# AsherJingkongChen/vlm-bridge-for-image-captioning

Hardware: NVIDIA B200
Metric: bridge fwd+bwd samples/sec (higher is better)
Workload: dtype bf16

## Files before the change

### include/b200_bridge.h

```cpp
#ifndef B200_BRIDGE_H_
#define B200_BRIDGE_H_

#include <stddef.h>
#include <stdint.h>

#ifdef __cplusplus
extern "C" {
#endif

#define B200B_ABI_VERSION 3

#define B200B_OK 0
#define B200B_ERR_SHAPE (-1)
#define B200B_ERR_ALIGN (-2)
#define B200B_ERR_ARG (-3)
#define B200B_ERR_DRIVER (-4)
#define B200B_ERR_TENSORMAP (-5)
#define B200B_ERR_WORKSPACE (-6)
#define B200B_ERR_DEVICE (-7)

int b200b_abi_version(void);
const char* b200b_last_error(void);
uint64_t b200b_launch_count(void);

int b200b_profile_begin(void* stream);
int b200b_profile_end(void);
const char* b200b_profile_entry(int index, float* ms);


enum b200b_epilogue {
  B200B_EPI_BF16_BIAS = 0,
  B200B_EPI_BF16_BIAS_GELU = 1,
  B200B_EPI_F32_BIAS_RESID = 2,
  B200B_EPI_BF16_DGELU = 3,
  B200B_EPI_F32 = 4
};

typedef struct b200b_gemm_args {
  const void* a;
  const void* b;
  int32_t a_major, b_major;
  int32_t m, n, k;
  int64_t lda, ldb;
  int32_t epilogue;
  int32_t block_n;
  void* out;
  int64_t ldo;
  void* aux;
  int64_t ldaux;
  const float* bias;
  const float* resid;
  int64_t ldr;
  float beta;
  float dropout_p;
  uint64_t seed;
  uint32_t dropout_stream;
  uint32_t cta_group;
} b200b_gemm_args;

int b200b_gemm(const b200b_gemm_args* args, void* stream);

int b200b_gemm_dual(const b200b_gemm_args* dgrad, const b200b_gemm_args* wgrad, void* stream);
int b200b_gemm_set_dual(int on);


int b200b_layernorm_fwd(const float* x, const float* gamma, const float* beta, void* y_bf16,
                        float* mean, float* rstd, int rows, int dim, float eps, void* stream);

int b200b_layernorm_bwd(const void* dy_bf16, const float* x, const float* mean, const float* rstd,
                        const float* gamma, const float* dres, float* dx, int rows, int dim,
                        void* stream);

size_t b200b_colsum_workspace_bytes(int rows, int cols);
int b200b_colsum(const void* dy_bf16, int64_t ld, const float* x, const float* mean,
                 const float* rstd, float* out_sum, float* out_gsum, int rows, int cols,
                 void* workspace, size_t workspace_bytes, void* stream);

int b200b_cast_bf16(const float* in, void* out_bf16, int64_t n, float dropout_p, uint64_t seed,
                    uint32_t dropout_stream, void* stream);

#define B200B_MAX_COLSUM_TASKS 16
typedef struct b200b_colsum_task {
  const float* partials;
  float* out;
  int32_t cols, chunks;
  int64_t chunk_stride;
} b200b_colsum_task;

int b200b_row_chunks(int rows);
int b200b_layernorm_fwd_rows(const float* x, const float* gamma, const float* beta, void* y_bf16,
                             float* mean, float* rstd, int rows, int dim, float eps, void* stream);
int b200b_layernorm_bwd_fused(const void* dy_bf16, const float* x, const float* mean, const float* rstd,
                              const float* gamma, const float* dres, float* dx, void* dy_next_bf16,
                              float* partials, int rows, int dim, void* stream);
int b200b_cast_bf16_colsum(const float* in, void* out_bf16, float* partials, int rows, int dim,
                           float dropout_p, uint64_t seed, uint32_t dropout_stream, void* stream);
int b200b_colsum_partials(const void* dy_bf16, int64_t ld, int rows, int cols, float* partials,
                          int* chunks_out, void* stream);
int b200b_colsum_finalize(const b200b_colsum_task* tasks, int ntasks, void* stream);

typedef struct b200b_attn_args {
  const void* q; int64_t ldq;
  const void* k; int64_t ldk;
  const void* v; int64_t ldv;
  void* o; int64_t ldo;
  float* lse;
  const void* d_o; int64_t lddo;
  void* dq; int64_t lddq;
  void* dk; int64_t lddk;
  void* dv; int64_t lddv;
  void* workspace; uint64_t workspace_bytes;
  int32_t batch, heads, len_q, len_k, head_dim;
  float dropout_p;
  uint64_t seed;
  uint32_t dropout_stream;
  uint32_t reserved;
} b200b_attn_args;

int b200b_attention_fwd(const b200b_attn_args* args, void* stream);
int b200b_attention_set_tc(int mask);
size_t b200b_attention_bwd_workspace_bytes(int batch, int heads, int len_q, int len_k);
int b200b_attention_bwd(const b200b_attn_args* args, void* stream);

size_t b200b_kv_cache_packed_bytes(int batch, int len_k, int heads, int head_dim, int num_blocks);
int b200b_kv_cache_pack(const void* kv, int64_t ldkv, void* packed, int batch, int len_k, int heads,
                        int head_dim, int num_blocks, void* stream);
int b200b_attention_decode_packed(const void* q, int64_t ldq, const void* kv_packed, int block_index,
                                  int num_blocks, void* o, int64_t ldo, float* lse, int batch, int heads,
                                  int len_q, int len_k, int head_dim, void* stream);

size_t b200b_kv_cache_tc_bytes(int batch, int len_k, int heads, int head_dim, int num_blocks);
int b200b_kv_cache_pack_tc(const void* kv, int64_t ldkv, void* packed, int batch, int len_k, int heads,
                           int head_dim, int num_blocks, void* stream);
int b200b_attention_decode_tc(const void* q, int64_t ldq, const void* kv_tc, int block_index, int num_blocks,
                              void* o, int64_t ldo, float* lse, int batch, int heads, int len_q, int len_k,
                              int head_dim, void* stream);

typedef struct b200b_bridge_dims {
  int32_t batch, len_text, len_vision;
  int32_t dim, dim_vision, dim_ffn;
  int32_t heads_cross, heads_self;
  int32_t num_blocks;
  int32_t flags;
} b200b_bridge_dims;

#define B200B_BRIDGE_WGRAD_BF16 1
#define B200B_BRIDGE_SEED_INDIRECT 2
#define B200B_BRIDGE_KV_PACKED 4
#define B200B_BRIDGE_KV_TC 8
#define B200B_BRIDGE_PART_CROSS 16
#define B200B_BRIDGE_PART_REST 32
#define B200B_SEED_INDIRECT 0x80000000u

typedef struct b200b_block_weights {
  const void* wq_c;
  const void* wo_c;
  const void* wqkv_s;
  const void* wo_s;
  const void* w1;
  const void* w2;
  const float* bq_c;
  const float* bo_c;
  const float* bqkv_s;
  const float* bo_s;
  const float* b1;
  const float* b2;
  const float* ln_c_g; const float* ln_c_b;
  const float* ln_s_g; const float* ln_s_b;
  const float* ln_f_g; const float* ln_f_b;
} b200b_block_weights;

typedef struct b200b_block_grads {
  void* wq_c; void* wo_c; void* wqkv_s; void* wo_s; void* w1; void* w2;
  float* bq_c; float* bo_c; float* bqkv_s; float* bo_s; float* b1; float* b2;
  float* ln_c_g; float* ln_c_b; float* ln_s_g; float* ln_s_b; float* ln_f_g; float* ln_f_b;
} b200b_block_grads;

size_t b200b_bridge_block_saved_bytes(const b200b_bridge_dims* dims);
size_t b200b_bridge_backward_workspace_bytes(const b200b_bridge_dims* dims);

int b200b_bridge_kv_project(const b200b_bridge_dims* dims, const float* vision_f32,
                            const void* wkv_all, const float* bkv_all, void* vision_bf16,
                            void* kv, void* stream);

int b200b_bridge_block_forward(const b200b_bridge_dims* dims, int block_index,
                               const b200b_block_weights* w, const float* x_in, const void* kv,
                               float* x_out, void* saved, size_t saved_bytes, float dropout_p,
                               uint64_t seed, void* stream);

typedef void (*b200b_grad_ready_fn)(void* user, const void* grad, int64_t elems);
typedef struct b200b_grad_notify {
  b200b_grad_ready_fn fn;
  void* user;
} b200b_grad_notify;

int b200b_bridge_block_backward(const b200b_bridge_dims* dims, int block_index,
                                const b200b_block_weights* w, const float* x_in, const void* kv,
                                const void* saved, const float* d_out, float* d_in, void* dkv,
                                const b200b_block_grads* g, void* workspace, size_t workspace_bytes,
                                float dropout_p, uint64_t seed, const b200b_grad_notify* notify,
                                void* stream);

int b200b_bridge_kv_backward(const b200b_bridge_dims* dims, const void* vision_bf16,
                             const void* dkv, void* dwkv_all, float* dbkv_all, void* workspace,
                             size_t workspace_bytes, void* stream);

size_t b200b_bridge_f32_workspace_bytes(const b200b_bridge_dims* dims);
int b200b_bridge_kv_project_f32(const b200b_bridge_dims* dims, const float* vision, const float* wkv_all,
                                const float* bkv_all, float* kv, void* stream);
int b200b_bridge_block_forward_f32(const b200b_bridge_dims* dims, int block_index, const b200b_block_weights* w,
                                   const float* x_in, const float* kv, float* x_out, void* workspace,
                                   size_t workspace_bytes, void* stream);

size_t b200b_grad_sqnorm_workspace_bytes(void);
int b200b_grad_sqnorm(const float* grad, int64_t n, const void* grad_bf16, int64_t n_bf16, void* workspace,
                      size_t workspace_bytes, float* out2, void* stream);
int b200b_adamw_fused(float* param, const float* grad, const void* grad_bf16, float* exp_avg, float* exp_avg_sq,
                      void* weights_bf16,
                      int64_t n, int64_t n_bf16, const float* sqnorm2, float max_grad_norm,
                      const float* grad_scale, const float* found_inf, float lr, float beta1, float beta2,
                      float eps, float weight_decay, int64_t step, float* step_dev, void* stream);

int b200b_cross_entropy_fwd(const void* logits, int dtype, int64_t ld, const int64_t* labels, int64_t rows,
                            int64_t vocab, int64_t ignore_index, int64_t shift_len, float* lse,
                            float* loss_rows, float* out2, void* stream);
int b200b_cross_entropy_bwd(const void* logits, int dtype, int64_t ld, const int64_t* labels, int64_t rows,
                            int64_t vocab, int64_t ignore_index, int64_t shift_len, const float* lse,
                            const float* out2, const float* grad_loss, void* dlogits, int64_t ldd,
                            void* stream);

int b200b_bf16_to_f32(const void* in_bf16, float* out, int64_t n, float scale, void* stream);

#define B200B_NVLS_MAX_RANKS 8
#define B200B_NVLS_MAX_BLOCKS 160
#define B200B_DTYPE_BF16 0
#define B200B_DTYPE_F32 1
typedef struct b200b_nvls_comm {
  void* multicast_base;
  void* local_base;
  void* flags[B200B_NVLS_MAX_RANKS];
  int32_t rank, world;
  int32_t timeout_s;
  int32_t reserved;
  void* error_word;
} b200b_nvls_comm;
#define B200B_NVLS_OUT_MULTICAST 1u
#define B200B_NVLS_EXCLUSIVE_SMS 2u
#define B200B_NVLS_UNROLL(n) (((uint32_t)(n) & 0xffu) << 8)
size_t b200b_allreduce_nvls_flag_bytes(void);
int b200b_allreduce_nvls(const b200b_nvls_comm* comm, int dtype, int64_t byte_offset, int64_t bytes,
                         float scale, float* out_f32, uint32_t epoch, const uint32_t* epoch_base,
                         int blocks, int threads, uint32_t flags, void* stream);

void b200b_set_sm_limit(int sms);
int b200b_get_sm_limit(void);

#ifdef __cplusplus
}
#endif
#endif
```

### vlm-bridge-for-image-captioning_b200/_lib.py

```python
from __future__ import annotations

import ctypes as C
import os
import threading

_PKG_DIR = os.path.dirname(os.path.abspath(__file__))
LIB_PATH = os.path.join(_PKG_DIR, "csrc", "libb200_bridge.so")

EPI_BF16_BIAS = 0
EPI_BF16_BIAS_GELU = 1
EPI_F32_BIAS_RESID = 2
EPI_BF16_DGELU = 3
EPI_F32 = 4
NVLS_OUT_MULTICAST = 1
NVLS_EXCLUSIVE_SMS = 2


class GemmArgs(C.Structure):
    _fields_ = [
        ("a", C.c_void_p),
        ("b", C.c_void_p),
        ("a_major", C.c_int32),
        ("b_major", C.c_int32),
        ("m", C.c_int32),
        ("n", C.c_int32),
        ("k", C.c_int32),
        ("lda", C.c_int64),
        ("ldb", C.c_int64),
        ("epilogue", C.c_int32),
        ("block_n", C.c_int32),
        ("out", C.c_void_p),
        ("ldo", C.c_int64),
        ("aux", C.c_void_p),
        ("ldaux", C.c_int64),
        ("bias", C.c_void_p),
        ("resid", C.c_void_p),
        ("ldr", C.c_int64),
        ("beta", C.c_float),
        ("dropout_p", C.c_float),
        ("seed", C.c_uint64),
        ("dropout_stream", C.c_uint32),
        ("cta_group", C.c_uint32),
    ]


class ColsumTask(C.Structure):
    _fields_ = [("partials", C.c_void_p), ("out", C.c_void_p), ("cols", C.c_int32), ("chunks", C.c_int32),
                ("chunk_stride", C.c_int64)]


class NvlsComm(C.Structure):
    _fields_ = [("multicast_base", C.c_void_p), ("local_base", C.c_void_p), ("flags", C.c_void_p * 8),
                ("rank", C.c_int32), ("world", C.c_int32), ("timeout_s", C.c_int32), ("reserved", C.c_int32),
                ("error_word", C.c_void_p)]


class AttnArgs(C.Structure):
    _fields_ = [
        ("q", C.c_void_p), ("ldq", C.c_int64),
        ("k", C.c_void_p), ("ldk", C.c_int64),
        ("v", C.c_void_p), ("ldv", C.c_int64),
        ("o", C.c_void_p), ("ldo", C.c_int64),
        ("lse", C.c_void_p),
        ("d_o", C.c_void_p), ("lddo", C.c_int64),
        ("dq", C.c_void_p), ("lddq", C.c_int64),
        ("dk", C.c_void_p), ("lddk", C.c_int64),
        ("dv", C.c_void_p), ("lddv", C.c_int64),
        ("workspace", C.c_void_p), ("workspace_bytes", C.c_uint64),
        ("batch", C.c_int32), ("heads", C.c_int32), ("len_q", C.c_int32), ("len_k", C.c_int32),
        ("head_dim", C.c_int32),
        ("dropout_p", C.c_float),
        ("seed", C.c_uint64),
        ("dropout_stream", C.c_uint32),
        ("reserved", C.c_uint32),
    ]


_lock = threading.Lock()
_lib = None


def _declare(lib) -> None:
    lib.b200b_abi_version.restype = C.c_int
    lib.b200b_abi_version.argtypes = []
    lib.b200b_last_error.restype = C.c_char_p
    lib.b200b_last_error.argtypes = []
    lib.b200b_launch_count.restype = C.c_uint64
    lib.b200b_launch_count.argtypes = []
    lib.b200b_profile_begin.restype = C.c_int
    lib.b200b_profile_begin.argtypes = [C.c_void_p]
    lib.b200b_profile_end.restype = C.c_int
    lib.b200b_profile_end.argtypes = []
    lib.b200b_profile_entry.restype = C.c_char_p
    lib.b200b_profile_entry.argtypes = [C.c_int, C.POINTER(C.c_float)]
    lib.b200b_gemm.restype = C.c_int
    lib.b200b_gemm.argtypes = [C.POINTER(GemmArgs), C.c_void_p]
    lib.b200b_layernorm_fwd.restype = C.c_int
    lib.b200b_layernorm_fwd.argtypes = [C.c_void_p] * 6 + [C.c_int, C.c_int, C.c_float, C.c_void_p]
    lib.b200b_layernorm_bwd.restype = C.c_int
    lib.b200b_layernorm_bwd.argtypes = [C.c_void_p] * 7 + [C.c_int, C.c_int, C.c_void_p]
    lib.b200b_colsum_workspace_bytes.restype = C.c_size_t
    lib.b200b_colsum_workspace_bytes.argtypes = [C.c_int, C.c_int]
    lib.b200b_colsum.restype = C.c_int
    lib.b200b_colsum.argtypes = [C.c_void_p, C.c_int64] + [C.c_void_p] * 5 + [C.c_int, C.c_int, C.c_void_p,
                                                                               C.c_size_t, C.c_void_p]
    lib.b200b_cast_bf16.restype = C.c_int
    lib.b200b_cast_bf16.argtypes = [C.c_void_p, C.c_void_p, C.c_int64, C.c_float, C.c_uint64, C.c_uint32,
                                    C.c_void_p]
    lib.b200b_row_chunks.restype = C.c_int
    lib.b200b_row_chunks.argtypes = [C.c_int]
    lib.b200b_layernorm_fwd_rows.restype = C.c_int
    lib.b200b_layernorm_fwd_rows.argtypes = [C.c_void_p] * 6 + [C.c_int, C.c_int, C.c_float, C.c_void_p]
    lib.b200b_layernorm_bwd_fused.restype = C.c_int
    lib.b200b_layernorm_bwd_fused.argtypes = [C.c_void_p] * 9 + [C.c_int, C.c_int, C.c_void_p]
    lib.b200b_cast_bf16_colsum.restype = C.c_int
    lib.b200b_cast_bf16_colsum.argtypes = [C.c_void_p] * 3 + [C.c_int, C.c_int, C.c_float, C.c_uint64, C.c_uint32,
                                           C.c_void_p]
    lib.b200b_colsum_partials.restype = C.c_int
    lib.b200b_colsum_partials.argtypes = [C.c_void_p, C.c_int64, C.c_int, C.c_int, C.c_void_p, C.POINTER(C.c_int),
                                          C.c_void_p]
    lib.b200b_bf16_to_f32.restype = C.c_int
    lib.b200b_bf16_to_f32.argtypes = [C.c_void_p, C.c_void_p, C.c_int64, C.c_float, C.c_void_p]
    lib.b200b_allreduce_nvls_flag_bytes.restype = C.c_size_t
    lib.b200b_allreduce_nvls_flag_bytes.argtypes = []
    lib.b200b_allreduce_nvls.restype = C.c_int
    lib.b200b_allreduce_nvls.argtypes = [C.POINTER(NvlsComm), C.c_int, C.c_int64, C.c_int64, C.c_float, C.c_void_p,
                                         C.c_uint32, C.c_void_p, C.c_int, C.c_int, C.c_uint32, C.c_void_p]
    lib.b200b_grad_sqnorm_workspace_bytes.restype = C.c_size_t
    lib.b200b_grad_sqnorm_workspace_bytes.argtypes = []
    lib.b200b_grad_sqnorm.restype = C.c_int
    lib.b200b_grad_sqnorm.argtypes = [C.c_void_p, C.c_int64, C.c_void_p, C.c_int64, C.c_void_p, C.c_size_t, C.c_void_p, C.c_void_p]
    lib.b200b_adamw_fused.restype = C.c_int
    lib.b200b_adamw_fused.argtypes = [C.c_void_p] * 6 + [C.c_int64, C.c_int64, C.c_void_p, C.c_float, C.c_void_p,
                                                          C.c_void_p] + [C.c_float] * 5 + [C.c_int64, C.c_void_p, C.c_void_p]
    lib.b200b_cross_entropy_fwd.restype = C.c_int
    lib.b200b_cross_entropy_fwd.argtypes = [C.c_void_p, C.c_int, C.c_int64, C.c_void_p] + [C.c_int64] * 4 + [C.c_void_p] * 4
    lib.b200b_cross_entropy_bwd.restype = C.c_int
    lib.b200b_cross_entropy_bwd.argtypes = ([C.c_void_p, C.c_int, C.c_int64, C.c_void_p] + [C.c_int64] * 4 +
                                            [C.c_void_p] * 4 + [C.c_int64, C.c_void_p])
    lib.b200b_gemm_dual.restype = C.c_int
    lib.b200b_gemm_dual.argtypes = [C.POINTER(GemmArgs), C.POINTER(GemmArgs), C.c_void_p]
    lib.b200b_gemm_set_dual.restype = C.c_int
    lib.b200b_gemm_set_dual.argtypes = [C.c_int]
    lib.b200b_attention_set_tc.restype = C.c_int
    lib.b200b_attention_set_tc.argtypes = [C.c_int]
    lib.b200b_set_sm_limit.restype = None
    lib.b200b_set_sm_limit.argtypes = [C.c_int]
    lib.b200b_get_sm_limit.restype = C.c_int
    lib.b200b_get_sm_limit.argtypes = []
    lib.b200b_colsum_finalize.restype = C.c_int
    lib.b200b_colsum_finalize.argtypes = [C.POINTER(ColsumTask), C.c_int, C.c_void_p]
    lib.b200b_attention_fwd.restype = C.c_int
    lib.b200b_attention_fwd.argtypes = [C.POINTER(AttnArgs), C.c_void_p]
    lib.b200b_kv_cache_packed_bytes.restype = C.c_size_t
    lib.b200b_kv_cache_packed_bytes.argtypes = [C.c_int] * 5
    lib.b200b_kv_cache_pack.restype = C.c_int
    lib.b200b_kv_cache_pack.argtypes = [C.c_void_p, C.c_int64, C.c_void_p] + [C.c_int] * 5 + [C.c_void_p]
    lib.b200b_attention_decode_packed.restype = C.c_int
    lib.b200b_attention_decode_packed.argtypes = [C.c_void_p, C.c_int64, C.c_void_p, C.c_int, C.c_int, C.c_void_p,
                                                  C.c_int64, C.c_void_p] + [C.c_int] * 5 + [C.c_void_p]
    lib.b200b_kv_cache_tc_bytes.restype = C.c_size_t
    lib.b200b_kv_cache_tc_bytes.argtypes = [C.c_int] * 5
    lib.b200b_kv_cache_pack_tc.restype = C.c_int
    lib.b200b_kv_cache_pack_tc.argtypes = [C.c_void_p, C.c_int64, C.c_void_p] + [C.c_int] * 5 + [C.c_void_p]
    lib.b200b_attention_decode_tc.restype = C.c_int
    lib.b200b_attention_decode_tc.argtypes = [C.c_void_p, C.c_int64, C.c_void_p, C.c_int, C.c_int, C.c_void_p,
                                              C.c_int64, C.c_void_p] + [C.c_int] * 5 + [C.c_void_p]
    lib.b200b_attention_bwd_workspace_bytes.restype = C.c_size_t
    lib.b200b_attention_bwd_workspace_bytes.argtypes = [C.c_int] * 4
    lib.b200b_attention_bwd.restype = C.c_int
    lib.b200b_attention_bwd.argtypes = [C.POINTER(AttnArgs), C.c_void_p]


def lib():
    global _lib
    if _lib is None:
        with _lock:
            if _lib is None:
                if not os.path.exists(LIB_PATH):
                    raise RuntimeError(
                        f"{LIB_PATH} is missing: build it with `python -m vlm_bridge_b200.build` "
                        "(there is no CPU or PyTorch fallback for the bridge kernels)"
                    )
                handle = C.CDLL(LIB_PATH)
                _declare(handle)
                _lib = handle
    return _lib


def check(rc: int, what: str) -> None:
    if rc != 0:
        msg = lib().b200b_last_error().decode("utf-8", "replace")
        raise RuntimeError(f"b200b {what} failed (rc={rc}): {msg}")


def launch_count() -> int:
    return int(lib().b200b_launch_count())


def profile_begin(stream_ptr: int) -> None:
    check(lib().b200b_profile_begin(C.c_void_p(stream_ptr)), "profile_begin")


def profile_end() -> list[tuple[str, float]]:
    n = lib().b200b_profile_end()
    out = []
    ms = C.c_float()
    for i in range(n):
        name = lib().b200b_profile_entry(i, C.byref(ms))
        if name is None:
            break
        out.append((name.decode(), float(ms.value)))
    return out
```

### vlm-bridge-for-image-captioning_b200/csrc/bridge.cu

```cuda
#include <string.h>

#include "common.cuh"
#include "launch.h"

namespace b200b {

static inline size_t al256(size_t x) { return (x + 255) & ~(size_t)255; }

struct Carver {
  uint8_t* base;
  size_t off = 0;
  explicit Carver(void* b) : base(reinterpret_cast<uint8_t*>(b)) {}
  template <typename T>
  T* take(size_t count) {
    T* p = reinterpret_cast<T*>(base + off);
    off += al256(count * sizeof(T));
    return p;
  }
};

struct Dims {
  int B, L, Nv, D, Dv, F, Hc, Hs, nb, flags;
  size_t T, Tv;
  int dc, ds;
};

static int read_dims(const b200b_bridge_dims* d, Dims* o, const char* what) {
  if (d == nullptr) {
    set_last_error("%s: null dims", what);
    return B200B_ERR_ARG;
  }
  o->B = d->batch; o->L = d->len_text; o->Nv = d->len_vision;
  o->D = d->dim; o->Dv = d->dim_vision; o->F = d->dim_ffn;
  o->Hc = d->heads_cross; o->Hs = d->heads_self; o->nb = d->num_blocks; o->flags = d->flags;
  if (o->B <= 0 || o->L <= 0 || o->Nv <= 0 || o->D <= 0 || o->Dv <= 0 || o->F <= 0 || o->Hc <= 0 || o->Hs <= 0 ||
      o->nb <= 0) {
    set_last_error("%s: all dims must be positive", what);
    return B200B_ERR_SHAPE;
  }
  if ((o->D % 8) || (o->Dv % 8) || (o->F % 8) || (o->D % o->Hc) || (o->D % o->Hs)) {
    set_last_error("%s: dim/dim_vision/dim_ffn must be multiples of 8 and dim divisible by the head counts", what);
    return B200B_ERR_SHAPE;
  }
  o->T = (size_t)o->B * o->L;
  o->Tv = (size_t)o->B * o->Nv;
  o->dc = o->D / o->Hc;
  o->ds = o->D / o->Hs;
  if (o->T > 0x7fffffff || o->Tv > 0x7fffffff) {
    set_last_error("%s: too many rows", what);
    return B200B_ERR_SHAPE;
  }
  return B200B_OK;
}

struct Saved {
  __nv_bfloat16 *xn1, *q, *o1, *xn2, *qkv, *o2, *xn3, *u, *h;
  float *x1, *x2;
  float *mean1, *rstd1, *mean2, *rstd2, *mean3, *rstd3;
  float *lse1, *lse2;
  size_t bytes;
};

static Saved carve_saved(const Dims& d, void* base) {
  Carver c(base);
  Saved s;
  const size_t TD = d.T * d.D, TF = d.T * d.F;
  s.xn1 = c.take<__nv_bfloat16>(TD);
  s.q = c.take<__nv_bfloat16>(TD);
  s.o1 = c.take<__nv_bfloat16>(TD);
  s.xn2 = c.take<__nv_bfloat16>(TD);
  s.qkv = c.take<__nv_bfloat16>(3 * TD);
  s.o2 = c.take<__nv_bfloat16>(TD);
  s.xn3 = c.take<__nv_bfloat16>(TD);
  s.u = c.take<__nv_bfloat16>(TF);
  s.h = c.take<__nv_bfloat16>(TF);
  s.x1 = c.take<float>(TD);
  s.x2 = c.take<float>(TD);
  s.mean1 = c.take<float>(d.T); s.rstd1 = c.take<float>(d.T);
  s.mean2 = c.take<float>(d.T); s.rstd2 = c.take<float>(d.T);
  s.mean3 = c.take<float>(d.T); s.rstd3 = c.take<float>(d.T);
  s.lse1 = c.take<float>((size_t)d.B * d.Hc * d.L);
  s.lse2 = c.take<float>((size_t)d.B * d.Hs * d.L);
  s.bytes = c.off;
  return s;
}

constexpr int kMaxRowChunks = 320;
struct BwdWs {
  __nv_bfloat16 *dy, *du, *dxn, *dattn, *dqkv;
  float* dx;
  uint8_t* attn_ws; size_t attn_ws_bytes;
  float *p_cast, *p_du, *p_lnf, *p_dqkv, *p_lns, *p_dq, *p_lnc, *p_dkv;
  size_t bytes;
};

static BwdWs carve_bwd(const Dims& d, void* base) {
  Carver c(base);
  BwdWs w;
  const size_t TD = d.T * d.D, TF = d.T * d.F;
  w.dy = c.take<__nv_bfloat16>(TD);
  w.du = c.take<__nv_bfloat16>(TF);
  w.dxn = c.take<__nv_bfloat16>(TD);
  w.dattn = c.take<__nv_bfloat16>(TD);
  w.dqkv = c.take<__nv_bfloat16>(3 * TD);
  w.dx = c.take<float>(TD);
  const size_t a1 = b200b_attention_bwd_workspace_bytes(d.B, d.Hc, d.L, d.Nv);
  const size_t a2 = b200b_attention_bwd_workspace_bytes(d.B, d.Hs, d.L, d.L);
  w.attn_ws_bytes = a1 > a2 ? a1 : a2;
  w.attn_ws = c.take<uint8_t>(w.attn_ws_bytes);
  const size_t rc = d.T < (size_t)kMaxRowChunks ? d.T : (size_t)kMaxRowChunks;
  const size_t D = d.D;
  w.p_cast = c.take<float>(rc * D);
  w.p_du = c.take<float>((size_t)64 * d.F);
  w.p_lnf = c.take<float>(rc * 3 * D);
  w.p_dqkv = c.take<float>((size_t)64 * 3 * D);
  w.p_lns = c.take<float>(rc * 3 * D);
  w.p_dq = c.take<float>((size_t)64 * D);
  w.p_lnc = c.take<float>(rc * 3 * D);
  w.p_dkv = c.take<float>((size_t)64 * 2 * D * d.nb);
  w.bytes = c.off;
  return w;
}

struct Finalizer {
  b200b_colsum_task t[B200B_MAX_COLSUM_TASKS];
  int n = 0;
  void add(const float* partials, float* out, int cols, int chunks, long long stride) {
    t[n].partials = partials; t[n].out = out; t[n].cols = cols; t[n].chunks = chunks; t[n].chunk_stride = stride;
    ++n;
  }
};

#define B200B_TRY(expr)        \
  do {                         \
    int rc_ = (expr);          \
    if (rc_ != B200B_OK) return rc_; \
  } while (0)

static int gemm(const void* a, int a_major, long long lda, const void* b, int b_major, long long ldb, int m, int n,
                int k, int epi, void* out, long long ldo, const float* bias, const float* resid, void* aux,
                long long ldaux, float p, uint64_t seed, uint32_t dstream, cudaStream_t st) {
  b200b_gemm_args g;
  memset(&g, 0, sizeof(g));
  g.a = a; g.b = b; g.a_major = a_major; g.b_major = b_major;
  g.m = m; g.n = n; g.k = k; g.lda = lda; g.ldb = ldb;
  g.epilogue = epi; g.block_n = 0;
  g.out = out; g.ldo = ldo; g.aux = aux; g.ldaux = ldaux;
  g.bias = bias; g.resid = resid; g.ldr = ldo;
  g.beta = 0.f; g.dropout_p = p; g.seed = seed; g.dropout_stream = dstream;
  return b200b_gemm(&g, st);
}

static int grad_pair(const void* dy, long long lddy, const void* w, const void* x, long long ldx, int rows, int n_out,
                     int n_in, void* dx, long long lddx, void* dw, int wgrad_epi, cudaStream_t st) {
  b200b_gemm_args dg, wg;
  memset(&dg, 0, sizeof(dg));
  memset(&wg, 0, sizeof(wg));
  dg.a = dy; dg.a_major = 0; dg.lda = lddy;
  dg.b = w; dg.b_major = 1; dg.ldb = n_in;
  dg.m = rows; dg.n = n_in; dg.k = n_out;
  dg.epilogue = B200B_EPI_BF16_BIAS; dg.out = dx; dg.ldo = lddx;
  wg.a = dy; wg.a_major = 1; wg.lda = lddy;
  wg.b = x; wg.b_major = 1; wg.ldb = ldx;
  wg.m = n_out; wg.n = n_in; wg.k = rows;
  wg.epilogue = wgrad_epi; wg.out = dw; wg.ldo = n_in;
  return b200b_gemm_dual(&dg, &wg, st);
}

static int attn(bool bwd, const void* q, long long ldq, const void* k, long long ldk, const void* v, long long ldv,
                void* o, long long ldo, float* lse, const void* d_o, void* dq, long long lddq, void* dk, long long lddk,
                void* dv, long long lddv, void* ws, size_t ws_bytes, int B, int H, int Lq, int Lk, int hd, float p,
                uint64_t seed, uint32_t dstream, cudaStream_t st) {
  b200b_attn_args a;
  memset(&a, 0, sizeof(a));
  a.q = q; a.ldq = ldq; a.k = k; a.ldk = ldk; a.v = v; a.ldv = ldv; a.o = o; a.ldo = ldo; a.lse = lse;
  a.d_o = d_o; a.lddo = ldo; a.dq = dq; a.lddq = lddq; a.dk = dk; a.lddk = lddk; a.dv = dv; a.lddv = lddv;
  a.workspace = ws; a.workspace_bytes = ws_bytes;
  a.batch = B; a.heads = H; a.len_q = Lq; a.len_k = Lk; a.head_dim = hd;
  a.dropout_p = p; a.seed = seed; a.dropout_stream = dstream;
  return bwd ? b200b_attention_bwd(&a, st) : b200b_attention_fwd(&a, st);
}

static inline uint32_t ds_cross(int i) { return 16u * i + 0; }
static inline uint32_t ds_self(int i) { return 16u * i + 1; }
static inline uint32_t ds_ffn_h(int i) { return 16u * i + 2; }
static inline uint32_t ds_ffn_o(int i) { return 16u * i + 3; }

}

using namespace b200b;

extern "C" size_t b200b_bridge_block_saved_bytes(const b200b_bridge_dims* dims) {
  Dims d;
  if (read_dims(dims, &d, "block_saved_bytes") != B200B_OK) return 0;
  return carve_saved(d, nullptr).bytes;
}

extern "C" size_t b200b_bridge_backward_workspace_bytes(const b200b_bridge_dims* dims) {
  Dims d;
  if (read_dims(dims, &d, "backward_workspace_bytes") != B200B_OK) return 0;
  return carve_bwd(d, nullptr).bytes;
}

extern "C" int b200b_bridge_kv_project(const b200b_bridge_dims* dims, const float* vision_f32, const void* wkv_all,
                                       const float* bkv_all, void* vision_bf16, void* kv, void* stream_) {
  cudaStream_t st = reinterpret_cast<cudaStream_t>(stream_);
  Dims d;
  B200B_TRY(read_dims(dims, &d, "kv_project"));
  if (!vision_f32 || !wkv_all || !bkv_all || !vision_bf16 || !kv) {
    set_last_error("kv_project: null argument");
    return B200B_ERR_ARG;
  }
  const int n = 2 * d.D * d.nb;
  B200B_TRY(b200b_cast_bf16(vision_f32, vision_bf16, (int64_t)d.Tv * d.Dv, 0.f, 0, 0, st));
  return gemm(vision_bf16, 0, d.Dv, wkv_all, 0, d.Dv, (int)d.Tv, n, d.Dv, B200B_EPI_BF16_BIAS, kv, n, bkv_all, nullptr,
              nullptr, 0, 0.f, 0, 0, st);
}

extern "C" int b200b_bridge_block_forward(const b200b_bridge_dims* dims, int i, const b200b_block_weights* w,
                                          const float* x_in, const void* kv, float* x_out, void* saved,
                                          size_t saved_bytes, float p, uint64_t seed, void* stream_) {
  cudaStream_t st = reinterpret_cast<cudaStream_t>(stream_);
  Dims d;
  B200B_TRY(read_dims(dims, &d, "block_forward"));
  if (!w || !x_in || !kv || !x_out || !saved || i < 0 || i >= d.nb) {
    set_last_error("block_forward: null argument or bad block index");
    return B200B_ERR_ARG;
  }
  Saved s = carve_saved(d, saved);
  if (saved_bytes < s.bytes) {
    set_last_error("block_forward: saved arena too small (%zu < %zu)", saved_bytes, s.bytes);
    return B200B_ERR_WORKSPACE;
  }
  const int T = (int)d.T, D = d.D, F = d.F;
  const uint32_t ind = (d.flags & B200B_BRIDGE_SEED_INDIRECT) ? B200B_SEED_INDIRECT : 0u;
  const long long ldkv = 2LL * D * d.nb;
  const __nv_bfloat16* kblk = reinterpret_cast<const __nv_bfloat16*>(kv) + (size_t)2 * D * i;
  const float eps = 1e-5f;

  const bool do_cross = !(d.flags & B200B_BRIDGE_PART_REST), do_rest = !(d.flags & B200B_BRIDGE_PART_CROSS);
  if (!do_cross && !do_rest) {
    set_last_error("block_forward: PART_CROSS and PART_REST are exclusive");
    return B200B_ERR_ARG;
  }
  if ((!do_cross || !do_rest) && p != 0.f) {
    set_last_error("block_forward: running a part of a block needs dropout_p == 0");
    return B200B_ERR_ARG;
  }
  float* x1w = do_rest ? s.x1 : x_out;
  const float* x1 = do_cross ? x1w : x_in;

  if (do_cross) {
    B200B_TRY(b200b_layernorm_fwd_rows(x_in, w->ln_c_g, w->ln_c_b, s.xn1, s.mean1, s.rstd1, T, D, eps, st));
    B200B_TRY(gemm(s.xn1, 0, D, w->wq_c, 0, D, T, D, D, B200B_EPI_BF16_BIAS, s.q, D, w->bq_c, nullptr, nullptr, 0, 0.f,
                   0, 0, st));
    if (d.flags & (B200B_BRIDGE_KV_PACKED | B200B_BRIDGE_KV_TC)) {
      if (p != 0.f || d.L > 64) {
        set_last_error("block_forward: a packed K/V cache needs dropout_p == 0 and len_text <= 64");
        return B200B_ERR_ARG;
      }
      if (d.flags & B200B_BRIDGE_KV_TC)
        B200B_TRY(b200b_attention_decode_tc(s.q, D, kv, i, d.nb, s.o1, D, s.lse1, d.B, d.Hc, d.L, d.Nv, d.dc, st));
      else
        B200B_TRY(b200b_attention_decode_packed(s.q, D, kv, i, d.nb, s.o1, D, s.lse1, d.B, d.Hc, d.L, d.Nv, d.dc, st));
    } else {
      B200B_TRY(attn(false, s.q, D, kblk, ldkv, kblk + D, ldkv, s.o1, D, s.lse1, nullptr, nullptr, 0, nullptr, 0,
                     nullptr, 0, nullptr, 0, d.B, d.Hc, d.L, d.Nv, d.dc, p, seed, (ds_cross(i) | ind), st));
    }
    B200B_TRY(gemm(s.o1, 0, D, w->wo_c, 0, D, T, D, D, B200B_EPI_F32_BIAS_RESID, x1w, D, w->bo_c, x_in, nullptr, 0, 0.f,
                   0, 0, st));
  }
  if (!do_rest) return B200B_OK;
  B200B_TRY(b200b_layernorm_fwd_rows(x1, w->ln_s_g, w->ln_s_b, s.xn2, s.mean2, s.rstd2, T, D, eps, st));
  B200B_TRY(gemm(s.xn2, 0, D, w->wqkv_s, 0, D, T, 3 * D, D, B200B_EPI_BF16_BIAS, s.qkv, 3 * D, w->bqkv_s, nullptr,
                 nullptr, 0, 0.f, 0, 0, st));
  B200B_TRY(attn(false, s.qkv, 3 * D, s.qkv + D, 3 * D, s.qkv + 2 * D, 3 * D, s.o2, D, s.lse2, nullptr, nullptr, 0,
                 nullptr, 0, nullptr, 0, nullptr, 0, d.B, d.Hs, d.L, d.L, d.ds, p, seed, (ds_self(i) | ind), st));
  B200B_TRY(gemm(s.o2, 0, D, w->wo_s, 0, D, T, D, D, B200B_EPI_F32_BIAS_RESID, s.x2, D, w->bo_s, x1, nullptr, 0, 0.f,
                 0, 0, st));
  B200B_TRY(b200b_layernorm_fwd_rows(s.x2, w->ln_f_g, w->ln_f_b, s.xn3, s.mean3, s.rstd3, T, D, eps, st));
  B200B_TRY(gemm(s.xn3, 0, D, w->w1, 0, D, T, F, D, B200B_EPI_BF16_BIAS_GELU, s.h, F, w->b1, nullptr, s.u, F, p, seed,
                 (ds_ffn_h(i) | ind), st));
  B200B_TRY(gemm(s.h, 0, F, w->w2, 0, F, T, D, F, B200B_EPI_F32_BIAS_RESID, x_out, D, w->b2, s.x2, nullptr, 0, p, seed,
                 (ds_ffn_o(i) | ind), st));
  return B200B_OK;
}

extern "C" int b200b_bridge_block_backward(const b200b_bridge_dims* dims, int i, const b200b_block_weights* w,
                                           const float* x_in, const void* kv, const void* saved, const float* d_out,
                                           float* d_in, void* dkv, const b200b_block_grads* g, void* workspace,
                                           size_t workspace_bytes, float p, uint64_t seed,
                                           const b200b_grad_notify* notify, void* stream_) {
  cudaStream_t st = reinterpret_cast<cudaStream_t>(stream_);
  Dims d;
  B200B_TRY(read_dims(dims, &d, "block_backward"));
  if (!w || !x_in || !kv || !saved || !d_out || !dkv || !g || !workspace || i < 0 || i >= d.nb) {
    set_last_error("block_backward: null argument or bad block index");
    return B200B_ERR_ARG;
  }
  Saved s = carve_saved(d, const_cast<void*>(saved));
  BwdWs ws = carve_bwd(d, workspace);
  if (workspace_bytes < ws.bytes) {
    set_last_error("block_backward: workspace too small (%zu < %zu)", workspace_bytes, ws.bytes);
    return B200B_ERR_WORKSPACE;
  }
  const int T = (int)d.T, D = d.D, F = d.F;
  const uint32_t ind = (d.flags & B200B_BRIDGE_SEED_INDIRECT) ? B200B_SEED_INDIRECT : 0u;
  const long long ldkv = 2LL * D * d.nb;
  const __nv_bfloat16* kblk = reinterpret_cast<const __nv_bfloat16*>(kv) + (size_t)2 * D * i;
  __nv_bfloat16* dkblk = reinterpret_cast<__nv_bfloat16*>(dkv) + (size_t)2 * D * i;
  const int EB = B200B_EPI_BF16_BIAS;
  const int EW = (d.flags & B200B_BRIDGE_WGRAD_BF16) ? B200B_EPI_BF16_BIAS : B200B_EPI_F32;
  auto ready = [&](const void* grad, long long elems) {
    if (notify != nullptr && notify->fn != nullptr) notify->fn(notify->user, grad, elems);
  };

  const int rchunks = b200b_row_chunks(T);
  if (rchunks <= 0 || rchunks > kMaxRowChunks) {
    set_last_error("block_backward: no usable device (row chunks = %d)", rchunks);
    return B200B_ERR_DEVICE;
  }
  Finalizer fin;
  int ch = 0;

  B200B_TRY(b200b_cast_bf16_colsum(d_out, ws.dy, ws.p_cast, T, D, p, seed, (ds_ffn_o(i) | ind), st));
  fin.add(ws.p_cast, g->b2, D, rchunks, D);
  B200B_TRY(gemm(ws.dy, 1, D, s.h, 1, F, D, F, T, EW, g->w2, F, nullptr, nullptr, nullptr, 0, 0.f, 0, 0, st));
  ready(g->w2, (long long)D * F);
  B200B_TRY(gemm(ws.dy, 0, D, w->w2, 1, F, T, F, D, B200B_EPI_BF16_DGELU, ws.du, F, nullptr, nullptr, s.u, F, p, seed,
                 (ds_ffn_h(i) | ind), st));
  B200B_TRY(b200b_colsum_partials(ws.du, F, T, F, ws.p_du, &ch, st));
  fin.add(ws.p_du, g->b1, F, ch, F);
  B200B_TRY(gemm(ws.du, 1, F, s.xn3, 1, D, F, D, T, EW, g->w1, D, nullptr, nullptr, nullptr, 0, 0.f, 0, 0, st));
  ready(g->w1, (long long)F * D);
  B200B_TRY(gemm(ws.du, 0, F, w->w1, 1, D, T, D, F, EB, ws.dxn, D, nullptr, nullptr, nullptr, 0, 0.f, 0, 0, st));
  B200B_TRY(b200b_layernorm_bwd_fused(ws.dxn, s.x2, s.mean3, s.rstd3, w->ln_f_g, d_out, ws.dx, ws.dy, ws.p_lnf, T, D, st));
  fin.add(ws.p_lnf, g->ln_f_b, D, rchunks, 3LL * D);
  fin.add(ws.p_lnf + D, g->ln_f_g, D, rchunks, 3LL * D);
  fin.add(ws.p_lnf + 2 * D, g->bo_s, D, rchunks, 3LL * D);
  B200B_TRY(grad_pair(ws.dy, D, w->wo_s, s.o2, D, T, D, D, ws.dattn, D, g->wo_s, EW, st));
  ready(g->wo_s, (long long)D * D);
  B200B_TRY(attn(true, s.qkv, 3 * D, s.qkv + D, 3 * D, s.qkv + 2 * D, 3 * D, s.o2, D, s.lse2, ws.dattn, ws.dqkv, 3 * D,
                 ws.dqkv + D, 3 * D, ws.dqkv + 2 * D, 3 * D, ws.attn_ws, ws.attn_ws_bytes, d.B, d.Hs, d.L, d.L, d.ds, p,
                 seed, (ds_self(i) | ind), st));
  B200B_TRY(b200b_colsum_partials(ws.dqkv, 3 * D, T, 3 * D, ws.p_dqkv, &ch, st));
  fin.add(ws.p_dqkv, g->bqkv_s, 3 * D, ch, 3LL * D);
  B200B_TRY(grad_pair(ws.dqkv, 3 * D, w->wqkv_s, s.xn2, D, T, 3 * D, D, ws.dxn, D, g->wqkv_s, EW, st));
  ready(g->wqkv_s, 3LL * D * D);
  B200B_TRY(b200b_layernorm_bwd_fused(ws.dxn, s.x1, s.mean2, s.rstd2, w->ln_s_g, ws.dx, ws.dx, ws.dy, ws.p_lns, T, D, st));
  fin.add(ws.p_lns, g->ln_s_b, D, rchunks, 3LL * D);
  fin.add(ws.p_lns + D, g->ln_s_g, D, rchunks, 3LL * D);
  fin.add(ws.p_lns + 2 * D, g->bo_c, D, rchunks, 3LL * D);
  B200B_TRY(grad_pair(ws.dy, D, w->wo_c, s.o1, D, T, D, D, ws.dattn, D, g->wo_c, EW, st));
  ready(g->wo_c, (long long)D * D);
  __nv_bfloat16* dq = ws.dqkv;
  B200B_TRY(attn(true, s.q, D, kblk, ldkv, kblk + D, ldkv, s.o1, D, s.lse1, ws.dattn, dq, D, dkblk, ldkv, dkblk + D, ldkv,
                 ws.attn_ws, ws.attn_ws_bytes, d.B, d.Hc, d.L, d.Nv, d.dc, p, seed, (ds_cross(i) | ind), st));
  B200B_TRY(b200b_colsum_partials(dq, D, T, D, ws.p_dq, &ch, st));
  fin.add(ws.p_dq, g->bq_c, D, ch, D);
  B200B_TRY(grad_pair(dq, D, w->wq_c, s.xn1, D, T, D, D, ws.dxn, D, g->wq_c, EW, st));
  ready(g->wq_c, (long long)D * D);
  B200B_TRY(b200b_layernorm_bwd_fused(ws.dxn, x_in, s.mean1, s.rstd1, w->ln_c_g, ws.dx, d_in, nullptr, ws.p_lnc, T, D, st));
  fin.add(ws.p_lnc, g->ln_c_b, D, rchunks, 3LL * D);
  fin.add(ws.p_lnc + D, g->ln_c_g, D, rchunks, 3LL * D);
  return b200b_colsum_finalize(fin.t, fin.n, st);
}

extern "C" int b200b_bridge_kv_backward(const b200b_bridge_dims* dims, const void* vision_bf16, const void* dkv,
                                        void* dwkv_all, float* dbkv_all, void* workspace, size_t workspace_bytes,
                                        void* stream_) {
  cudaStream_t st = reinterpret_cast<cudaStream_t>(stream_);
  Dims d;
  B200B_TRY(read_dims(dims, &d, "kv_backward"));
  if (!vision_bf16 || !dkv || !dwkv_all || !dbkv_all || !workspace) {
    set_last_error("kv_backward: null argument");
    return B200B_ERR_ARG;
  }
  BwdWs ws = carve_bwd(d, workspace);
  if (workspace_bytes < ws.bytes) {
    set_last_error("kv_backward: workspace too small (%zu < %zu)", workspace_bytes, ws.bytes);
    return B200B_ERR_WORKSPACE;
  }
  const int n = 2 * d.D * d.nb;
  int ch = 0;
  B200B_TRY(b200b_colsum_partials(dkv, n, (int)d.Tv, n, ws.p_dkv, &ch, st));
  b200b_colsum_task t;
  t.partials = ws.p_dkv; t.out = dbkv_all; t.cols = n; t.chunks = ch; t.chunk_stride = n;
  B200B_TRY(b200b_colsum_finalize(&t, 1, st));
  const int EW = (d.flags & B200B_BRIDGE_WGRAD_BF16) ? B200B_EPI_BF16_BIAS : B200B_EPI_F32;
  return gemm(dkv, 1, n, vision_bf16, 1, d.Dv, n, d.Dv, (int)d.Tv, EW, dwkv_all, d.Dv, nullptr, nullptr,
              nullptr, 0, 0.f, 0, 0, st);
}
```

### vlm-bridge-for-image-captioning_b200/csrc/common.cuh

```cuda
#pragma once

#include <cuda.h>
#include <cuda_bf16.h>
#include <cuda_runtime.h>
#include <stdint.h>
#include <stdio.h>

#include "../../include/b200_bridge.h"

namespace b200b {

__device__ __forceinline__ uint32_t smem_u32(const void* p) {
  return static_cast<uint32_t>(__cvta_generic_to_shared(p));
}
__device__ __forceinline__ int lane_id() { return threadIdx.x & 31; }

__device__ __forceinline__ uint32_t pack_bf16(float lo, float hi) {
  __nv_bfloat162 v = __floats2bfloat162_rn(lo, hi);
  return *reinterpret_cast<uint32_t*>(&v);
}
__device__ __forceinline__ float bf16_round(float x) {
  return __bfloat162float(__float2bfloat16_rn(x));
}
__device__ __forceinline__ float bf16_lo(uint32_t v) { return __uint_as_float(v << 16); }
__device__ __forceinline__ float bf16_hi(uint32_t v) { return __uint_as_float(v & 0xffff0000u); }

__device__ __forceinline__ float warp_sum(float v) {
#pragma unroll
  for (int o = 16; o > 0; o >>= 1) v += __shfl_xor_sync(0xffffffffu, v, o);
  return v;
}
__device__ __forceinline__ float warp_max(float v) {
#pragma unroll
  for (int o = 16; o > 0; o >>= 1) v = fmaxf(v, __shfl_xor_sync(0xffffffffu, v, o));
  return v;
}

__device__ __forceinline__ float rcp_approx(float x) {
  float r;
  asm("rcp.approx.ftz.f32 %0, %1;" : "=f"(r) : "f"(x));
  return r;
}
__device__ __forceinline__ float ex2_approx(float x) {
  float r;
  asm("ex2.approx.ftz.f32 %0, %1;" : "=f"(r) : "f"(x));
  return r;
}
__device__ __forceinline__ float normal_cdf(float x, float* gauss) {
  const float z = fabsf(x) * 0.70710678118654752440f;
  const float t = rcp_approx(fmaf(0.3275911f, z, 1.0f));
  float poly = fmaf(t, 1.061405429f, -1.453152027f);
  poly = fmaf(poly, t, 1.421413741f);
  poly = fmaf(poly, t, -0.284496736f);
  poly = fmaf(poly, t, 0.254829592f);
  poly *= t;
  const float e = ex2_approx(-1.4426950408889634f * z * z);
  *gauss = e;
  const float half_erfc = 0.5f * poly * e;
  return x >= 0.0f ? 1.0f - half_erfc : half_erfc;
}
__device__ __forceinline__ float gelu_erf(float x) {
  float g;
  return x * normal_cdf(x, &g);
}
__device__ __forceinline__ float gelu_erf_grad(float x) {
  float g;
  const float cdf = normal_cdf(x, &g);
  return fmaf(x * 0.39894228040143267794f, g, cdf);
}

struct DropoutCfg {
  uint32_t thr;
  float scale;
  uint32_t seed_lo, seed_hi;
  const unsigned long long* seed_ptr;
};

__device__ __forceinline__ DropoutCfg dropout_resolve(DropoutCfg d) {
  if (d.seed_ptr != nullptr && d.thr != 0) {
    const unsigned long long s = __ldg(d.seed_ptr);
    d.seed_lo = (uint32_t)s;
    d.seed_hi = (uint32_t)(s >> 32);
  }
  return d;
}

__device__ __forceinline__ uint4 philox4x32_10(uint4 ctr, uint2 key) {
  constexpr uint32_t M0 = 0xD2511F53u, M1 = 0xCD9E8D57u, W0 = 0x9E3779B9u, W1 = 0xBB67AE85u;
#pragma unroll
  for (int r = 0; r < 10; ++r) {
    const uint32_t hi0 = __umulhi(M0, ctr.x), lo0 = M0 * ctr.x;
    const uint32_t hi1 = __umulhi(M1, ctr.z), lo1 = M1 * ctr.z;
    ctr = make_uint4(hi1 ^ ctr.y ^ key.x, lo1, hi0 ^ ctr.w ^ key.y, lo0);
    key.x += W0;
    key.y += W1;
  }
  return ctr;
}

__device__ __forceinline__ uint4 dropout_bits8(const DropoutCfg& d, uint32_t stream, uint64_t group) {
  return philox4x32_10(make_uint4((uint32_t)group, (uint32_t)(group >> 32), stream, 0x0b200b00u),
                       make_uint2(d.seed_lo, d.seed_hi));
}
__device__ __forceinline__ bool dropout_keep(const uint4& bits, int e , uint32_t thr) {
  const uint32_t w = (e < 4) ? ((e < 2) ? bits.x : bits.y) : ((e < 6) ? bits.z : bits.w);
  const uint32_t u = (e & 1) ? (w >> 16) : (w & 0xffffu);
  return u >= thr;
}

__device__ __forceinline__ void pdl_launch_dependents() {
  asm volatile("griddepcontrol.launch_dependents;" ::: "memory");
}
__device__ __forceinline__ void pdl_wait() { asm volatile("griddepcontrol.wait;" ::: "memory"); }
__device__ __forceinline__ void pdl_prologue() {
  pdl_launch_dependents();
  pdl_wait();
}
__device__ __forceinline__ void pdl_prologue_late_trigger() { pdl_wait(); }

__device__ __forceinline__ void mbar_init(uint64_t* bar, uint32_t count) {
  asm volatile("mbarrier.init.shared::cta.b64 [%0], %1;" ::"r"(smem_u32(bar)), "r"(count));
}
__device__ __forceinline__ void fence_barrier_init() {
  asm volatile("fence.mbarrier_init.release.cluster;" ::: "memory");
}
__device__ __forceinline__ void fence_proxy_async() {
  asm volatile("fence.proxy.async.shared::cta;" ::: "memory");
}
__device__ __forceinline__ void mbar_arrive(uint64_t* bar) {
  asm volatile("mbarrier.arrive.shared::cta.b64 _, [%0];" ::"r"(smem_u32(bar)) : "memory");
}
__device__ __forceinline__ void mbar_arrive_expect_tx(uint64_t* bar, uint32_t bytes) {
  asm volatile("mbarrier.arrive.expect_tx.shared::cta.b64 _, [%0], %1;" ::"r"(smem_u32(bar)),
               "r"(bytes)
               : "memory");
}
__device__ __forceinline__ bool mbar_try_wait(uint64_t* bar, uint32_t parity) {
  uint32_t ok;
  asm volatile(
      "{\n\t"
      ".reg .pred p;\n\t"
      "mbarrier.try_wait.parity.shared::cta.b64 p, [%1], %2;\n\t"
      "selp.b32 %0, 1, 0, p;\n\t"
      "}"
      : "=r"(ok)
      : "r"(smem_u32(bar)), "r"(parity)
      : "memory");
  return ok != 0;
}
__device__ __forceinline__ void mbar_wait(uint64_t* bar, uint32_t parity) {
  if (mbar_try_wait(bar, parity)) return;
  const long long t0 = clock64();
  while (!mbar_try_wait(bar, parity)) {
    if (clock64() - t0 > 4000000000LL) {
      printf("b200b: mbarrier wait timed out (block %d thread %d)\n", (int)blockIdx.x, (int)threadIdx.x);
      __trap();
    }
  }
}

__device__ __forceinline__ void tma_prefetch_desc(const CUtensorMap* tm) {
  asm volatile("prefetch.tensormap [%0];" ::"l"(reinterpret_cast<uint64_t>(tm)) : "memory");
}
__device__ __forceinline__ void tma_load_2d(void* smem_dst, const CUtensorMap* tm, uint64_t* bar,
                                            int c_inner, int c_outer) {
  asm volatile(
      "cp.async.bulk.tensor.2d.shared::cluster.global.mbarrier::complete_tx::bytes"
      " [%0], [%1, {%3, %4}], [%2];"
      :
      : "r"(smem_u32(smem_dst)), "l"(reinterpret_cast<uint64_t>(tm)), "r"(smem_u32(bar)),
        "r"(c_inner), "r"(c_outer)
      : "memory");
}
__device__ __forceinline__ void bulk_load_1d(void* smem_dst, const void* gsrc, uint32_t bytes,
                                             uint64_t* bar) {
  asm volatile(
      "cp.async.bulk.shared::cluster.global.mbarrier::complete_tx::bytes [%0], [%1], %2, [%3];"
      :
      : "r"(smem_u32(smem_dst)), "l"(reinterpret_cast<uint64_t>(gsrc)), "r"(bytes),
        "r"(smem_u32(bar))
      : "memory");
}

__device__ __forceinline__ void tmem_alloc(uint32_t* dst_smem, uint32_t ncols) {
  asm volatile("tcgen05.alloc.cta_group::1.sync.aligned.shared::cta.b32 [%0], %1;" ::"r"(
                   smem_u32(dst_smem)),
               "r"(ncols)
               : "memory");
}
__device__ __forceinline__ void tmem_relinquish() {
  asm volatile("tcgen05.relinquish_alloc_permit.cta_group::1.sync.aligned;" ::: "memory");
}
__device__ __forceinline__ void tmem_dealloc(uint32_t taddr, uint32_t ncols) {
  asm volatile("tcgen05.dealloc.cta_group::1.sync.aligned.b32 %0, %1;" ::"r"(taddr), "r"(ncols)
               : "memory");
}
__device__ __forceinline__ void tc_fence_before() {
  asm volatile("tcgen05.fence::before_thread_sync;" ::: "memory");
}
__device__ __forceinline__ void tc_fence_after() {
  asm volatile("tcgen05.fence::after_thread_sync;" ::: "memory");
}
__device__ __forceinline__ void umma_bf16(uint32_t d_tmem, uint64_t a_desc, uint64_t b_desc,
                                          uint32_t idesc, uint32_t accumulate) {
  asm volatile(
      "{\n\t"
      ".reg .pred p;\n\t"
      "setp.ne.b32 p, %4, 0;\n\t"
      "tcgen05.mma.cta_group::1.kind::f16 [%0], %1, %2, %3, p;\n\t"
      "}"
      :
      : "r"(d_tmem), "l"(a_desc), "l"(b_desc), "r"(idesc), "r"(accumulate)
      : "memory");
}
__device__ __forceinline__ void umma_commit(uint64_t* bar) {
  asm volatile("tcgen05.commit.cta_group::1.mbarrier::arrive::one.shared::cluster.b64 [%0];" ::"r"(
                   smem_u32(bar))
               : "memory");
}
__device__ __forceinline__ void tmem_ld_32x32(uint32_t taddr, uint32_t (&v)[32]) {
  asm volatile(
      "tcgen05.ld.sync.aligned.32x32b.x32.b32 "
      "{%0, %1, %2, %3, %4, %5, %6, %7, %8, %9, %10, %11, %12, %13, %14, %15, "
      "%16, %17, %18, %19, %20, %21, %22, %23, %24, %25, %26, %27, %28, %29, %30, %31}, [%32];"
      : "=r"(v[0]), "=r"(v[1]), "=r"(v[2]), "=r"(v[3]), "=r"(v[4]), "=r"(v[5]), "=r"(v[6]),
        "=r"(v[7]), "=r"(v[8]), "=r"(v[9]), "=r"(v[10]), "=r"(v[11]), "=r"(v[12]), "=r"(v[13]),
        "=r"(v[14]), "=r"(v[15]), "=r"(v[16]), "=r"(v[17]), "=r"(v[18]), "=r"(v[19]), "=r"(v[20]),
        "=r"(v[21]), "=r"(v[22]), "=r"(v[23]), "=r"(v[24]), "=r"(v[25]), "=r"(v[26]), "=r"(v[27]),
        "=r"(v[28]), "=r"(v[29]), "=r"(v[30]), "=r"(v[31])
      : "r"(taddr)
      : "memory");
}
__device__ __forceinline__ void tmem_ld_wait() {
  asm volatile("tcgen05.wait::ld.sync.aligned;" ::: "memory");
}

__device__ __forceinline__ uint64_t umma_smem_desc(uint32_t smem_addr, uint32_t lbo_bytes,
                                                   uint32_t sbo_bytes) {
  uint64_t d = 0;
  d |= (uint64_t)((smem_addr & 0x3FFFFu) >> 4);
  d |= (uint64_t)((lbo_bytes >> 4) & 0x3FFFu) << 16;
  d |= (uint64_t)((sbo_bytes >> 4) & 0x3FFFu) << 32;
  d |= (uint64_t)1 << 46;
  d |= (uint64_t)2 << 61;
  return d;
}
__host__ __device__ constexpr uint32_t umma_idesc_bf16(int m, int n, bool a_mn, bool b_mn) {
  return (1u << 4) | (1u << 7) | (1u << 10) | ((a_mn ? 1u : 0u) << 15) | ((b_mn ? 1u : 0u) << 16) |
         ((uint32_t)(n >> 3) << 17) | ((uint32_t)(m >> 4) << 24);
}

__device__ __forceinline__ uint32_t cluster_ctarank() {
  uint32_t r;
  asm volatile("mov.u32 %0, %%cluster_ctarank;" : "=r"(r));
  return r;
}
__device__ __forceinline__ uint32_t cluster_id_x() {
  uint32_t r;
  asm volatile("mov.u32 %0, %%clusterid.x;" : "=r"(r));
  return r;
}
__device__ __forceinline__ uint32_t cluster_nctaid_x() {
  uint32_t r;
  asm volatile("mov.u32 %0, %%nclusterid.x;" : "=r"(r));
  return r;
}
__device__ __forceinline__ void cluster_sync_all() {
  asm volatile("barrier.cluster.arrive.release.aligned;\n\tbarrier.cluster.wait.acquire.aligned;" ::: "memory");
}
__device__ __forceinline__ void mbar_arrive_cluster(uint64_t* bar, uint32_t rank) {
  asm volatile(
      "{\n\t"
      ".reg .b32 ra;\n\t"
      "mapa.shared::cluster.u32 ra, %0, %1;\n\t"
      "mbarrier.arrive.shared::cluster.b64 _, [ra];\n\t"
      "}" ::"r"(smem_u32(bar)),
      "r"(rank)
      : "memory");
}
__device__ __forceinline__ void tma_load_2d_pair(void* smem_dst, const CUtensorMap* tm, uint64_t* bar,
                                                 int c_inner, int c_outer) {
  asm volatile(
      "cp.async.bulk.tensor.2d.cta_group::2.shared::cluster.global.mbarrier::complete_tx::bytes"
      " [%0], [%1, {%3, %4}], [%2];"
      :
      : "r"(smem_u32(smem_dst)), "l"(reinterpret_cast<uint64_t>(tm)), "r"(smem_u32(bar) & 0xFEFFFFFFu),
        "r"(c_inner), "r"(c_outer)
      : "memory");
}
__device__ __forceinline__ void tmem_alloc_pair(uint32_t* dst_smem, uint32_t ncols) {
  asm volatile("tcgen05.alloc.cta_group::2.sync.aligned.shared::cta.b32 [%0], %1;" ::"r"(smem_u32(dst_smem)),
               "r"(ncols)
               : "memory");
}
__device__ __forceinline__ void tmem_relinquish_pair() {
  asm volatile("tcgen05.relinquish_alloc_permit.cta_group::2.sync.aligned;" ::: "memory");
}
__device__ __forceinline__ void tmem_dealloc_pair(uint32_t taddr, uint32_t ncols) {
  asm volatile("tcgen05.dealloc.cta_group::2.sync.aligned.b32 %0, %1;" ::"r"(taddr), "r"(ncols) : "memory");
}
__device__ __forceinline__ void umma_bf16_pair(uint32_t d_tmem, uint64_t a_desc, uint64_t b_desc, uint32_t idesc,
                                               uint32_t accumulate) {
  asm volatile(
      "{\n\t"
      ".reg .pred p;\n\t"
      "setp.ne.b32 p, %4, 0;\n\t"
      "tcgen05.mma.cta_group::2.kind::f16 [%0], %1, %2, %3, p;\n\t"
      "}"
      :
      : "r"(d_tmem), "l"(a_desc), "l"(b_desc), "r"(idesc), "r"(accumulate)
      : "memory");
}
__device__ __forceinline__ void umma_commit_pair(uint64_t* bar, uint16_t mask) {
  asm volatile(
      "tcgen05.commit.cta_group::2.mbarrier::arrive::one.shared::cluster.multicast::cluster.b64 [%0], %1;" ::"r"(
          smem_u32(bar)),
      "h"(mask)
      : "memory");
}

__device__ __forceinline__ bool elect_one() {
  uint32_t pred = 0;
  asm volatile(
      "{\n\t"
      ".reg .b32 rx;\n\t"
      ".reg .pred px;\n\t"
      "elect.sync rx|px, 0xffffffff;\n\t"
      "@px mov.s32 %0, 1;\n\t"
      "}"
      : "+r"(pred));
  return pred != 0;
}
__device__ __forceinline__ void mbar_arrive_a(uint32_t bar) {
  asm volatile("mbarrier.arrive.shared::cta.b64 _, [%0];" ::"r"(bar) : "memory");
}
__device__ __forceinline__ void mbar_arrive_expect_tx_a(uint32_t bar, uint32_t bytes) {
  asm volatile("mbarrier.arrive.expect_tx.shared::cta.b64 _, [%0], %1;" ::"r"(bar), "r"(bytes) : "memory");
}
__device__ __forceinline__ bool mbar_try_wait_a(uint32_t bar, uint32_t parity) {
  uint32_t ok;
  asm volatile(
      "{\n\t"
      ".reg .pred p;\n\t"
      "mbarrier.try_wait.parity.shared::cta.b64 p, [%1], %2;\n\t"
      "selp.b32 %0, 1, 0, p;\n\t"
      "}"
      : "=r"(ok)
      : "r"(bar), "r"(parity)
      : "memory");
  return ok != 0;
}
static __device__ __noinline__ void mbar_wait_slow_a(uint32_t bar, uint32_t parity) {
  const long long t0 = clock64();
  while (!mbar_try_wait_a(bar, parity)) {
    if (clock64() - t0 > 4000000000LL) {
      printf("b200b: mbarrier wait timed out (block %d thread %d)\n", (int)blockIdx.x, (int)threadIdx.x);
      __trap();
    }
  }
}
__device__ __forceinline__ void mbar_wait_a(uint32_t bar, uint32_t parity) {
  if (mbar_try_wait_a(bar, parity)) return;
  if (mbar_try_wait_a(bar, parity)) return;
  mbar_wait_slow_a(bar, parity);
}
__device__ __forceinline__ void tma_load_2d_a(uint32_t smem_dst, const CUtensorMap* tm, uint32_t bar, int c_inner,
                                              int c_outer) {
  asm volatile(
      "cp.async.bulk.tensor.2d.shared::cluster.global.mbarrier::complete_tx::bytes"
      " [%0], [%1, {%3, %4}], [%2];"
      :
      : "r"(smem_dst), "l"(reinterpret_cast<uint64_t>(tm)), "r"(bar), "r"(c_inner), "r"(c_outer)
      : "memory");
}
__device__ __forceinline__ void tma_load_2d_pair_a(uint32_t smem_dst, const CUtensorMap* tm, uint32_t bar_even_cta,
                                                   int c_inner, int c_outer) {
  asm volatile(
      "cp.async.bulk.tensor.2d.cta_group::2.shared::cluster.global.mbarrier::complete_tx::bytes"
      " [%0], [%1, {%3, %4}], [%2];"
      :
      : "r"(smem_dst), "l"(reinterpret_cast<uint64_t>(tm)), "r"(bar_even_cta), "r"(c_inner), "r"(c_outer)
      : "memory");
}
__device__ __forceinline__ void umma_commit_a(uint32_t bar) {
  asm volatile("tcgen05.commit.cta_group::1.mbarrier::arrive::one.shared::cluster.b64 [%0];" ::"r"(bar) : "memory");
}
__device__ __forceinline__ void umma_commit_pair_a(uint32_t bar, uint16_t mask) {
  asm volatile(
      "tcgen05.commit.cta_group::2.mbarrier::arrive::one.shared::cluster.multicast::cluster.b64 [%0], %1;" ::"r"(bar),
      "h"(mask)
      : "memory");
}
__device__ __forceinline__ uint32_t mapa_u32(uint32_t addr, uint32_t rank) {
  uint32_t r;
  asm volatile("mapa.shared::cluster.u32 %0, %1, %2;" : "=r"(r) : "r"(addr), "r"(rank));
  return r;
}
__device__ __forceinline__ void mbar_arrive_cluster_a(uint32_t cluster_addr) {
  asm volatile("mbarrier.arrive.shared::cluster.b64 _, [%0];" ::"r"(cluster_addr) : "memory");
}

__device__ __forceinline__ void tmem_ld_32x32_x16(uint32_t taddr, uint32_t (&v)[16]) {
  asm volatile(
      "tcgen05.ld.sync.aligned.32x32b.x16.b32 "
      "{%0, %1, %2, %3, %4, %5, %6, %7, %8, %9, %10, %11, %12, %13, %14, %15}, [%16];"
      : "=r"(v[0]), "=r"(v[1]), "=r"(v[2]), "=r"(v[3]), "=r"(v[4]), "=r"(v[5]), "=r"(v[6]), "=r"(v[7]), "=r"(v[8]),
        "=r"(v[9]), "=r"(v[10]), "=r"(v[11]), "=r"(v[12]), "=r"(v[13]), "=r"(v[14]), "=r"(v[15])
      : "r"(taddr)
      : "memory");
}
__device__ __forceinline__ void tmem_st_32x32_x16(uint32_t taddr, const uint32_t (&v)[16]) {
  asm volatile(
      "tcgen05.st.sync.aligned.32x32b.x16.b32 [%0], "
      "{%1, %2, %3, %4, %5, %6, %7, %8, %9, %10, %11, %12, %13, %14, %15, %16};" ::"r"(taddr),
      "r"(v[0]), "r"(v[1]), "r"(v[2]), "r"(v[3]), "r"(v[4]), "r"(v[5]), "r"(v[6]), "r"(v[7]), "r"(v[8]), "r"(v[9]),
      "r"(v[10]), "r"(v[11]), "r"(v[12]), "r"(v[13]), "r"(v[14]), "r"(v[15])
      : "memory");
}
__device__ __forceinline__ void tmem_st_wait() { asm volatile("tcgen05.wait::st.sync.aligned;" ::: "memory"); }

__device__ __forceinline__ void umma_bf16_tmem_a(uint32_t d_tmem, uint32_t a_tmem, uint64_t b_desc, uint32_t idesc,
                                                 uint32_t accumulate) {
  asm volatile(
      "{\n\t"
      ".reg .pred p;\n\t"
      "setp.ne.b32 p, %4, 0;\n\t"
      "tcgen05.mma.cta_group::1.kind::f16 [%0], [%1], %2, %3, p;\n\t"
      "}"
      :
      : "r"(d_tmem), "r"(a_tmem), "l"(b_desc), "r"(idesc), "r"(accumulate)
      : "memory");
}

__device__ __forceinline__ uint64_t umma_desc_sw64(uint32_t smem_addr, uint32_t lbo_bytes) {
  uint64_t d = 0;
  d |= (uint64_t)((smem_addr & 0x3FFFFu) >> 4);
  d |= (uint64_t)((lbo_bytes >> 4) & 0x3FFFu) << 16;
  d |= (uint64_t)(512u >> 4) << 32;
  d |= (uint64_t)1 << 46;
  d |= (uint64_t)4 << 61;
  return d;
}
__device__ __forceinline__ uint64_t desc_sw64_kmajor(uint32_t tile, uint32_t rows, int ks) {
  return umma_desc_sw64(tile + (uint32_t)(ks >> 1) * rows * 64u + (uint32_t)(ks & 1) * 32u, 16u);
}
__device__ __forceinline__ uint64_t desc_sw64_mnmajor(uint32_t tile, uint32_t rows, int chunk0, int kc) {
  return umma_desc_sw64(tile + (uint32_t)chunk0 * rows * 64u + (uint32_t)kc * 1024u, rows * 64u);
}
__device__ __forceinline__ uint32_t sw64_unit_offset(uint32_t row, uint32_t col, uint32_t rows) {
  return (col >> 5) * rows * 64u + row * 64u + ((((col >> 3) & 3u) ^ ((row >> 1) & 3u)) << 4);
}
__device__ __forceinline__ void tma_load_4d(uint32_t smem_dst, const CUtensorMap* tm, uint32_t bar, int c0, int c1,
                                            int c2, int c3) {
  asm volatile(
      "cp.async.bulk.tensor.4d.shared::cluster.global.mbarrier::complete_tx::bytes"
      " [%0], [%1, {%3, %4, %5, %6}], [%2];"
      :
      : "r"(smem_dst), "l"(reinterpret_cast<uint64_t>(tm)), "r"(bar), "r"(c0), "r"(c1), "r"(c2), "r"(c3)
      : "memory");
}

__device__ __forceinline__ void mma_m16n8k16(float (&c)[4], const uint32_t (&a)[4],
                                             const uint32_t (&b)[2]) {
  asm volatile(
      "mma.sync.aligned.m16n8k16.row.col.f32.bf16.bf16.f32 {%0,%1,%2,%3}, {%4,%5,%6,%7}, {%8,%9}, "
      "{%0,%1,%2,%3};"
      : "+f"(c[0]), "+f"(c[1]), "+f"(c[2]), "+f"(c[3])
      : "r"(a[0]), "r"(a[1]), "r"(a[2]), "r"(a[3]), "r"(b[0]), "r"(b[1]));
}
__device__ __forceinline__ void ldmatrix_x4(uint32_t (&r)[4], uint32_t saddr) {
  asm volatile("ldmatrix.sync.aligned.m8n8.x4.shared.b16 {%0,%1,%2,%3}, [%4];"
               : "=r"(r[0]), "=r"(r[1]), "=r"(r[2]), "=r"(r[3])
               : "r"(saddr));
}
__device__ __forceinline__ void ldmatrix_x4_trans(uint32_t (&r)[4], uint32_t saddr) {
  asm volatile("ldmatrix.sync.aligned.m8n8.x4.trans.shared.b16 {%0,%1,%2,%3}, [%4];"
               : "=r"(r[0]), "=r"(r[1]), "=r"(r[2]), "=r"(r[3])
               : "r"(saddr));
}
__device__ __forceinline__ void ldmatrix_x2(uint32_t (&r)[2], uint32_t saddr) {
  asm volatile("ldmatrix.sync.aligned.m8n8.x2.shared.b16 {%0,%1}, [%2];"
               : "=r"(r[0]), "=r"(r[1])
               : "r"(saddr));
}
__device__ __forceinline__ void ldmatrix_x2_trans(uint32_t (&r)[2], uint32_t saddr) {
  asm volatile("ldmatrix.sync.aligned.m8n8.x2.trans.shared.b16 {%0,%1}, [%2];"
               : "=r"(r[0]), "=r"(r[1])
               : "r"(saddr));
}

}
```

### vlm-bridge-for-image-captioning_b200/csrc/gemm_sm100.cu

```cuda
#include <stdarg.h>
#include <stdio.h>
#include <stdlib.h>

#include <mutex>

#include "../../include/b200_bridge.h"
#include "common.cuh"
#include "launch.h"

namespace b200b {

struct GemmKernelParams {
  int m, n, k;
  int num_m_blocks, num_n_blocks, num_k_blocks;
  void* out;
  long long ldo;
  void* aux;
  long long ldaux;
  const float* bias;
  const float* resid;
  long long ldr;
  float beta;
  DropoutCfg drop;
  uint32_t drop_stream;
};

constexpr int kBlockM = 128;
constexpr int kBlockK = 64;
constexpr int kUmmaK = 16;
constexpr int kEpiWarps = 8;
constexpr int kGemmThreads = 64 + 32 * kEpiWarps;
constexpr int kProducerWarp = kEpiWarps;
constexpr int kMmaWarp = kEpiWarps + 1;

template <int BLOCK_N>
struct GemmCfg {
  static constexpr int kStages = (BLOCK_N == 256) ? 4 : 6;
  static constexpr uint32_t kABytes = kBlockM * kBlockK * 2;
  static constexpr uint32_t kBBytes = BLOCK_N * kBlockK * 2;
  static constexpr uint32_t kStageBytes = kABytes + kBBytes;
  static constexpr uint32_t kTmemCols = 2 * BLOCK_N;
  static constexpr size_t kSmemBytes = (size_t)kStages * kStageBytes + 1024 + kEpiWarps * 32 * 33 * 4;
};

constexpr int kGroupPasses = 4;

template <int EPI>
struct EpiOperands {
  float4 bias;
  float4 resid[kGroupPasses];
  uint2 aux[kGroupPasses];
};

template <int EPI>
constexpr bool kEpiHasDropout =
    (EPI == B200B_EPI_BF16_BIAS_GELU || EPI == B200B_EPI_F32_BIAS_RESID || EPI == B200B_EPI_BF16_DGELU);

template <int EPI>
__device__ __forceinline__ void epi_fetch(const GemmKernelParams& p, int row0, int col, int r_sub,
                                          EpiOperands<EPI>& o) {
  const bool col_ok = col < p.n;
  if constexpr (EPI == B200B_EPI_BF16_BIAS || EPI == B200B_EPI_BF16_BIAS_GELU || EPI == B200B_EPI_F32_BIAS_RESID) {
    o.bias = (p.bias != nullptr && col_ok) ? __ldg(reinterpret_cast<const float4*>(p.bias + col))
                                           : make_float4(0.f, 0.f, 0.f, 0.f);
  }
  if constexpr (EPI == B200B_EPI_F32_BIAS_RESID) {
#pragma unroll
    for (int pass = 0; pass < kGroupPasses; ++pass) {
      const int r = row0 + 4 * pass + r_sub;
      o.resid[pass] = (col_ok && r < p.m) ? *reinterpret_cast<const float4*>(p.resid + (long long)r * p.ldr + col)
                                          : make_float4(0.f, 0.f, 0.f, 0.f);
    }
  }
  if constexpr (EPI == B200B_EPI_BF16_DGELU) {
#pragma unroll
    for (int pass = 0; pass < kGroupPasses; ++pass) {
      const int r = row0 + 4 * pass + r_sub;
      o.aux[pass] = (col_ok && r < p.m)
                        ? *reinterpret_cast<const uint2*>(reinterpret_cast<const __nv_bfloat16*>(p.aux) +
                                                          (long long)r * p.ldaux + col)
                        : make_uint2(0u, 0u);
    }
  }
}

static __device__ __noinline__ uint4 dropout_bits8_call(uint32_t seed_lo, uint32_t seed_hi, uint32_t stream,
                                                        uint32_t group_lo, uint32_t group_hi) {
  return philox4x32_10(make_uint4(group_lo, group_hi, stream, 0x0b200b00u), make_uint2(seed_lo, seed_hi));
}

__device__ __forceinline__ void epi_dropout_bits(const GemmKernelParams& p, uint2 seed, int row0, int col, int r_sub,
                                                 int cg, uint2 (&w)[kGroupPasses]) {
#pragma unroll
  for (int i = 0; i < kGroupPasses; ++i) w[i] = make_uint2(0u, 0u);
  if (p.drop.thr == 0) return;
  const bool odd = (cg & 1) != 0;
#pragma unroll
  for (int pp = 0; pp < kGroupPasses; pp += 2) {
    const int row = row0 + 4 * (pp + (odd ? 1 : 0)) + r_sub;
    const uint64_t group = ((uint64_t)row * (uint64_t)p.n + (uint64_t)col) >> 3;
    const uint4 b = dropout_bits8_call(seed.x, seed.y, p.drop_stream, (uint32_t)group,
                                       (uint32_t)(group >> 32));
    const uint32_t r0 = __shfl_xor_sync(0xffffffffu, odd ? b.x : b.z, 1);
    const uint32_t r1 = __shfl_xor_sync(0xffffffffu, odd ? b.y : b.w, 1);
    w[pp] = odd ? make_uint2(r0, r1) : make_uint2(b.x, b.y);
    w[pp + 1] = odd ? make_uint2(b.z, b.w) : make_uint2(r0, r1);
  }
}
__device__ __forceinline__ bool keep4(const uint2& w, int i, uint32_t thr) {
  const uint32_t v = (i < 2) ? w.x : w.y;
  return ((i & 1) ? (v >> 16) : (v & 0xffffu)) >= thr;
}

template <int EPI>
__device__ __forceinline__ void epilogue4(const GemmKernelParams& p, int row, int col, float4 acc, const float4& bias,
                                          const float4& resid, const uint2& aux, const uint2& w, bool store) {
  float f[4] = {acc.x, acc.y, acc.z, acc.w};
  const uint32_t thr = p.drop.thr;
  const float scale = p.drop.scale;

  if constexpr (EPI == B200B_EPI_BF16_BIAS || EPI == B200B_EPI_BF16_BIAS_GELU ||
                EPI == B200B_EPI_F32_BIAS_RESID) {
    f[0] += bias.x; f[1] += bias.y; f[2] += bias.z; f[3] += bias.w;
  }

  if constexpr (EPI == B200B_EPI_BF16_BIAS) {
    uint2 o;
    o.x = pack_bf16(f[0], f[1]); o.y = pack_bf16(f[2], f[3]);
    if (store) *reinterpret_cast<uint2*>(reinterpret_cast<__nv_bfloat16*>(p.out) + (long long)row * p.ldo + col) = o;
  } else if constexpr (EPI == B200B_EPI_BF16_BIAS_GELU) {
    float h[4];
#pragma unroll
    for (int i = 0; i < 4; ++i) {
      f[i] = bf16_round(f[i]);
      h[i] = bf16_round(gelu_erf(f[i]));
      h[i] = keep4(w, i, thr) ? h[i] * scale : 0.0f;
    }
    uint2 u, o;
    u.x = pack_bf16(f[0], f[1]); u.y = pack_bf16(f[2], f[3]);
    o.x = pack_bf16(h[0], h[1]); o.y = pack_bf16(h[2], h[3]);
    if (store) {
      *reinterpret_cast<uint2*>(reinterpret_cast<__nv_bfloat16*>(p.aux) + (long long)row * p.ldaux + col) = u;
      *reinterpret_cast<uint2*>(reinterpret_cast<__nv_bfloat16*>(p.out) + (long long)row * p.ldo + col) = o;
    }
  } else if constexpr (EPI == B200B_EPI_F32_BIAS_RESID) {
    const float r[4] = {resid.x, resid.y, resid.z, resid.w};
    float o[4];
#pragma unroll
    for (int i = 0; i < 4; ++i) {
      float y = bf16_round(f[i]);
      if (thr != 0) y = keep4(w, i, thr) ? bf16_round(y * scale) : 0.0f;
      o[i] = r[i] + y;
    }
    if (store)
      *reinterpret_cast<float4*>(reinterpret_cast<float*>(p.out) + (long long)row * p.ldo + col) =
          make_float4(o[0], o[1], o[2], o[3]);
  } else if constexpr (EPI == B200B_EPI_BF16_DGELU) {
    const float u[4] = {bf16_lo(aux.x), bf16_hi(aux.x), bf16_lo(aux.y), bf16_hi(aux.y)};
    float g[4];
#pragma unroll
    for (int i = 0; i < 4; ++i) {
      float d = bf16_round(f[i]);
      if (thr != 0) d = keep4(w, i, thr) ? bf16_round(d * scale) : 0.0f;
      g[i] = d * gelu_erf_grad(u[i]);
    }
    uint2 o;
    o.x = pack_bf16(g[0], g[1]); o.y = pack_bf16(g[2], g[3]);
    if (store) *reinterpret_cast<uint2*>(reinterpret_cast<__nv_bfloat16*>(p.out) + (long long)row * p.ldo + col) = o;
  } else {
    float* op = reinterpret_cast<float*>(p.out) + (long long)row * p.ldo + col;
    if (store) {
      if (p.beta != 0.0f) {
        const float4 o0 = *reinterpret_cast<const float4*>(op);
        f[0] += p.beta * o0.x; f[1] += p.beta * o0.y; f[2] += p.beta * o0.z; f[3] += p.beta * o0.w;
      }
      *reinterpret_cast<float4*>(op) = make_float4(f[0], f[1], f[2], f[3]);
    }
  }
}


constexpr int kEpiLd = 33;
constexpr uint32_t kEpiBytesPerWarp = 32 * kEpiLd * 4;
constexpr uint32_t kEpiBytes = kEpiWarps * kEpiBytesPerWarp;

template <int BLOCK_N, int EPI>
__device__ __forceinline__ void drain_prefetch(const GemmKernelParams& p, int row0, int n_idx, int half, int lane,
                                               EpiOperands<EPI>& ops) {
  epi_fetch<EPI>(p, row0, n_idx + 32 * half + 4 * (lane & 7), lane >> 3, ops);
}

template <int BLOCK_N, int EPI>
__device__ __forceinline__ void drain_accumulator(const GemmKernelParams& p, uint32_t t_row, int row0 ,
                                                  int n_idx, float* stage , int lane, int half,
                                                  EpiOperands<EPI>& ops ,
                                                  uint2 seed ) {
  const int r_sub = lane >> 3, cg = lane & 7;
  constexpr int kChunks = BLOCK_N / 64;
#pragma unroll 1
  for (int i = 0; i < kChunks; ++i) {
    const int c0 = 32 * (2 * i + half);
    if (n_idx + c0 >= p.n) break;
    {
      uint32_t v[32];
      tmem_ld_32x32(t_row + (uint32_t)c0, v);
      tmem_ld_wait();
#pragma unroll
      for (int j = 0; j < 32; ++j) stage[lane * kEpiLd + j] = __uint_as_float(v[j]);
    }
    __syncwarp();
    const int col = n_idx + c0 + 4 * cg;
#pragma unroll 1
    for (int grp = 0; grp < 8 / kGroupPasses; ++grp) {
      const int grow0 = row0 + 4 * kGroupPasses * grp;
      EpiOperands<EPI> nxt;
      {
        const bool last_grp = grp == 8 / kGroupPasses - 1;
        const int nrow0 = last_grp ? row0 : grow0 + 4 * kGroupPasses;
        const int ncol = last_grp ? col + 64 : col;
        if (!(last_grp && i + 1 == kChunks)) epi_fetch<EPI>(p, nrow0, ncol, r_sub, nxt);
      }
      uint2 w[kGroupPasses];
      if constexpr (kEpiHasDropout<EPI>) epi_dropout_bits(p, seed, grow0, col, r_sub, cg, w);
#pragma unroll
      for (int pass = 0; pass < kGroupPasses; ++pass) {
        const int r = 4 * (kGroupPasses * grp + pass) + r_sub;
        const float* sp = stage + r * kEpiLd + 4 * cg;
        const float4 acc = make_float4(sp[0], sp[1], sp[2], sp[3]);
        epilogue4<EPI>(p, row0 + r, col, acc, ops.bias, ops.resid[pass], ops.aux[pass], w[pass],
                       col < p.n && row0 + r < p.m);
      }
      ops = nxt;
    }
    __syncwarp();
  }
}

template <bool MN>
struct DescConsts {
  static constexpr uint32_t kLbo = MN ? 8192u : 16u;
  static constexpr uint32_t kKStep16 = (MN ? 2048u : 32u) >> 4;
};
__device__ __forceinline__ uint64_t desc_with_lo(uint64_t base, uint32_t add16) {
  return base + (uint64_t)add16;
}

template <int BLOCK_N, bool A_MN, bool B_MN, int EPI>
__global__ void __launch_bounds__(kGemmThreads, 1)
gemm_tcgen05_kernel(const __grid_constant__ CUtensorMap tm_a, const __grid_constant__ CUtensorMap tm_b,
                    const GemmKernelParams p) {
  using Cfg = GemmCfg<BLOCK_N>;
  constexpr int kStages = Cfg::kStages;

  extern __shared__ uint8_t smem_raw[];
  __shared__ __align__(8) uint64_t full_bar[kStages];
  __shared__ __align__(8) uint64_t empty_bar[kStages];
  __shared__ __align__(8) uint64_t tmem_full_bar[2];
  __shared__ __align__(8) uint64_t tmem_empty_bar[2];
  __shared__ uint32_t tmem_base_smem;

  const int warp = threadIdx.x >> 5;
  const int lane = threadIdx.x & 31;
  const uint32_t smem0 = (smem_u32(smem_raw) + 1023u) & ~1023u;
  uint8_t* smem_gen = smem_raw + (smem0 - smem_u32(smem_raw));
  const uint32_t full0 = smem_u32(full_bar), empty0 = smem_u32(empty_bar);
  const uint32_t tfull0 = smem_u32(tmem_full_bar), tempty0 = smem_u32(tmem_empty_bar);

  if (warp == kProducerWarp && lane == 0) {
    tma_prefetch_desc(&tm_a);
    tma_prefetch_desc(&tm_b);
#pragma unroll
    for (int s = 0; s < kStages; ++s) {
      mbar_init(&full_bar[s], 1);
      mbar_init(&empty_bar[s], 1);
    }
    mbar_init(&tmem_full_bar[0], 1);
    mbar_init(&tmem_full_bar[1], 1);
    mbar_init(&tmem_empty_bar[0], 32 * kEpiWarps);
    mbar_init(&tmem_empty_bar[1], 32 * kEpiWarps);
    fence_barrier_init();
  }
  if (warp == kMmaWarp) {
    tmem_alloc(&tmem_base_smem, Cfg::kTmemCols);
    tmem_relinquish();
  }
  tc_fence_before();
  __syncthreads();
  tc_fence_after();
  pdl_launch_dependents();
  pdl_wait();
  const uint32_t tmem_base = tmem_base_smem;
  const int num_tiles = p.num_m_blocks * p.num_n_blocks;

  if (warp == kProducerWarp) {
    int stage = 0;
    uint32_t phase = 0;
    for (int tile = blockIdx.x; tile < num_tiles; tile += gridDim.x) {
      const int m_idx = (tile % p.num_m_blocks) * kBlockM;
      const int n_idx = (tile / p.num_m_blocks) * BLOCK_N;
      for (int kb = 0; kb < p.num_k_blocks; ++kb) {
        mbar_wait_a(empty0 + 8u * stage, phase ^ 1);
        if (elect_one()) {
          const uint32_t sa = smem0 + (uint32_t)stage * Cfg::kStageBytes;
          const uint32_t sb = sa + Cfg::kABytes;
          const uint32_t fb = full0 + 8u * stage;
          mbar_arrive_expect_tx_a(fb, Cfg::kStageBytes);
          const int k_idx = kb * kBlockK;
          if constexpr (!A_MN) {
            tma_load_2d_a(sa, &tm_a, fb, k_idx, m_idx);
          } else {
#pragma unroll
            for (int j = 0; j < kBlockM / 64; ++j)
              tma_load_2d_a(sa + j * 8192, &tm_a, fb, m_idx + 64 * j, k_idx);
          }
          if constexpr (!B_MN) {
            tma_load_2d_a(sb, &tm_b, fb, k_idx, n_idx);
          } else {
#pragma unroll
            for (int j = 0; j < BLOCK_N / 64; ++j)
              tma_load_2d_a(sb + j * 8192, &tm_b, fb, n_idx + 64 * j, k_idx);
          }
        }
        __syncwarp();
        if (++stage == kStages) { stage = 0; phase ^= 1; }
      }
    }
  } else if (warp == kMmaWarp) {
    constexpr uint32_t idesc = umma_idesc_bf16(kBlockM, BLOCK_N, A_MN, B_MN);
    const uint64_t adesc0 = umma_smem_desc(smem0, DescConsts<A_MN>::kLbo, 1024u);
    const uint64_t bdesc0 = umma_smem_desc(smem0 + Cfg::kABytes, DescConsts<B_MN>::kLbo, 1024u);
    int stage = 0;
    uint32_t phase = 0;
    int iter = 0;
    for (int tile = blockIdx.x; tile < num_tiles; tile += gridDim.x, ++iter) {
      const int acc = iter & 1;
      const uint32_t acc_phase = (iter >> 1) & 1;
      mbar_wait_a(tempty0 + 8u * acc, acc_phase ^ 1);
      tc_fence_after();
      const uint32_t d_tmem = tmem_base + (uint32_t)(acc * BLOCK_N);
      for (int kb = 0; kb < p.num_k_blocks; ++kb) {
        mbar_wait_a(full0 + 8u * stage, phase);
        tc_fence_after();
        if (elect_one()) {
          const uint32_t soff16 = ((uint32_t)stage * Cfg::kStageBytes) >> 4;
#pragma unroll
          for (int k = 0; k < kBlockK / kUmmaK; ++k) {
            umma_bf16(d_tmem, desc_with_lo(adesc0, soff16 + k * DescConsts<A_MN>::kKStep16),
                      desc_with_lo(bdesc0, soff16 + k * DescConsts<B_MN>::kKStep16), idesc, (kb | k) != 0 ? 1u : 0u);
          }
          umma_commit_a(empty0 + 8u * stage);
          if (kb == p.num_k_blocks - 1) umma_commit_a(tfull0 + 8u * acc);
        }
        __syncwarp();
        if (++stage == kStages) { stage = 0; phase ^= 1; }
      }
    }
  } else {
    const int quad = warp & 3;
    const int half = warp >> 2;
    float* epi_stage =
        reinterpret_cast<float*>(smem_gen + (size_t)kStages * Cfg::kStageBytes) + warp * 32 * kEpiLd;
    const DropoutCfg drop = dropout_resolve(p.drop);
    const uint2 seed = make_uint2(drop.seed_lo, drop.seed_hi);
    int iter = 0;
    for (int tile = blockIdx.x; tile < num_tiles; tile += gridDim.x, ++iter) {
      const int acc = iter & 1;
      const uint32_t acc_phase = (iter >> 1) & 1;
      const int m_idx = (tile % p.num_m_blocks) * kBlockM;
      const int n_idx = (tile / p.num_m_blocks) * BLOCK_N;
      EpiOperands<EPI> ops;
      drain_prefetch<BLOCK_N, EPI>(p, m_idx + quad * 32, n_idx, half, lane, ops);
      mbar_wait_a(tfull0 + 8u * acc, acc_phase);
      tc_fence_after();
      drain_accumulator<BLOCK_N, EPI>(p, tmem_base + ((uint32_t)(quad * 32) << 16) + (uint32_t)(acc * BLOCK_N),
                                      m_idx + quad * 32, n_idx, epi_stage, lane, half, ops, seed);
      tc_fence_before();
      mbar_arrive_a(tempty0 + 8u * acc);
    }
  }

  tc_fence_before();
  __syncthreads();
  if (warp == kMmaWarp) tmem_dealloc(tmem_base, Cfg::kTmemCols);
}

template <int BLOCK_N>
struct GemmPairCfg {
  static constexpr int kStages = (BLOCK_N == 256) ? 5 : 7;
  static constexpr uint32_t kABytes = kBlockM * kBlockK * 2;
  static constexpr uint32_t kBBytes = (BLOCK_N / 2) * kBlockK * 2;
  static constexpr uint32_t kStageBytes = kABytes + kBBytes;
  static constexpr uint32_t kTmemCols = 2 * BLOCK_N;
  static constexpr size_t kSmemBytes = (size_t)kStages * kStageBytes + 1024 + kEpiBytes;
};

template <int BLOCK_N, bool A_MN, bool B_MN, int EPI>
__global__ void __cluster_dims__(2, 1, 1) __launch_bounds__(kGemmThreads, 1)
gemm_tcgen05_pair_kernel(const __grid_constant__ CUtensorMap tm_a, const __grid_constant__ CUtensorMap tm_b,
                         const GemmKernelParams p) {
  using Cfg = GemmPairCfg<BLOCK_N>;
  constexpr int kStages = Cfg::kStages;
  constexpr int kHalfN = BLOCK_N / 2;

  extern __shared__ uint8_t smem_raw[];
  __shared__ __align__(8) uint64_t full_bar[kStages];
  __shared__ __align__(8) uint64_t empty_bar[kStages];
  __shared__ __align__(8) uint64_t tmem_full_bar[2];
  __shared__ __align__(8) uint64_t tmem_empty_bar[2];
  __shared__ uint32_t tmem_base_smem;

  const int warp = threadIdx.x >> 5;
  const int lane = threadIdx.x & 31;
  const uint32_t cta_rank = cluster_ctarank();
  const bool leader = cta_rank == 0;
  const int pair_id = (int)cluster_id_x();
  const int num_pairs = (int)cluster_nctaid_x();
  const uint32_t smem0 = (smem_u32(smem_raw) + 1023u) & ~1023u;
  uint8_t* smem_gen = smem_raw + (smem0 - smem_u32(smem_raw));
  const uint32_t full0 = smem_u32(full_bar), empty0 = smem_u32(empty_bar);
  const uint32_t tfull0 = smem_u32(tmem_full_bar), tempty0 = smem_u32(tmem_empty_bar);
  const uint32_t full0_even = full0 & 0xFEFFFFFFu;
  const uint32_t tempty0_even = mapa_u32(tempty0, 0);

  if (warp == kProducerWarp && lane == 0) {
    tma_prefetch_desc(&tm_a);
    tma_prefetch_desc(&tm_b);
#pragma unroll
    for (int s = 0; s < kStages; ++s) {
      mbar_init(&full_bar[s], 1);
      mbar_init(&empty_bar[s], 1);
    }
    mbar_init(&tmem_full_bar[0], 1);
    mbar_init(&tmem_full_bar[1], 1);
    mbar_init(&tmem_empty_bar[0], 2 * 32 * kEpiWarps);
    mbar_init(&tmem_empty_bar[1], 2 * 32 * kEpiWarps);
    fence_barrier_init();
  }
  if (warp == kMmaWarp) {
    tmem_alloc_pair(&tmem_base_smem, Cfg::kTmemCols);
    tmem_relinquish_pair();
  }
  tc_fence_before();
  cluster_sync_all();
  tc_fence_after();
  pdl_launch_dependents();
  pdl_wait();
  const uint32_t tmem_base = tmem_base_smem;
  const int num_tiles = p.num_m_blocks * p.num_n_blocks;

  if (warp == kProducerWarp) {
    int stage = 0;
    uint32_t phase = 0;
    for (int tile = pair_id; tile < num_tiles; tile += num_pairs) {
      const int m_idx = (tile % p.num_m_blocks) * (2 * kBlockM) + (int)cta_rank * kBlockM;
      const int n_idx = (tile / p.num_m_blocks) * BLOCK_N + (int)cta_rank * kHalfN;
      for (int kb = 0; kb < p.num_k_blocks; ++kb) {
        mbar_wait_a(empty0 + 8u * stage, phase ^ 1);
        if (elect_one()) {
          const uint32_t sa = smem0 + (uint32_t)stage * Cfg::kStageBytes;
          const uint32_t sb = sa + Cfg::kABytes;
          const uint32_t fb = full0_even + 8u * stage;
          if (leader) mbar_arrive_expect_tx_a(full0 + 8u * stage, 2 * Cfg::kStageBytes);
          const int k_idx = kb * kBlockK;
          if constexpr (!A_MN) {
            tma_load_2d_pair_a(sa, &tm_a, fb, k_idx, m_idx);
          } else {
#pragma unroll
            for (int j = 0; j < kBlockM / 64; ++j) tma_load_2d_pair_a(sa + j * 8192, &tm_a, fb, m_idx + 64 * j, k_idx);
          }
          if constexpr (!B_MN) {
            tma_load_2d_pair_a(sb, &tm_b, fb, k_idx, n_idx);
          } else {
#pragma unroll
            for (int j = 0; j < kHalfN / 64; ++j) tma_load_2d_pair_a(sb + j * 8192, &tm_b, fb, n_idx + 64 * j, k_idx);
          }
        }
        __syncwarp();
        if (++stage == kStages) { stage = 0; phase ^= 1; }
      }
    }
  } else if (warp == kMmaWarp) {
    if (leader) {
      constexpr uint32_t idesc = umma_idesc_bf16(2 * kBlockM, BLOCK_N, A_MN, B_MN);
      const uint64_t adesc0 = umma_smem_desc(smem0, DescConsts<A_MN>::kLbo, 1024u);
      const uint64_t bdesc0 = umma_smem_desc(smem0 + Cfg::kABytes, DescConsts<B_MN>::kLbo, 1024u);
      int stage = 0;
      uint32_t phase = 0;
      int iter = 0;
      for (int tile = pair_id; tile < num_tiles; tile += num_pairs, ++iter) {
        const int acc = iter & 1;
        const uint32_t acc_phase = (iter >> 1) & 1;
        mbar_wait_a(tempty0 + 8u * acc, acc_phase ^ 1);
        tc_fence_after();
        const uint32_t d_tmem = tmem_base + (uint32_t)(acc * BLOCK_N);
        for (int kb = 0; kb < p.num_k_blocks; ++kb) {
          mbar_wait_a(full0 + 8u * stage, phase);
          tc_fence_after();
          if (elect_one()) {
            const uint32_t soff16 = ((uint32_t)stage * Cfg::kStageBytes) >> 4;
#pragma unroll
            for (int k = 0; k < kBlockK / kUmmaK; ++k) {
              umma_bf16_pair(d_tmem, desc_with_lo(adesc0, soff16 + k * DescConsts<A_MN>::kKStep16),
                             desc_with_lo(bdesc0, soff16 + k * DescConsts<B_MN>::kKStep16), idesc,
                             (kb | k) != 0 ? 1u : 0u);
            }
            umma_commit_pair_a(empty0 + 8u * stage, 0b11);
            if (kb == p.num_k_blocks - 1) umma_commit_pair_a(tfull0 + 8u * acc, 0b11);
          }
          __syncwarp();
          if (++stage == kStages) { stage = 0; phase ^= 1; }
        }
      }
    }
  } else {
    const int quad = warp & 3;
    const int half = warp >> 2;
    float* epi_stage =
        reinterpret_cast<float*>(smem_gen + (size_t)kStages * Cfg::kStageBytes) + warp * 32 * kEpiLd;
    const DropoutCfg drop = dropout_resolve(p.drop);
    const uint2 seed = make_uint2(drop.seed_lo, drop.seed_hi);
    int iter = 0;
    for (int tile = pair_id; tile < num_tiles; tile += num_pairs, ++iter) {
      const int acc = iter & 1;
      const uint32_t acc_phase = (iter >> 1) & 1;
      const int m_idx = (tile % p.num_m_blocks) * (2 * kBlockM) + (int)cta_rank * kBlockM;
      const int n_idx = (tile / p.num_m_blocks) * BLOCK_N;
      EpiOperands<EPI> ops;
      drain_prefetch<BLOCK_N, EPI>(p, m_idx + quad * 32, n_idx, half, lane, ops);
      mbar_wait_a(tfull0 + 8u * acc, acc_phase);
      tc_fence_after();
      drain_accumulator<BLOCK_N, EPI>(p, tmem_base + ((uint32_t)(quad * 32) << 16) + (uint32_t)(acc * BLOCK_N),
                                      m_idx + quad * 32, n_idx, epi_stage, lane, half, ops, seed);
      tc_fence_before();
      mbar_arrive_cluster_a(tempty0_even + 8u * acc);
    }
  }

  tc_fence_before();
  cluster_sync_all();
  if (warp == kMmaWarp) tmem_dealloc_pair(tmem_base, Cfg::kTmemCols);
}

template <int EPI0, int EPI1>
__global__ void __cluster_dims__(2, 1, 1) __launch_bounds__(kGemmThreads, 1)
gemm_tcgen05_pair_dual_kernel(const __grid_constant__ CUtensorMap tm_a0, const __grid_constant__ CUtensorMap tm_b0,
                              const __grid_constant__ CUtensorMap tm_a1, const __grid_constant__ CUtensorMap tm_b1,
                              const GemmKernelParams p0, const GemmKernelParams p1) {
  constexpr int BLOCK_N = 128;
  using Cfg = GemmPairCfg<BLOCK_N>;
  constexpr int kStages = Cfg::kStages;
  constexpr int kHalfN = BLOCK_N / 2;

  extern __shared__ uint8_t smem_raw[];
  __shared__ __align__(8) uint64_t full_bar[kStages];
  __shared__ __align__(8) uint64_t empty_bar[kStages];
  __shared__ __align__(8) uint64_t tmem_full_bar[2];
  __shared__ __align__(8) uint64_t tmem_empty_bar[2];
  __shared__ uint32_t tmem_base_smem;

  const int warp = threadIdx.x >> 5;
  const int lane = threadIdx.x & 31;
  const uint32_t cta_rank = cluster_ctarank();
  const bool leader = cta_rank == 0;
  const int pair_id = (int)cluster_id_x();
  const int num_pairs = (int)cluster_nctaid_x();
  const uint32_t smem0 = (smem_u32(smem_raw) + 1023u) & ~1023u;
  uint8_t* smem_gen = smem_raw + (smem0 - smem_u32(smem_raw));
  const uint32_t full0 = smem_u32(full_bar), empty0 = smem_u32(empty_bar);
  const uint32_t tfull0 = smem_u32(tmem_full_bar), tempty0 = smem_u32(tmem_empty_bar);
  const uint32_t full0_even = full0 & 0xFEFFFFFFu;
  const uint32_t tempty0_even = mapa_u32(tempty0, 0);

  if (warp == kProducerWarp && lane == 0) {
    tma_prefetch_desc(&tm_a0);
    tma_prefetch_desc(&tm_b0);
    tma_prefetch_desc(&tm_a1);
    tma_prefetch_desc(&tm_b1);
#pragma unroll
    for (int s = 0; s < kStages; ++s) {
      mbar_init(&full_bar[s], 1);
      mbar_init(&empty_bar[s], 1);
    }
    mbar_init(&tmem_full_bar[0], 1);
    mbar_init(&tmem_full_bar[1], 1);
    mbar_init(&tmem_empty_bar[0], 2 * 32 * kEpiWarps);
    mbar_init(&tmem_empty_bar[1], 2 * 32 * kEpiWarps);
    fence_barrier_init();
  }
  if (warp == kMmaWarp) {
    tmem_alloc_pair(&tmem_base_smem, Cfg::kTmemCols);
    tmem_relinquish_pair();
  }
  tc_fence_before();
  cluster_sync_all();
  tc_fence_after();
  pdl_launch_dependents();
  pdl_wait();
  const uint32_t tmem_base = tmem_base_smem;
  const int tiles0 = p0.num_m_blocks * p0.num_n_blocks;
  const int num_tiles = tiles0 + p1.num_m_blocks * p1.num_n_blocks;

  if (warp == kProducerWarp) {
    int stage = 0;
    uint32_t phase = 0;
    for (int tile = pair_id; tile < num_tiles; tile += num_pairs) {
      const bool second = tile >= tiles0;
      const int lt = second ? tile - tiles0 : tile;
      const int mb = second ? p1.num_m_blocks : p0.num_m_blocks;
      const int nkb = second ? p1.num_k_blocks : p0.num_k_blocks;
      const CUtensorMap* ta = second ? &tm_a1 : &tm_a0;
      const CUtensorMap* tb = second ? &tm_b1 : &tm_b0;
      const int m_idx = (lt % mb) * (2 * kBlockM) + (int)cta_rank * kBlockM;
      const int n_idx = (lt / mb) * BLOCK_N + (int)cta_rank * kHalfN;
      for (int kb = 0; kb < nkb; ++kb) {
        mbar_wait_a(empty0 + 8u * stage, phase ^ 1);
        if (elect_one()) {
          const uint32_t sa = smem0 + (uint32_t)stage * Cfg::kStageBytes;
          const uint32_t sb = sa + Cfg::kABytes;
          const uint32_t fb = full0_even + 8u * stage;
          if (leader) mbar_arrive_expect_tx_a(full0 + 8u * stage, 2 * Cfg::kStageBytes);
          const int k_idx = kb * kBlockK;
          if (!second) {
            tma_load_2d_pair_a(sa, ta, fb, k_idx, m_idx);
          } else {
#pragma unroll
            for (int j = 0; j < kBlockM / 64; ++j) tma_load_2d_pair_a(sa + j * 8192, ta, fb, m_idx + 64 * j, k_idx);
          }
#pragma unroll
          for (int j = 0; j < kHalfN / 64; ++j) tma_load_2d_pair_a(sb + j * 8192, tb, fb, n_idx + 64 * j, k_idx);
        }
        __syncwarp();
        if (++stage == kStages) { stage = 0; phase ^= 1; }
      }
    }
  } else if (warp == kMmaWarp) {
    if (leader) {
      constexpr uint32_t idesc0 = umma_idesc_bf16(2 * kBlockM, BLOCK_N, false, true);
      constexpr uint32_t idesc1 = umma_idesc_bf16(2 * kBlockM, BLOCK_N, true, true);
      const uint64_t adesc_k = umma_smem_desc(smem0, DescConsts<false>::kLbo, 1024u);
      const uint64_t adesc_mn = umma_smem_desc(smem0, DescConsts<true>::kLbo, 1024u);
      const uint64_t bdesc0 = umma_smem_desc(smem0 + Cfg::kABytes, DescConsts<true>::kLbo, 1024u);
      int stage = 0;
      uint32_t phase = 0;
      int iter = 0;
      for (int tile = pair_id; tile < num_tiles; tile += num_pairs, ++iter) {
        const bool second = tile >= tiles0;
        const int nkb = second ? p1.num_k_blocks : p0.num_k_blocks;
        const uint32_t idesc = second ? idesc1 : idesc0;
        const uint64_t adesc0 = second ? adesc_mn : adesc_k;
        const uint32_t a_kstep = second ? DescConsts<true>::kKStep16 : DescConsts<false>::kKStep16;
        const int acc = iter & 1;
        const uint32_t acc_phase = (iter >> 1) & 1;
        mbar_wait_a(tempty0 + 8u * acc, acc_phase ^ 1);
        tc_fence_after();
        const uint32_t d_tmem = tmem_base + (uint32_t)(acc * BLOCK_N);
        for (int kb = 0; kb < nkb; ++kb) {
          mbar_wait_a(full0 + 8u * stage, phase);
          tc_fence_after();
          if (elect_one()) {
            const uint32_t soff16 = ((uint32_t)stage * Cfg::kStageBytes) >> 4;
#pragma unroll
            for (int k = 0; k < kBlockK / kUmmaK; ++k) {
              umma_bf16_pair(d_tmem, desc_with_lo(adesc0, soff16 + k * a_kstep),
                             desc_with_lo(bdesc0, soff16 + k * DescConsts<true>::kKStep16), idesc, (kb | k) != 0 ? 1u : 0u);
            }
            umma_commit_pair_a(empty0 + 8u * stage, 0b11);
            if (kb == nkb - 1) umma_commit_pair_a(tfull0 + 8u * acc, 0b11);
          }
          __syncwarp();
          if (++stage == kStages) { stage = 0; phase ^= 1; }
        }
      }
    }
  } else {
    const int quad = warp & 3;
    const int half = warp >> 2;
    float* epi_stage =
        reinterpret_cast<float*>(smem_gen + (size_t)kStages * Cfg::kStageBytes) + warp * 32 * kEpiLd;
    const uint2 seed = make_uint2(0u, 0u);
    int iter = 0;
    for (int tile = pair_id; tile < num_tiles; tile += num_pairs, ++iter) {
      const bool second = tile >= tiles0;
      const int lt = second ? tile - tiles0 : tile;
      const int mb = second ? p1.num_m_blocks : p0.num_m_blocks;
      const int acc = iter & 1;
      const uint32_t acc_phase = (iter >> 1) & 1;
      const int m_idx = (lt % mb) * (2 * kBlockM) + (int)cta_rank * kBlockM;
      const int n_idx = (lt / mb) * BLOCK_N;
      const uint32_t t_row = tmem_base + ((uint32_t)(quad * 32) << 16) + (uint32_t)(acc * BLOCK_N);
      if (!second) {
        EpiOperands<EPI0> ops;
        drain_prefetch<BLOCK_N, EPI0>(p0, m_idx + quad * 32, n_idx, half, lane, ops);
        mbar_wait_a(tfull0 + 8u * acc, acc_phase);
        tc_fence_after();
        drain_accumulator<BLOCK_N, EPI0>(p0, t_row, m_idx + quad * 32, n_idx, epi_stage, lane, half, ops, seed);
      } else {
        EpiOperands<EPI1> ops;
        drain_prefetch<BLOCK_N, EPI1>(p1, m_idx + quad * 32, n_idx, half, lane, ops);
        mbar_wait_a(tfull0 + 8u * acc, acc_phase);
        tc_fence_after();
        drain_accumulator<BLOCK_N, EPI1>(p1, t_row, m_idx + quad * 32, n_idx, epi_stage, lane, half, ops, seed);
      }
      tc_fence_before();
      mbar_arrive_cluster_a(tempty0_even + 8u * acc);
    }
  }

  tc_fence_before();
  cluster_sync_all();
  if (warp == kMmaWarp) tmem_dealloc_pair(tmem_base, Cfg::kTmemCols);
}

typedef CUresult (*EncodeTiledFn)(CUtensorMap*, CUtensorMapDataType, cuuint32_t, void*, const cuuint64_t*,
                                  const cuuint64_t*, const cuuint32_t*, const cuuint32_t*,
                                  CUtensorMapInterleave, CUtensorMapSwizzle, CUtensorMapL2promotion,
                                  CUtensorMapFloatOOBfill);

static EncodeTiledFn get_encode_fn() {
  static EncodeTiledFn fn = nullptr;
  static std::once_flag once;
  std::call_once(once, [] {
    void* ptr = nullptr;
    cudaDriverEntryPointQueryResult qres;
    cudaError_t e = cudaGetDriverEntryPoint("cuTensorMapEncodeTiled", &ptr, cudaEnableDefault, &qres);
    if (e == cudaSuccess && qres == cudaDriverEntryPointSuccess) fn = reinterpret_cast<EncodeTiledFn>(ptr);
  });
  return fn;
}

static int make_tmap_bf16(CUtensorMap* tm, const void* base, uint64_t inner, uint64_t outer,
                          uint64_t ld_elems, uint32_t box_outer) {
  EncodeTiledFn fn = get_encode_fn();
  if (fn == nullptr) {
    set_last_error("cuTensorMapEncodeTiled not available from the driver");
    return B200B_ERR_DRIVER;
  }
  cuuint64_t dims[2] = {inner, outer};
  cuuint64_t strides[1] = {ld_elems * 2};
  cuuint32_t box[2] = {64, box_outer};
  cuuint32_t estr[2] = {1, 1};
  CUresult r = fn(tm, CU_TENSOR_MAP_DATA_TYPE_BFLOAT16, 2, const_cast<void*>(base), dims, strides, box, estr,
                  CU_TENSOR_MAP_INTERLEAVE_NONE, CU_TENSOR_MAP_SWIZZLE_128B, CU_TENSOR_MAP_L2_PROMOTION_L2_256B,
                  CU_TENSOR_MAP_FLOAT_OOB_FILL_NONE);
  if (r != CUDA_SUCCESS) {
    set_last_error("cuTensorMapEncodeTiled failed (%d): inner=%llu outer=%llu ld=%llu box_outer=%u base=%p", (int)r,
                   (unsigned long long)inner, (unsigned long long)outer, (unsigned long long)ld_elems, box_outer, base);
    return B200B_ERR_TENSORMAP;
  }
  return B200B_OK;
}

template <bool PAIR, int BLOCK_N, bool A_MN, bool B_MN, int EPI>
static int launch_gemm(const CUtensorMap& ta, const CUtensorMap& tb, const GemmKernelParams& p, int grid,
                       cudaStream_t stream) {
  static bool configured = false;
  if constexpr (PAIR) {
    auto kern = gemm_tcgen05_pair_kernel<BLOCK_N, A_MN, B_MN, EPI>;
    if (!configured) {
      cudaError_t e = cudaFuncSetAttribute(kern, cudaFuncAttributeMaxDynamicSharedMemorySize,
                                           (int)GemmPairCfg<BLOCK_N>::kSmemBytes);
      if (e != cudaSuccess) {
        set_last_error("cudaFuncSetAttribute(gemm pair) failed: %s", cudaGetErrorString(e));
        return (int)e;
      }
      configured = true;
    }
    launch_pdl(kPdlGemm, kern, dim3(grid), dim3(kGemmThreads), GemmPairCfg<BLOCK_N>::kSmemBytes, stream, ta, tb, p);
    return check_launch("gemm_tcgen05_pair_kernel", stream);
  } else {
    auto kern = gemm_tcgen05_kernel<BLOCK_N, A_MN, B_MN, EPI>;
    if (!configured) {
      cudaError_t e = cudaFuncSetAttribute(kern, cudaFuncAttributeMaxDynamicSharedMemorySize,
                                           (int)GemmCfg<BLOCK_N>::kSmemBytes);
      if (e != cudaSuccess) {
        set_last_error("cudaFuncSetAttribute(gemm) failed: %s", cudaGetErrorString(e));
        return (int)e;
      }
      configured = true;
    }
    launch_pdl(kPdlGemm, kern, dim3(grid), dim3(kGemmThreads), GemmCfg<BLOCK_N>::kSmemBytes, stream, ta, tb, p);
    return check_launch("gemm_tcgen05_kernel", stream);
  }
}

template <bool PAIR, int BLOCK_N, bool A_MN, bool B_MN>
static int dispatch_epi(int epi, const CUtensorMap& ta, const CUtensorMap& tb, const GemmKernelParams& p, int grid,
                        cudaStream_t stream) {
  switch (epi) {
    case B200B_EPI_BF16_BIAS:
      return launch_gemm<PAIR, BLOCK_N, A_MN, B_MN, B200B_EPI_BF16_BIAS>(ta, tb, p, grid, stream);
    case B200B_EPI_BF16_DGELU:
      return launch_gemm<PAIR, BLOCK_N, A_MN, B_MN, B200B_EPI_BF16_DGELU>(ta, tb, p, grid, stream);
    case B200B_EPI_F32:
      return launch_gemm<PAIR, BLOCK_N, A_MN, B_MN, B200B_EPI_F32>(ta, tb, p, grid, stream);
    default:
      break;
  }
  if constexpr (!A_MN && !B_MN) {
    switch (epi) {
      case B200B_EPI_BF16_BIAS_GELU:
        return launch_gemm<PAIR, BLOCK_N, false, false, B200B_EPI_BF16_BIAS_GELU>(ta, tb, p, grid, stream);
      case B200B_EPI_F32_BIAS_RESID:
        return launch_gemm<PAIR, BLOCK_N, false, false, B200B_EPI_F32_BIAS_RESID>(ta, tb, p, grid, stream);
      default:
        break;
    }
  }
  set_last_error("gemm: epilogue %d not built for a_major=%d b_major=%d", epi, (int)A_MN, (int)B_MN);
  return B200B_ERR_ARG;
}

template <bool PAIR, int BLOCK_N>
static int dispatch_major(int a_mn, int b_mn, int epi, const CUtensorMap& ta, const CUtensorMap& tb,
                          const GemmKernelParams& p, int grid, cudaStream_t stream) {
  if (!a_mn && !b_mn) return dispatch_epi<PAIR, BLOCK_N, false, false>(epi, ta, tb, p, grid, stream);
  if (!a_mn && b_mn) return dispatch_epi<PAIR, BLOCK_N, false, true>(epi, ta, tb, p, grid, stream);
  if (a_mn && b_mn) return dispatch_epi<PAIR, BLOCK_N, true, true>(epi, ta, tb, p, grid, stream);
  set_last_error("gemm: a_major=1,b_major=0 is not built");
  return B200B_ERR_ARG;
}

static bool aligned16(const void* p) { return (reinterpret_cast<uintptr_t>(p) & 15) == 0; }

struct TileChoice {
  int cta_group, block_n;
};

TileChoice choose_tile(int m, int n, int num_sms) {
  const long long units = num_sms >= 2 ? num_sms / 2 : 1;
  double best = 1e300;
  TileChoice out{2, 256};
  const int widths[2] = {256, 128};
  for (int bn : widths) {
    const long long tiles = ((m + 255) / 256) * (long long)((n + bn - 1) / bn);
    const long long waves = (tiles + units - 1) / units;
    const double cost = (double)waves * bn / (bn == 256 ? 1.0 : 0.88);
    if (cost < best) { best = cost; out = {2, bn}; }
  }
  return out;
}

}

using namespace b200b;

extern "C" int b200b_gemm(const b200b_gemm_args* a, void* stream_) {
  cudaStream_t stream = reinterpret_cast<cudaStream_t>(stream_);
  if (a == nullptr || a->a == nullptr || a->b == nullptr || a->out == nullptr) {
    set_last_error("gemm: null argument");
    return B200B_ERR_ARG;
  }
  if (a->m <= 0 || a->n <= 0 || a->k <= 0 || (a->n % 8) != 0) {
    set_last_error("gemm: need m,n,k > 0 and n a multiple of 8 (got m=%d n=%d k=%d)", a->m, a->n, a->k);
    return B200B_ERR_SHAPE;
  }
  const int epi = a->epilogue;
  if (epi < 0 || epi > B200B_EPI_F32) {
    set_last_error("gemm: bad epilogue %d", epi);
    return B200B_ERR_ARG;
  }
  const bool out_f32 = (epi == B200B_EPI_F32_BIAS_RESID || epi == B200B_EPI_F32);
  if (!aligned16(a->a) || !aligned16(a->b) || !aligned16(a->out) || (a->lda % 8) || (a->ldb % 8) ||
      (a->ldo % (out_f32 ? 4 : 8))) {
    set_last_error("gemm: operands must be 16-byte aligned with 16-byte aligned row pitch");
    return B200B_ERR_ALIGN;
  }
  if (a->bias != nullptr && !aligned16(a->bias)) {
    set_last_error("gemm: bias must be 16-byte aligned");
    return B200B_ERR_ALIGN;
  }
  if (epi == B200B_EPI_BF16_BIAS_GELU || epi == B200B_EPI_BF16_DGELU) {
    if (a->aux == nullptr || !aligned16(a->aux) || (a->ldaux % 8)) {
      set_last_error("gemm: epilogue %d needs a 16-byte aligned aux tensor", epi);
      return B200B_ERR_ARG;
    }
  }
  if (epi == B200B_EPI_F32_BIAS_RESID) {
    if (a->resid == nullptr || !aligned16(a->resid) || (a->ldr % 4)) {
      set_last_error("gemm: residual epilogue needs a 16-byte aligned resid tensor");
      return B200B_ERR_ARG;
    }
  }
  if (!(a->dropout_p >= 0.0f && a->dropout_p < 1.0f)) {
    set_last_error("gemm: dropout_p must be in [0,1)");
    return B200B_ERR_ARG;
  }
  int num_sms = 0;
  int rc = device_sm_count(&num_sms);
  if (rc != B200B_OK) return rc;

  int block_n = a->block_n;
  int cta_group = (int)a->cta_group;
  if (block_n == 0 || cta_group == 0) {
    const TileChoice c = choose_tile(a->m, a->n, num_sms);
    if (block_n == 0 && cta_group == 0) { block_n = c.block_n; cta_group = c.cta_group; }
    else if (block_n == 0) block_n = 256;
    else cta_group = 1;
  }
  if ((block_n != 128 && block_n != 256) || (cta_group != 1 && cta_group != 2)) {
    set_last_error("gemm: block_n must be 0, 128 or 256 and cta_group 0, 1 or 2");
    return B200B_ERR_ARG;
  }
  if (num_sms < 2) cta_group = 1;
  const bool pair = cta_group == 2;
  const int b_rows = pair ? block_n / 2 : block_n;

  CUtensorMap ta, tb;
  if (!a->a_major) rc = make_tmap_bf16(&ta, a->a, (uint64_t)a->k, (uint64_t)a->m, (uint64_t)a->lda, kBlockM);
  else             rc = make_tmap_bf16(&ta, a->a, (uint64_t)a->m, (uint64_t)a->k, (uint64_t)a->lda, kBlockK);
  if (rc != B200B_OK) return rc;
  if (!a->b_major) rc = make_tmap_bf16(&tb, a->b, (uint64_t)a->k, (uint64_t)a->n, (uint64_t)a->ldb, (uint32_t)b_rows);
  else             rc = make_tmap_bf16(&tb, a->b, (uint64_t)a->n, (uint64_t)a->k, (uint64_t)a->ldb, kBlockK);
  if (rc != B200B_OK) return rc;

  GemmKernelParams p;
  p.m = a->m; p.n = a->n; p.k = a->k;
  const int tile_m = pair ? 2 * kBlockM : kBlockM;
  p.num_m_blocks = (a->m + tile_m - 1) / tile_m;
  p.num_n_blocks = (a->n + block_n - 1) / block_n;
  p.num_k_blocks = (a->k + kBlockK - 1) / kBlockK;
  p.out = a->out; p.ldo = a->ldo;
  p.aux = a->aux; p.ldaux = a->ldaux;
  p.bias = a->bias;
  p.resid = a->resid; p.ldr = a->ldr;
  p.beta = a->beta;
  p.drop_stream = a->dropout_stream;
  p.drop = make_dropout_cfg(a->dropout_p, a->seed, &p.drop_stream);

  const long long tiles = (long long)p.num_m_blocks * p.num_n_blocks;
  if (pair) {
    const long long pairs = num_sms / 2;
    const int grid = 2 * (int)(tiles < pairs ? tiles : pairs);
    if (block_n == 256) return dispatch_major<true, 256>(a->a_major, a->b_major, epi, ta, tb, p, grid, stream);
    return dispatch_major<true, 128>(a->a_major, a->b_major, epi, ta, tb, p, grid, stream);
  }
  const int grid = (int)(tiles < num_sms ? tiles : num_sms);
  if (block_n == 256) return dispatch_major<false, 256>(a->a_major, a->b_major, epi, ta, tb, p, grid, stream);
  return dispatch_major<false, 128>(a->a_major, a->b_major, epi, ta, tb, p, grid, stream);
}

namespace b200b {

static void fill_params(const b200b_gemm_args* a, GemmKernelParams* p) {
  p->m = a->m; p->n = a->n; p->k = a->k;
  p->num_m_blocks = (a->m + 2 * kBlockM - 1) / (2 * kBlockM);
  p->num_n_blocks = (a->n + 127) / 128;
  p->num_k_blocks = (a->k + kBlockK - 1) / kBlockK;
  p->out = a->out; p->ldo = a->ldo;
  p->aux = nullptr; p->ldaux = 0;
  p->bias = a->bias;
  p->resid = nullptr; p->ldr = 0;
  p->beta = a->beta;
  p->drop_stream = 0;
  p->drop = make_dropout_cfg(0.f, 0, nullptr);
}

template <int EPI1>
static int launch_dual(const CUtensorMap& ta0, const CUtensorMap& tb0, const CUtensorMap& ta1, const CUtensorMap& tb1,
                       const GemmKernelParams& p0, const GemmKernelParams& p1, int grid, cudaStream_t stream) {
  static bool configured = false;
  auto kern = gemm_tcgen05_pair_dual_kernel<B200B_EPI_BF16_BIAS, EPI1>;
  if (!configured) {
    cudaError_t e = cudaFuncSetAttribute(kern, cudaFuncAttributeMaxDynamicSharedMemorySize, (int)GemmPairCfg<128>::kSmemBytes);
    if (e != cudaSuccess) {
      set_last_error("cudaFuncSetAttribute(gemm dual) failed: %s", cudaGetErrorString(e));
      return (int)e;
    }
    configured = true;
  }
  launch_pdl(kPdlGemm, kern, dim3(grid), dim3(kGemmThreads), GemmPairCfg<128>::kSmemBytes, stream, ta0, tb0, ta1, tb1, p0, p1);
  return check_launch("gemm_tcgen05_pair_dual_kernel", stream);
}

static int g_gemm_dual = -1;

}

extern "C" int b200b_gemm_set_dual(int on) {
  if (g_gemm_dual < 0) {
    const char* e = getenv("B200B_GEMM_DUAL");
    g_gemm_dual = e ? atoi(e) : 1;
  }
  const int prev = g_gemm_dual;
  if (on >= 0) g_gemm_dual = on;
  return prev;
}

extern "C" int b200b_gemm_dual(const b200b_gemm_args* dgrad, const b200b_gemm_args* wgrad, void* stream_) {
  cudaStream_t stream = reinterpret_cast<cudaStream_t>(stream_);
  if (dgrad == nullptr || wgrad == nullptr) {
    set_last_error("gemm_dual: null argument");
    return B200B_ERR_ARG;
  }
  int num_sms = 0;
  int rc = device_sm_count(&num_sms);
  if (rc != B200B_OK) return rc;
  const bool eligible =
      b200b_gemm_set_dual(-1) != 0 && num_sms >= 2 && dgrad->a_major == 0 && dgrad->b_major == 1 && dgrad->epilogue == B200B_EPI_BF16_BIAS &&
      dgrad->bias == nullptr && wgrad->a_major == 1 && wgrad->b_major == 1 &&
      (wgrad->epilogue == B200B_EPI_F32 || wgrad->epilogue == B200B_EPI_BF16_BIAS) && wgrad->bias == nullptr &&
      wgrad->beta == 0.f && dgrad->dropout_p == 0.f && wgrad->dropout_p == 0.f && dgrad->block_n == 0 && wgrad->block_n == 0 &&
      dgrad->cta_group == 0 && wgrad->cta_group == 0 && dgrad->m > 0 && dgrad->n > 0 && dgrad->k > 0 && wgrad->m > 0 &&
      wgrad->n > 0 && wgrad->k > 0 && (dgrad->n % 8) == 0 && (wgrad->n % 8) == 0 &&
      choose_tile(dgrad->m, dgrad->n, num_sms).block_n == 128 && choose_tile(wgrad->m, wgrad->n, num_sms).block_n == 128 &&
      aligned16(dgrad->a) && aligned16(dgrad->b) && aligned16(dgrad->out) && aligned16(wgrad->a) && aligned16(wgrad->b) &&
      aligned16(wgrad->out) && (dgrad->lda % 8) == 0 && (dgrad->ldb % 8) == 0 && (dgrad->ldo % 8) == 0 &&
      (wgrad->lda % 8) == 0 && (wgrad->ldb % 8) == 0 && (wgrad->ldo % (wgrad->epilogue == B200B_EPI_F32 ? 4 : 8)) == 0;
  if (!eligible) {
    rc = b200b_gemm(wgrad, stream_);
    if (rc != B200B_OK) return rc;
    return b200b_gemm(dgrad, stream_);
  }
  CUtensorMap ta0, tb0, ta1, tb1;
  if ((rc = make_tmap_bf16(&ta0, dgrad->a, (uint64_t)dgrad->k, (uint64_t)dgrad->m, (uint64_t)dgrad->lda, kBlockM)) != B200B_OK) return rc;
  if ((rc = make_tmap_bf16(&tb0, dgrad->b, (uint64_t)dgrad->n, (uint64_t)dgrad->k, (uint64_t)dgrad->ldb, kBlockK)) != B200B_OK) return rc;
  if ((rc = make_tmap_bf16(&ta1, wgrad->a, (uint64_t)wgrad->m, (uint64_t)wgrad->k, (uint64_t)wgrad->lda, kBlockK)) != B200B_OK) return rc;
  if ((rc = make_tmap_bf16(&tb1, wgrad->b, (uint64_t)wgrad->n, (uint64_t)wgrad->k, (uint64_t)wgrad->ldb, kBlockK)) != B200B_OK) return rc;
  GemmKernelParams p0, p1;
  fill_params(dgrad, &p0);
  fill_params(wgrad, &p1);
  const long long tiles = (long long)p0.num_m_blocks * p0.num_n_blocks + (long long)p1.num_m_blocks * p1.num_n_blocks;
  const long long pairs = num_sms / 2;
  const int grid = 2 * (int)(tiles < pairs ? tiles : pairs);
  if (wgrad->epilogue == B200B_EPI_F32) return launch_dual<B200B_EPI_F32>(ta0, tb0, ta1, tb1, p0, p1, grid, stream);
  return launch_dual<B200B_EPI_BF16_BIAS>(ta0, tb0, ta1, tb1, p0, p1, grid, stream);
}
```

### vlm-bridge-for-image-captioning_b200/ops.py

```python
from __future__ import annotations

import ctypes as C

import torch

from . import _lib
from ._lib import (EPI_BF16_BIAS, EPI_BF16_BIAS_GELU, EPI_BF16_DGELU, EPI_F32,
                   EPI_F32_BIAS_RESID)


def _stream_ptr() -> C.c_void_p:
    return C.c_void_p(torch.cuda.current_stream().cuda_stream)


def _ptr(t: torch.Tensor | None) -> int | None:
    return None if t is None else t.data_ptr()


def _need_cuda(*ts: torch.Tensor | None) -> None:
    for t in ts:
        if t is not None and not t.is_cuda:
            raise RuntimeError("b200 bridge kernels need CUDA tensors (there is no CPU fallback)")


def gemm(a: torch.Tensor, b: torch.Tensor, *, a_major: int = 0, b_major: int = 0,
         epilogue: int = EPI_BF16_BIAS, out: torch.Tensor | None = None,
         bias: torch.Tensor | None = None, aux: torch.Tensor | None = None,
         resid: torch.Tensor | None = None, beta: float = 0.0, dropout_p: float = 0.0,
         seed: int = 0, dropout_stream: int = 0, block_n: int = 0, cta_group: int = 0) -> torch.Tensor:
    _need_cuda(a, b, out, bias, aux, resid)
    if a.dtype != torch.bfloat16 or b.dtype != torch.bfloat16:
        raise RuntimeError("gemm operands must be bf16")
    if a.dim() != 2 or b.dim() != 2 or a.stride(1) != 1 or b.stride(1) != 1:
        raise RuntimeError("gemm operands must be 2-D with unit inner stride")
    m, k = (a.shape[1], a.shape[0]) if a_major else (a.shape[0], a.shape[1])
    n, kb = (b.shape[1], b.shape[0]) if b_major else (b.shape[0], b.shape[1])
    if k != kb:
        raise RuntimeError(f"gemm: contraction mismatch {k} vs {kb}")
    out_f32 = epilogue in (EPI_F32_BIAS_RESID, EPI_F32)
    if out is None:
        out = torch.empty((m, n), device=a.device, dtype=torch.float32 if out_f32 else torch.bfloat16)
    if out.dtype != (torch.float32 if out_f32 else torch.bfloat16) or out.shape != (m, n) or out.stride(1) != 1:
        raise RuntimeError("gemm: bad `out` tensor")
    if epilogue == EPI_BF16_BIAS_GELU and aux is None:
        aux = torch.empty((m, n), device=a.device, dtype=torch.bfloat16)
    args = _lib.GemmArgs(
        a=a.data_ptr(), b=b.data_ptr(), a_major=a_major, b_major=b_major, m=m, n=n, k=k,
        lda=a.stride(0), ldb=b.stride(0), epilogue=epilogue, block_n=block_n,
        out=out.data_ptr(), ldo=out.stride(0),
        aux=_ptr(aux), ldaux=0 if aux is None else aux.stride(0),
        bias=_ptr(bias), resid=_ptr(resid), ldr=0 if resid is None else resid.stride(0),
        beta=beta, dropout_p=dropout_p, seed=seed, dropout_stream=dropout_stream, cta_group=cta_group)
    _lib.check(_lib.lib().b200b_gemm(C.byref(args), _stream_ptr()), "gemm")
    if epilogue == EPI_BF16_BIAS_GELU:
        return out, aux
    return out


def layernorm_fwd(x: torch.Tensor, gamma: torch.Tensor, beta: torch.Tensor, eps: float = 1e-5):
    _need_cuda(x, gamma, beta)
    rows, dim = x.shape
    y = torch.empty((rows, dim), device=x.device, dtype=torch.bfloat16)
    mean = torch.empty(rows, device=x.device, dtype=torch.float32)
    rstd = torch.empty(rows, device=x.device, dtype=torch.float32)
    _lib.check(_lib.lib().b200b_layernorm_fwd(x.data_ptr(), gamma.data_ptr(), beta.data_ptr(), y.data_ptr(),
                                              mean.data_ptr(), rstd.data_ptr(), rows, dim, eps, _stream_ptr()),
               "layernorm_fwd")
    return y, mean, rstd


def layernorm_bwd(dy: torch.Tensor, x: torch.Tensor, mean: torch.Tensor, rstd: torch.Tensor,
                  gamma: torch.Tensor, dres: torch.Tensor | None = None, out: torch.Tensor | None = None):
    _need_cuda(dy, x, mean, rstd, gamma, dres, out)
    rows, dim = x.shape
    if out is None:
        out = torch.empty_like(x)
    _lib.check(_lib.lib().b200b_layernorm_bwd(dy.data_ptr(), x.data_ptr(), mean.data_ptr(), rstd.data_ptr(),
                                              gamma.data_ptr(), _ptr(dres), out.data_ptr(), rows, dim,
                                              _stream_ptr()), "layernorm_bwd")
    return out


def layernorm_fwd_rows(x: torch.Tensor, gamma: torch.Tensor, beta: torch.Tensor, eps: float = 1e-5):
    _need_cuda(x, gamma, beta)
    rows, dim = x.shape
    y = torch.empty((rows, dim), device=x.device, dtype=torch.bfloat16)
    mean = torch.empty(rows, device=x.device, dtype=torch.float32)
    rstd = torch.empty(rows, device=x.device, dtype=torch.float32)
    _lib.check(_lib.lib().b200b_layernorm_fwd_rows(x.data_ptr(), gamma.data_ptr(), beta.data_ptr(), y.data_ptr(),
                                                   mean.data_ptr(), rstd.data_ptr(), rows, dim, eps, _stream_ptr()),
               "layernorm_fwd_rows")
    return y, mean, rstd


def finalize_colsums(tasks) -> None:
    arr = (_lib.ColsumTask * len(tasks))()
    for i, (part, out, cols, chunks, stride) in enumerate(tasks):
        arr[i] = _lib.ColsumTask(part.data_ptr(), out.data_ptr(), cols, chunks, stride)
    _lib.check(_lib.lib().b200b_colsum_finalize(arr, len(tasks), _stream_ptr()), "colsum_finalize")


def layernorm_bwd_fused(dy, x, mean, rstd, gamma, dres=None, want_dx=True, want_dy_next=True):
    _need_cuda(dy, x, mean, rstd, gamma, dres)
    rows, dim = x.shape
    chunks = _lib.lib().b200b_row_chunks(rows)
    part = torch.empty((chunks, 3, dim), device=x.device, dtype=torch.float32)
    dx = torch.empty_like(x) if want_dx else None
    dyn = torch.empty((rows, dim), device=x.device, dtype=torch.bfloat16) if (want_dx and want_dy_next) else None
    _lib.check(_lib.lib().b200b_layernorm_bwd_fused(dy.data_ptr(), x.data_ptr(), mean.data_ptr(), rstd.data_ptr(),
                                                    gamma.data_ptr(), _ptr(dres), _ptr(dx), _ptr(dyn), part.data_ptr(),
                                                    rows, dim, _stream_ptr()), "layernorm_bwd_fused")
    outs = [torch.empty(dim, device=x.device, dtype=torch.float32) for _ in range(3)]
    n_out = 3 if dyn is not None else 2
    finalize_colsums([(part[0, j], outs[j], dim, chunks, 3 * dim) for j in range(n_out)])
    return dx, dyn, outs[0], outs[1], (outs[2] if dyn is not None else None)


def cast_bf16_colsum(x: torch.Tensor, dropout_p: float = 0.0, seed: int = 0, dropout_stream: int = 0):
    _need_cuda(x)
    rows, dim = x.shape
    chunks = _lib.lib().b200b_row_chunks(rows)
    part = torch.empty((chunks, dim), device=x.device, dtype=torch.float32)
    out = torch.empty((rows, dim), device=x.device, dtype=torch.bfloat16)
    _lib.check(_lib.lib().b200b_cast_bf16_colsum(x.data_ptr(), out.data_ptr(), part.data_ptr(), rows, dim, dropout_p,
                                                 seed, dropout_stream, _stream_ptr()), "cast_bf16_colsum")
    s = torch.empty(dim, device=x.device, dtype=torch.float32)
    finalize_colsums([(part, s, dim, chunks, dim)])
    return out, s


def colsum_two_stage(dy: torch.Tensor) -> torch.Tensor:
    _need_cuda(dy)
    rows, cols = dy.shape
    part = torch.empty((64, cols), device=dy.device, dtype=torch.float32)
    ch = C.c_int(0)
    _lib.check(_lib.lib().b200b_colsum_partials(dy.data_ptr(), dy.stride(0), rows, cols, part.data_ptr(), C.byref(ch),
                                                _stream_ptr()), "colsum_partials")
    s = torch.empty(cols, device=dy.device, dtype=torch.float32)
    finalize_colsums([(part, s, cols, ch.value, cols)])
    return s


def colsum(dy: torch.Tensor, *, x: torch.Tensor | None = None, mean: torch.Tensor | None = None,
           rstd: torch.Tensor | None = None, out_sum: torch.Tensor | None = None,
           out_gsum: torch.Tensor | None = None, workspace: torch.Tensor | None = None):
    _need_cuda(dy, x, out_sum, out_gsum)
    rows, cols = dy.shape
    if out_sum is None:
        out_sum = torch.empty(cols, device=dy.device, dtype=torch.float32)
    if x is not None and out_gsum is None:
        out_gsum = torch.empty(cols, device=dy.device, dtype=torch.float32)
    nbytes = _lib.lib().b200b_colsum_workspace_bytes(rows, cols)
    if workspace is None:
        workspace = torch.empty(nbytes, device=dy.device, dtype=torch.uint8)
    _lib.check(_lib.lib().b200b_colsum(dy.data_ptr(), dy.stride(0), _ptr(x), _ptr(mean), _ptr(rstd),
                                       out_sum.data_ptr(), _ptr(out_gsum), rows, cols, workspace.data_ptr(),
                                       workspace.numel(), _stream_ptr()), "colsum")
    return (out_sum, out_gsum) if x is not None else out_sum


def cast_bf16(x: torch.Tensor, out: torch.Tensor | None = None, dropout_p: float = 0.0, seed: int = 0,
              dropout_stream: int = 0) -> torch.Tensor:
    _need_cuda(x, out)
    if not x.is_contiguous() or x.dtype != torch.float32:
        raise RuntimeError("cast_bf16 needs a contiguous fp32 tensor")
    if out is None:
        out = torch.empty(x.shape, device=x.device, dtype=torch.bfloat16)
    _lib.check(_lib.lib().b200b_cast_bf16(x.data_ptr(), out.data_ptr(), x.numel(), dropout_p, seed,
                                          dropout_stream, _stream_ptr()), "cast_bf16")
    return out


def _attn_args(q, k, v, o, lse, batch, heads, len_q, len_k, head_dim, dropout_p, seed, dropout_stream):
    return _lib.AttnArgs(q=q.data_ptr(), ldq=q.stride(0), k=k.data_ptr(), ldk=k.stride(0),
                         v=v.data_ptr(), ldv=v.stride(0), o=o.data_ptr(), ldo=o.stride(0),
                         lse=lse.data_ptr(), batch=batch, heads=heads, len_q=len_q, len_k=len_k,
                         head_dim=head_dim, dropout_p=dropout_p, seed=seed, dropout_stream=dropout_stream,
                         reserved=0)


def attention_fwd(q: torch.Tensor, k: torch.Tensor, v: torch.Tensor, *, batch: int, heads: int,
                  len_q: int, len_k: int, head_dim: int, dropout_p: float = 0.0, seed: int = 0,
                  dropout_stream: int = 0, out: torch.Tensor | None = None):
    _need_cuda(q, k, v, out)
    if out is None:
        out = torch.empty((batch * len_q, heads * head_dim), device=q.device, dtype=torch.bfloat16)
    lse = torch.empty((batch, heads, len_q), device=q.device, dtype=torch.float32)
    args = _attn_args(q, k, v, out, lse, batch, heads, len_q, len_k, head_dim, dropout_p, seed, dropout_stream)
    _lib.check(_lib.lib().b200b_attention_fwd(C.byref(args), _stream_ptr()), "attention_fwd")
    return out, lse


def attention_bwd(d_o: torch.Tensor, q: torch.Tensor, k: torch.Tensor, v: torch.Tensor, o: torch.Tensor,
                  lse: torch.Tensor, dq: torch.Tensor, dk: torch.Tensor, dv: torch.Tensor, *, batch: int,
                  heads: int, len_q: int, len_k: int, head_dim: int, dropout_p: float = 0.0, seed: int = 0,
                  dropout_stream: int = 0, workspace: torch.Tensor | None = None) -> None:
    _need_cuda(d_o, q, k, v, o, lse, dq, dk, dv)
    nbytes = _lib.lib().b200b_attention_bwd_workspace_bytes(batch, heads, len_q, len_k)
    if workspace is None:
        workspace = torch.empty(nbytes, device=q.device, dtype=torch.uint8)
    args = _attn_args(q, k, v, o, lse, batch, heads, len_q, len_k, head_dim, dropout_p, seed, dropout_stream)
    args.d_o, args.lddo = d_o.data_ptr(), d_o.stride(0)
    args.dq, args.lddq = dq.data_ptr(), dq.stride(0)
    args.dk, args.lddk = dk.data_ptr(), dk.stride(0)
    args.dv, args.lddv = dv.data_ptr(), dv.stride(0)
    args.workspace, args.workspace_bytes = workspace.data_ptr(), workspace.numel()
    _lib.check(_lib.lib().b200b_attention_bwd(C.byref(args), _stream_ptr()), "attention_bwd")


def kv_cache_pack(kv: torch.Tensor, *, batch: int, len_k: int, heads: int, head_dim: int,
                  num_blocks: int) -> torch.Tensor:
    _need_cuda(kv)
    nbytes = _lib.lib().b200b_kv_cache_packed_bytes(batch, len_k, heads, head_dim, num_blocks)
    packed = torch.empty(nbytes, device=kv.device, dtype=torch.uint8)
    _lib.check(_lib.lib().b200b_kv_cache_pack(kv.data_ptr(), kv.stride(0), packed.data_ptr(), batch, len_k, heads,
                                              head_dim, num_blocks, _stream_ptr()), "kv_cache_pack")
    return packed


def attention_decode_packed(q: torch.Tensor, kv_packed: torch.Tensor, *, block_index: int, num_blocks: int,
                            batch: int, heads: int, len_q: int, len_k: int, head_dim: int,
                            out: torch.Tensor | None = None, want_lse: bool = True):
    _need_cuda(q, kv_packed, out)
    if out is None:
        out = torch.empty((batch * len_q, heads * head_dim), device=q.device, dtype=torch.bfloat16)
    lse = torch.empty((batch, heads, len_q), device=q.device, dtype=torch.float32) if want_lse else None
    _lib.check(_lib.lib().b200b_attention_decode_packed(
        q.data_ptr(), q.stride(0), kv_packed.data_ptr(), block_index, num_blocks, out.data_ptr(), out.stride(0),
        _ptr(lse), batch, heads, len_q, len_k, head_dim, _stream_ptr()), "attention_decode_packed")
    return out, lse


def kv_cache_pack_tc(kv: torch.Tensor, *, batch: int, len_k: int, heads: int, head_dim: int,
                     num_blocks: int) -> torch.Tensor:
    _need_cuda(kv)
    nbytes = _lib.lib().b200b_kv_cache_tc_bytes(batch, len_k, heads, head_dim, num_blocks)
    packed = torch.empty(nbytes, device=kv.device, dtype=torch.uint8)
    _lib.check(_lib.lib().b200b_kv_cache_pack_tc(kv.data_ptr(), kv.stride(0), packed.data_ptr(), batch, len_k, heads,
                                                 head_dim, num_blocks, _stream_ptr()), "kv_cache_pack_tc")
    return packed


def attention_decode_tc(q: torch.Tensor, kv_tc: torch.Tensor, *, block_index: int, num_blocks: int, batch: int,
                        heads: int, len_q: int, len_k: int, head_dim: int, out: torch.Tensor | None = None,
                        want_lse: bool = True):
    _need_cuda(q, kv_tc, out)
    if out is None:
        out = torch.empty((batch * len_q, heads * head_dim), device=q.device, dtype=torch.bfloat16)
    lse = torch.empty((batch, heads, len_q), device=q.device, dtype=torch.float32) if want_lse else None
    _lib.check(_lib.lib().b200b_attention_decode_tc(
        q.data_ptr(), q.stride(0), kv_tc.data_ptr(), block_index, num_blocks, out.data_ptr(), out.stride(0),
        _ptr(lse), batch, heads, len_q, len_k, head_dim, _stream_ptr()), "attention_decode_tc")
    return out, lse


def gemm_grad_pair(dy: torch.Tensor, w: torch.Tensor, x: torch.Tensor, *, wgrad_dtype: torch.dtype = torch.float32):
    _need_cuda(dy, w, x)
    rows, n_out = dy.shape
    n_in = w.shape[1]
    dx = torch.empty((rows, n_in), device=dy.device, dtype=torch.bfloat16)
    dw = torch.empty((n_out, n_in), device=dy.device, dtype=wgrad_dtype)
    dg = _lib.GemmArgs(a=dy.data_ptr(), b=w.data_ptr(), a_major=0, b_major=1, m=rows, n=n_in, k=n_out, lda=dy.stride(0),
                       ldb=w.stride(0), epilogue=EPI_BF16_BIAS, block_n=0, out=dx.data_ptr(), ldo=dx.stride(0), aux=None,
                       ldaux=0, bias=None, resid=None, ldr=0, beta=0.0, dropout_p=0.0, seed=0, dropout_stream=0, cta_group=0)
    wg = _lib.GemmArgs(a=dy.data_ptr(), b=x.data_ptr(), a_major=1, b_major=1, m=n_out, n=n_in, k=rows, lda=dy.stride(0),
                       ldb=x.stride(0), epilogue=EPI_F32 if wgrad_dtype == torch.float32 else EPI_BF16_BIAS, block_n=0,
                       out=dw.data_ptr(), ldo=dw.stride(0), aux=None, ldaux=0, bias=None, resid=None, ldr=0, beta=0.0,
                       dropout_p=0.0, seed=0, dropout_stream=0, cta_group=0)
    _lib.check(_lib.lib().b200b_gemm_dual(C.byref(dg), C.byref(wg), _stream_ptr()), "gemm_dual")
    return dx, dw
```

Measured before the change: 5022.

## Fold bias-gradient column sums into weight-gradient GEMM via extra ones tile

Bias gradients are now computed inside the weight-gradient GEMM. An extra N block multiplies dY^T by a constant all-ones B tile held in device memory and loaded by TMA, and its epilogue writes only the first accumulator column. This replaces the separate colsum-partials kernels and their finalize steps for b2, b1, bqkv_s, bq_c and bkv, which removes extra launches and extra passes over the gradient activations. In exchange every affected GEMM gets an extra tile column of MMA work and more branching in its producer, MMA and epilogue paths, and the ones tile reuses loaded stages across k-blocks, which is easy to get wrong.

```diff
diff --git a/include/b200_bridge.h b/include/b200_bridge.h
--- a/include/b200_bridge.h
+++ b/include/b200_bridge.h
@@ -56,6 +56,7 @@
   uint64_t seed;
   uint32_t dropout_stream;
   uint32_t cta_group;
+  float* bias_grad;
 } b200b_gemm_args;
 
 int b200b_gemm(const b200b_gemm_args* args, void* stream);
diff --git a/vlm-bridge-for-image-captioning_b200/_lib.py b/vlm-bridge-for-image-captioning_b200/_lib.py
--- a/vlm-bridge-for-image-captioning_b200/_lib.py
+++ b/vlm-bridge-for-image-captioning_b200/_lib.py
@@ -41,6 +41,7 @@
         ("seed", C.c_uint64),
         ("dropout_stream", C.c_uint32),
         ("cta_group", C.c_uint32),
+        ("bias_grad", C.c_void_p),
     ]
 
 
diff --git a/vlm-bridge-for-image-captioning_b200/csrc/bridge.cu b/vlm-bridge-for-image-captioning_b200/csrc/bridge.cu
--- a/vlm-bridge-for-image-captioning_b200/csrc/bridge.cu
+++ b/vlm-bridge-for-image-captioning_b200/csrc/bridge.cu
@@ -90,7 +90,7 @@
   __nv_bfloat16 *dy, *du, *dxn, *dattn, *dqkv;
   float* dx;
   uint8_t* attn_ws; size_t attn_ws_bytes;
-  float *p_cast, *p_du, *p_lnf, *p_dqkv, *p_lns, *p_dq, *p_lnc, *p_dkv;
+  float *p_lnf, *p_lns, *p_lnc;
   size_t bytes;
 };
 
@@ -110,14 +110,9 @@
   w.attn_ws = c.take<uint8_t>(w.attn_ws_bytes);
   const size_t rc = d.T < (size_t)kMaxRowChunks ? d.T : (size_t)kMaxRowChunks;
   const size_t D = d.D;
-  w.p_cast = c.take<float>(rc * D);
-  w.p_du = c.take<float>((size_t)64 * d.F);
   w.p_lnf = c.take<float>(rc * 3 * D);
-  w.p_dqkv = c.take<float>((size_t)64 * 3 * D);
   w.p_lns = c.take<float>(rc * 3 * D);
-  w.p_dq = c.take<float>((size_t)64 * D);
   w.p_lnc = c.take<float>(rc * 3 * D);
-  w.p_dkv = c.take<float>((size_t)64 * 2 * D * d.nb);
   w.bytes = c.off;
   return w;
 }
@@ -139,7 +134,7 @@
 
 static int gemm(const void* a, int a_major, long long lda, const void* b, int b_major, long long ldb, int m, int n,
                 int k, int epi, void* out, long long ldo, const float* bias, const float* resid, void* aux,
-                long long ldaux, float p, uint64_t seed, uint32_t dstream, cudaStream_t st) {
+                long long ldaux, float p, uint64_t seed, uint32_t dstream, cudaStream_t st, float* bias_grad = nullptr) {
   b200b_gemm_args g;
   memset(&g, 0, sizeof(g));
   g.a = a; g.b = b; g.a_major = a_major; g.b_major = b_major;
@@ -148,11 +143,12 @@
   g.out = out; g.ldo = ldo; g.aux = aux; g.ldaux = ldaux;
   g.bias = bias; g.resid = resid; g.ldr = ldo;
   g.beta = 0.f; g.dropout_p = p; g.seed = seed; g.dropout_stream = dstream;
+  g.bias_grad = bias_grad;
   return b200b_gemm(&g, st);
 }
 
 static int grad_pair(const void* dy, long long lddy, const void* w, const void* x, long long ldx, int rows, int n_out,
-                     int n_in, void* dx, long long lddx, void* dw, int wgrad_epi, cudaStream_t st) {
+                     int n_in, void* dx, long long lddx, void* dw, int wgrad_epi, float* db, cudaStream_t st) {
   b200b_gemm_args dg, wg;
   memset(&dg, 0, sizeof(dg));
   memset(&wg, 0, sizeof(wg));
@@ -164,6 +160,7 @@
   wg.b = x; wg.b_major = 1; wg.ldb = ldx;
   wg.m = n_out; wg.n = n_in; wg.k = rows;
   wg.epilogue = wgrad_epi; wg.out = dw; wg.ldo = n_in;
+  wg.bias_grad = db;
   return b200b_gemm_dual(&dg, &wg, st);
 }
 
@@ -321,44 +318,36 @@
     return B200B_ERR_DEVICE;
   }
   Finalizer fin;
-  int ch = 0;
-
-  B200B_TRY(b200b_cast_bf16_colsum(d_out, ws.dy, ws.p_cast, T, D, p, seed, (ds_ffn_o(i) | ind), st));
-  fin.add(ws.p_cast, g->b2, D, rchunks, D);
-  B200B_TRY(gemm(ws.dy, 1, D, s.h, 1, F, D, F, T, EW, g->w2, F, nullptr, nullptr, nullptr, 0, 0.f, 0, 0, st));
+
+  B200B_TRY(b200b_cast_bf16(d_out, ws.dy, (int64_t)T * D, p, seed, (ds_ffn_o(i) | ind), st));
+  B200B_TRY(gemm(ws.dy, 1, D, s.h, 1, F, D, F, T, EW, g->w2, F, nullptr, nullptr, nullptr, 0, 0.f, 0, 0, st, g->b2));
   ready(g->w2, (long long)D * F);
   B200B_TRY(gemm(ws.dy, 0, D, w->w2, 1, F, T, F, D, B200B_EPI_BF16_DGELU, ws.du, F, nullptr, nullptr, s.u, F, p, seed,
                  (ds_ffn_h(i) | ind), st));
-  B200B_TRY(b200b_colsum_partials(ws.du, F, T, F, ws.p_du, &ch, st));
-  fin.add(ws.p_du, g->b1, F, ch, F);
-  B200B_TRY(gemm(ws.du, 1, F, s.xn3, 1, D, F, D, T, EW, g->w1, D, nullptr, nullptr, nullptr, 0, 0.f, 0, 0, st));
+  B200B_TRY(gemm(ws.du, 1, F, s.xn3, 1, D, F, D, T, EW, g->w1, D, nullptr, nullptr, nullptr, 0, 0.f, 0, 0, st, g->b1));
   ready(g->w1, (long long)F * D);
   B200B_TRY(gemm(ws.du, 0, F, w->w1, 1, D, T, D, F, EB, ws.dxn, D, nullptr, nullptr, nullptr, 0, 0.f, 0, 0, st));
   B200B_TRY(b200b_layernorm_bwd_fused(ws.dxn, s.x2, s.mean3, s.rstd3, w->ln_f_g, d_out, ws.dx, ws.dy, ws.p_lnf, T, D, st));
   fin.add(ws.p_lnf, g->ln_f_b, D, rchunks, 3LL * D);
   fin.add(ws.p_lnf + D, g->ln_f_g, D, rchunks, 3LL * D);
   fin.add(ws.p_lnf + 2 * D, g->bo_s, D, rchunks, 3LL * D);
-  B200B_TRY(grad_pair(ws.dy, D, w->wo_s, s.o2, D, T, D, D, ws.dattn, D, g->wo_s, EW, st));
+  B200B_TRY(grad_pair(ws.dy, D, w->wo_s, s.o2, D, T, D, D, ws.dattn, D, g->wo_s, EW, nullptr, st));
   ready(g->wo_s, (long long)D * D);
   B200B_TRY(attn(true, s.qkv, 3 * D, s.qkv + D, 3 * D, s.qkv + 2 * D, 3 * D, s.o2, D, s.lse2, ws.dattn, ws.dqkv, 3 * D,
                  ws.dqkv + D, 3 * D, ws.dqkv + 2 * D, 3 * D, ws.attn_ws, ws.attn_ws_bytes, d.B, d.Hs, d.L, d.L, d.ds, p,
                  seed, (ds_self(i) | ind), st));
-  B200B_TRY(b200b_colsum_partials(ws.dqkv, 3 * D, T, 3 * D, ws.p_dqkv, &ch, st));
-  fin.add(ws.p_dqkv, g->bqkv_s, 3 * D, ch, 3LL * D);
-  B200B_TRY(grad_pair(ws.dqkv, 3 * D, w->wqkv_s, s.xn2, D, T, 3 * D, D, ws.dxn, D, g->wqkv_s, EW, st));
+  B200B_TRY(grad_pair(ws.dqkv, 3 * D, w->wqkv_s, s.xn2, D, T, 3 * D, D, ws.dxn, D, g->wqkv_s, EW, g->bqkv_s, st));
   ready(g->wqkv_s, 3LL * D * D);
   B200B_TRY(b200b_layernorm_bwd_fused(ws.dxn, s.x1, s.mean2, s.rstd2, w->ln_s_g, ws.dx, ws.dx, ws.dy, ws.p_lns, T, D, st));
   fin.add(ws.p_lns, g->ln_s_b, D, rchunks, 3LL * D);
   fin.add(ws.p_lns + D, g->ln_s_g, D, rchunks, 3LL * D);
   fin.add(ws.p_lns + 2 * D, g->bo_c, D, rchunks, 3LL * D);
-  B200B_TRY(grad_pair(ws.dy, D, w->wo_c, s.o1, D, T, D, D, ws.dattn, D, g->wo_c, EW, st));
+  B200B_TRY(grad_pair(ws.dy, D, w->wo_c, s.o1, D, T, D, D, ws.dattn, D, g->wo_c, EW, nullptr, st));
   ready(g->wo_c, (long long)D * D);
   __nv_bfloat16* dq = ws.dqkv;
   B200B_TRY(attn(true, s.q, D, kblk, ldkv, kblk + D, ldkv, s.o1, D, s.lse1, ws.dattn, dq, D, dkblk, ldkv, dkblk + D, ldkv,
                  ws.attn_ws, ws.attn_ws_bytes, d.B, d.Hc, d.L, d.Nv, d.dc, p, seed, (ds_cross(i) | ind), st));
-  B200B_TRY(b200b_colsum_partials(dq, D, T, D, ws.p_dq, &ch, st));
-  fin.add(ws.p_dq, g->bq_c, D, ch, D);
-  B200B_TRY(grad_pair(dq, D, w->wq_c, s.xn1, D, T, D, D, ws.dxn, D, g->wq_c, EW, st));
+  B200B_TRY(grad_pair(dq, D, w->wq_c, s.xn1, D, T, D, D, ws.dxn, D, g->wq_c, EW, g->bq_c, st));
   ready(g->wq_c, (long long)D * D);
   B200B_TRY(b200b_layernorm_bwd_fused(ws.dxn, x_in, s.mean1, s.rstd1, w->ln_c_g, ws.dx, d_in, nullptr, ws.p_lnc, T, D, st));
   fin.add(ws.p_lnc, g->ln_c_b, D, rchunks, 3LL * D);
@@ -382,12 +371,7 @@
     return B200B_ERR_WORKSPACE;
   }
   const int n = 2 * d.D * d.nb;
-  int ch = 0;
-  B200B_TRY(b200b_colsum_partials(dkv, n, (int)d.Tv, n, ws.p_dkv, &ch, st));
-  b200b_colsum_task t;
-  t.partials = ws.p_dkv; t.out = dbkv_all; t.cols = n; t.chunks = ch; t.chunk_stride = n;
-  B200B_TRY(b200b_colsum_finalize(&t, 1, st));
   const int EW = (d.flags & B200B_BRIDGE_WGRAD_BF16) ? B200B_EPI_BF16_BIAS : B200B_EPI_F32;
   return gemm(dkv, 1, n, vision_bf16, 1, d.Dv, n, d.Dv, (int)d.Tv, EW, dwkv_all, d.Dv, nullptr, nullptr,
-              nullptr, 0, 0.f, 0, 0, st);
-}
+              nullptr, 0, 0.f, 0, 0, st, dbkv_all);
+}
diff --git a/vlm-bridge-for-image-captioning_b200/csrc/common.cuh b/vlm-bridge-for-image-captioning_b200/csrc/common.cuh
--- a/vlm-bridge-for-image-captioning_b200/csrc/common.cuh
+++ b/vlm-bridge-for-image-captioning_b200/csrc/common.cuh
@@ -231,6 +231,9 @@
       : "r"(taddr)
       : "memory");
 }
+__device__ __forceinline__ void tmem_ld_32x32_x1(uint32_t taddr, uint32_t& v) {
+  asm volatile("tcgen05.ld.sync.aligned.32x32b.x1.b32 {%0}, [%1];" : "=r"(v) : "r"(taddr) : "memory");
+}
 __device__ __forceinline__ void tmem_ld_wait() {
   asm volatile("tcgen05.wait::ld.sync.aligned;" ::: "memory");
 }
diff --git a/vlm-bridge-for-image-captioning_b200/csrc/gemm_sm100.cu b/vlm-bridge-for-image-captioning_b200/csrc/gemm_sm100.cu
--- a/vlm-bridge-for-image-captioning_b200/csrc/gemm_sm100.cu
+++ b/vlm-bridge-for-image-captioning_b200/csrc/gemm_sm100.cu
@@ -1,6 +1,7 @@
 #include <stdarg.h>
 #include <stdio.h>
 #include <stdlib.h>
+#include <string.h>
 
 #include <mutex>
 
@@ -23,6 +24,7 @@
   float beta;
   DropoutCfg drop;
   uint32_t drop_stream;
+  float* bias_grad;
 };
 
 constexpr int kBlockM = 128;
@@ -236,6 +238,30 @@
   }
 }
 
+struct OnesTile {
+  uint32_t v[64 * 64 / 2];
+  constexpr OnesTile() : v() {
+    for (int i = 0; i < 64 * 64 / 2; ++i) v[i] = 0x3f803f80u;
+  }
+};
+__device__ __align__(128) OnesTile g_ones_tile = OnesTile();
+
+constexpr int kOnesN = 64;
+__device__ __forceinline__ bool ones_loads_b(int kb, int stages) { return kb < stages; }
+
+template <bool A_MN>
+__device__ __forceinline__ bool is_bias_grad_block(const GemmKernelParams& p, int n_blk) {
+  if constexpr (A_MN) return p.bias_grad != nullptr && n_blk == p.num_n_blocks - 1;
+  else return false;
+}
+
+__device__ __forceinline__ void store_bias_grad(const GemmKernelParams& p, uint32_t t_row, int row0, int lane) {
+  uint32_t v;
+  tmem_ld_32x32_x1(t_row, v);
+  tmem_ld_wait();
+  if (row0 + lane < p.m) p.bias_grad[row0 + lane] = __uint_as_float(v);
+}
+
 template <bool MN>
 struct DescConsts {
   static constexpr uint32_t kLbo = MN ? 8192u : 16u;
@@ -248,7 +274,7 @@
 template <int BLOCK_N, bool A_MN, bool B_MN, int EPI>
 __global__ void __launch_bounds__(kGemmThreads, 1)
 gemm_tcgen05_kernel(const __grid_constant__ CUtensorMap tm_a, const __grid_constant__ CUtensorMap tm_b,
-                    const GemmKernelParams p) {
+                    const __grid_constant__ CUtensorMap tm_ones, const GemmKernelParams p) {
   using Cfg = GemmCfg<BLOCK_N>;
   constexpr int kStages = Cfg::kStages;
 
@@ -269,6 +295,7 @@
   if (warp == kProducerWarp && lane == 0) {
     tma_prefetch_desc(&tm_a);
     tma_prefetch_desc(&tm_b);
+    if (is_bias_grad_block<A_MN>(p, p.num_n_blocks - 1)) tma_prefetch_desc(&tm_ones);
 #pragma unroll
     for (int s = 0; s < kStages; ++s) {
       mbar_init(&full_bar[s], 1);
@@ -298,13 +325,15 @@
     for (int tile = blockIdx.x; tile < num_tiles; tile += gridDim.x) {
       const int m_idx = (tile % p.num_m_blocks) * kBlockM;
       const int n_idx = (tile / p.num_m_blocks) * BLOCK_N;
+      const bool ones = is_bias_grad_block<A_MN>(p, tile / p.num_m_blocks);
       for (int kb = 0; kb < p.num_k_blocks; ++kb) {
         mbar_wait_a(empty0 + 8u * stage, phase ^ 1);
         if (elect_one()) {
           const uint32_t sa = smem0 + (uint32_t)stage * Cfg::kStageBytes;
           const uint32_t sb = sa + Cfg::kABytes;
           const uint32_t fb = full0 + 8u * stage;
-          mbar_arrive_expect_tx_a(fb, Cfg::kStageBytes);
+          const bool ones_b = ones && ones_loads_b(kb, kStages);
+          mbar_arrive_expect_tx_a(fb, ones ? Cfg::kABytes + (ones_b ? 8192u : 0u) : Cfg::kStageBytes);
           const int k_idx = kb * kBlockK;
           if constexpr (!A_MN) {
             tma_load_2d_a(sa, &tm_a, fb, k_idx, m_idx);
@@ -317,8 +346,10 @@
             tma_load_2d_a(sb, &tm_b, fb, k_idx, n_idx);
           } else {
 #pragma unroll
-            for (int j = 0; j < BLOCK_N / 64; ++j)
-              tma_load_2d_a(sb + j * 8192, &tm_b, fb, n_idx + 64 * j, k_idx);
+            for (int j = 0; j < BLOCK_N / 64; ++j) {
+              if (!ones) tma_load_2d_a(sb + j * 8192, &tm_b, fb, n_idx + 64 * j, k_idx);
+            }
+            if (ones_b) tma_load_2d_a(sb, &tm_ones, fb, 0, 0);
           }
         }
         __syncwarp();
@@ -326,13 +357,15 @@
       }
     }
   } else if (warp == kMmaWarp) {
-    constexpr uint32_t idesc = umma_idesc_bf16(kBlockM, BLOCK_N, A_MN, B_MN);
+    constexpr uint32_t idesc_full = umma_idesc_bf16(kBlockM, BLOCK_N, A_MN, B_MN);
+    constexpr uint32_t idesc_ones = umma_idesc_bf16(kBlockM, kOnesN, A_MN, B_MN);
     const uint64_t adesc0 = umma_smem_desc(smem0, DescConsts<A_MN>::kLbo, 1024u);
     const uint64_t bdesc0 = umma_smem_desc(smem0 + Cfg::kABytes, DescConsts<B_MN>::kLbo, 1024u);
     int stage = 0;
     uint32_t phase = 0;
     int iter = 0;
     for (int tile = blockIdx.x; tile < num_tiles; tile += gridDim.x, ++iter) {
+      const uint32_t idesc = is_bias_grad_block<A_MN>(p, tile / p.num_m_blocks) ? idesc_ones : idesc_full;
       const int acc = iter & 1;
       const uint32_t acc_phase = (iter >> 1) & 1;
       mbar_wait_a(tempty0 + 8u * acc, acc_phase ^ 1);
@@ -368,12 +401,18 @@
       const uint32_t acc_phase = (iter >> 1) & 1;
       const int m_idx = (tile % p.num_m_blocks) * kBlockM;
       const int n_idx = (tile / p.num_m_blocks) * BLOCK_N;
-      EpiOperands<EPI> ops;
-      drain_prefetch<BLOCK_N, EPI>(p, m_idx + quad * 32, n_idx, half, lane, ops);
-      mbar_wait_a(tfull0 + 8u * acc, acc_phase);
-      tc_fence_after();
-      drain_accumulator<BLOCK_N, EPI>(p, tmem_base + ((uint32_t)(quad * 32) << 16) + (uint32_t)(acc * BLOCK_N),
-                                      m_idx + quad * 32, n_idx, epi_stage, lane, half, ops, seed);
+      const uint32_t t_row = tmem_base + ((uint32_t)(quad * 32) << 16) + (uint32_t)(acc * BLOCK_N);
+      if (is_bias_grad_block<A_MN>(p, tile / p.num_m_blocks)) {
+        mbar_wait_a(tfull0 + 8u * acc, acc_phase);
+        tc_fence_after();
+        if (half == 0) store_bias_grad(p, t_row, m_idx + quad * 32, lane);
+      } else {
+        EpiOperands<EPI> ops;
+        drain_prefetch<BLOCK_N, EPI>(p, m_idx + quad * 32, n_idx, half, lane, ops);
+        mbar_wait_a(tfull0 + 8u * acc, acc_phase);
+        tc_fence_after();
+        drain_accumulator<BLOCK_N, EPI>(p, t_row, m_idx + quad * 32, n_idx, epi_stage, lane, half, ops, seed);
+      }
       tc_fence_before();
       mbar_arrive_a(tempty0 + 8u * acc);
     }
@@ -397,7 +436,7 @@
 template <int BLOCK_N, bool A_MN, bool B_MN, int EPI>
 __global__ void __cluster_dims__(2, 1, 1) __launch_bounds__(kGemmThreads, 1)
 gemm_tcgen05_pair_kernel(const __grid_constant__ CUtensorMap tm_a, const __grid_constant__ CUtensorMap tm_b,
-                         const GemmKernelParams p) {
+                         const __grid_constant__ CUtensorMap tm_ones, const GemmKernelParams p) {
   using Cfg = GemmPairCfg<BLOCK_N>;
   constexpr int kStages = Cfg::kStages;
   constexpr int kHalfN = BLOCK_N / 2;
@@ -425,6 +464,7 @@
   if (warp == kProducerWarp && lane == 0) {
     tma_prefetch_desc(&tm_a);
     tma_prefetch_desc(&tm_b);
+    if (is_bias_grad_block<A_MN>(p, p.num_n_blocks - 1)) tma_prefetch_desc(&tm_ones);
 #pragma unroll
     for (int s = 0; s < kStages; ++s) {
       mbar_init(&full_bar[s], 1);
@@ -454,13 +494,16 @@
     for (int tile = pair_id; tile < num_tiles; tile += num_pairs) {
       const int m_idx = (tile % p.num_m_blocks) * (2 * kBlockM) + (int)cta_rank * kBlockM;
       const int n_idx = (tile / p.num_m_blocks) * BLOCK_N + (int)cta_rank * kHalfN;
+      const bool ones = is_bias_grad_block<A_MN>(p, tile / p.num_m_blocks);
       for (int kb = 0; kb < p.num_k_blocks; ++kb) {
         mbar_wait_a(empty0 + 8u * stage, phase ^ 1);
         if (elect_one()) {
           const uint32_t sa = smem0 + (uint32_t)stage * Cfg::kStageBytes;
           const uint32_t sb = sa + Cfg::kABytes;
           const uint32_t fb = full0_even + 8u * stage;
-          if (leader) mbar_arrive_expect_tx_a(full0 + 8u * stage, 2 * Cfg::kStageBytes);
+          const bool ones_b = ones && ones_loads_b(kb, kStages);
+          if (leader)
+            mbar_arrive_expect_tx_a(full0 + 8u * stage, 2 * (ones ? Cfg::kABytes + (ones_b ? 8192u : 0u) : Cfg::kStageBytes));
           const int k_idx = kb * kBlockK;
           if constexpr (!A_MN) {
             tma_load_2d_pair_a(sa, &tm_a, fb, k_idx, m_idx);
@@ -472,7 +515,10 @@
             tma_load_2d_pair_a(sb, &tm_b, fb, k_idx, n_idx);
           } else {
 #pragma unroll
-            for (int j = 0; j < kHalfN / 64; ++j) tma_load_2d_pair_a(sb + j * 8192, &tm_b, fb, n_idx + 64 * j, k_idx);
+            for (int j = 0; j < kHalfN / 64; ++j) {
+              if (!ones) tma_load_2d_pair_a(sb + j * 8192, &tm_b, fb, n_idx + 64 * j, k_idx);
+            }
+            if (ones_b) tma_load_2d_pair_a(sb, &tm_ones, fb, 0, 0);
           }
         }
         __syncwarp();
@@ -481,13 +527,15 @@
     }
   } else if (warp == kMmaWarp) {
     if (leader) {
-      constexpr uint32_t idesc = umma_idesc_bf16(2 * kBlockM, BLOCK_N, A_MN, B_MN);
+      constexpr uint32_t idesc_full = umma_idesc_bf16(2 * kBlockM, BLOCK_N, A_MN, B_MN);
+      constexpr uint32_t idesc_ones = umma_idesc_bf16(2 * kBlockM, kOnesN, A_MN, B_MN);
       const uint64_t adesc0 = umma_smem_desc(smem0, DescConsts<A_MN>::kLbo, 1024u);
       const uint64_t bdesc0 = umma_smem_desc(smem0 + Cfg::kABytes, DescConsts<B_MN>::kLbo, 1024u);
       int stage = 0;
       uint32_t phase = 0;
       int iter = 0;
       for (int tile = pair_id; tile < num_tiles; tile += num_pairs, ++iter) {
+        const uint32_t idesc = is_bias_grad_block<A_MN>(p, tile / p.num_m_blocks) ? idesc_ones : idesc_full;
         const int acc = iter & 1;
         const uint32_t acc_phase = (iter >> 1) & 1;
         mbar_wait_a(tempty0 + 8u * acc, acc_phase ^ 1);
@@ -525,12 +573,18 @@
       const uint32_t acc_phase = (iter >> 1) & 1;
       const int m_idx = (tile % p.num_m_blocks) * (2 * kBlockM) + (int)cta_rank * kBlockM;
       const int n_idx = (tile / p.num_m_blocks) * BLOCK_N;
-      EpiOperands<EPI> ops;
-      drain_prefetch<BLOCK_N, EPI>(p, m_idx + quad * 32, n_idx, half, lane, ops);
-      mbar_wait_a(tfull0 + 8u * acc, acc_phase);
-      tc_fence_after();
-      drain_accumulator<BLOCK_N, EPI>(p, tmem_base + ((uint32_t)(quad * 32) << 16) + (uint32_t)(acc * BLOCK_N),
-                                      m_idx + quad * 32, n_idx, epi_stage, lane, half, ops, seed);
+      const uint32_t t_row = tmem_base + ((uint32_t)(quad * 32) << 16) + (uint32_t)(acc * BLOCK_N);
+      if (is_bias_grad_block<A_MN>(p, tile / p.num_m_blocks)) {
+        mbar_wait_a(tfull0 + 8u * acc, acc_phase);
+        tc_fence_after();
+        if (half == 0) store_bias_grad(p, t_row, m_idx + quad * 32, lane);
+      } else {
+        EpiOperands<EPI> ops;
+        drain_prefetch<BLOCK_N, EPI>(p, m_idx + quad * 32, n_idx, half, lane, ops);
+        mbar_wait_a(tfull0 + 8u * acc, acc_phase);
+        tc_fence_after();
+        drain_accumulator<BLOCK_N, EPI>(p, t_row, m_idx + quad * 32, n_idx, epi_stage, lane, half, ops, seed);
+      }
       tc_fence_before();
       mbar_arrive_cluster_a(tempty0_even + 8u * acc);
     }
@@ -545,7 +599,8 @@
 __global__ void __cluster_dims__(2, 1, 1) __launch_bounds__(kGemmThreads, 1)
 gemm_tcgen05_pair_dual_kernel(const __grid_constant__ CUtensorMap tm_a0, const __grid_constant__ CUtensorMap tm_b0,
                               const __grid_constant__ CUtensorMap tm_a1, const __grid_constant__ CUtensorMap tm_b1,
-                              const GemmKernelParams p0, const GemmKernelParams p1) {
+                              const __grid_constant__ CUtensorMap tm_ones, const GemmKernelParams p0,
+                              const GemmKernelParams p1) {
   constexpr int BLOCK_N = 128;
   using Cfg = GemmPairCfg<BLOCK_N>;
   constexpr int kStages = Cfg::kStages;
@@ -576,6 +631,7 @@
     tma_prefetch_desc(&tm_b0);
     tma_prefetch_desc(&tm_a1);
     tma_prefetch_desc(&tm_b1);
+    if (p1.bias_grad != nullptr) tma_prefetch_desc(&tm_ones);
 #pragma unroll
     for (int s = 0; s < kStages; ++s) {
       mbar_init(&full_bar[s], 1);
@@ -612,13 +668,16 @@
       const CUtensorMap* tb = second ? &tm_b1 : &tm_b0;
       const int m_idx = (lt % mb) * (2 * kBlockM) + (int)cta_rank * kBlockM;
       const int n_idx = (lt / mb) * BLOCK_N + (int)cta_rank * kHalfN;
+      const bool ones = second && is_bias_grad_block<true>(p1, lt / mb);
       for (int kb = 0; kb < nkb; ++kb) {
         mbar_wait_a(empty0 + 8u * stage, phase ^ 1);
         if (elect_one()) {
           const uint32_t sa = smem0 + (uint32_t)stage * Cfg::kStageBytes;
           const uint32_t sb = sa + Cfg::kABytes;
           const uint32_t fb = full0_even + 8u * stage;
-          if (leader) mbar_arrive_expect_tx_a(full0 + 8u * stage, 2 * Cfg::kStageBytes);
+          const bool ones_b = ones && ones_loads_b(kb, kStages);
+          if (leader)
+            mbar_arrive_expect_tx_a(full0 + 8u * stage, 2 * (ones ? Cfg::kABytes + (ones_b ? 8192u : 0u) : Cfg::kStageBytes));
           const int k_idx = kb * kBlockK;
           if (!second) {
             tma_load_2d_pair_a(sa, ta, fb, k_idx, m_idx);
@@ -627,7 +686,10 @@
             for (int j = 0; j < kBlockM / 64; ++j) tma_load_2d_pair_a(sa + j * 8192, ta, fb, m_idx + 64 * j, k_idx);
           }
 #pragma unroll
-          for (int j = 0; j < kHalfN / 64; ++j) tma_load_2d_pair_a(sb + j * 8192, tb, fb, n_idx + 64 * j, k_idx);
+          for (int j = 0; j < kHalfN / 64; ++j) {
+            if (!ones) tma_load_2d_pair_a(sb + j * 8192, tb, fb, n_idx + 64 * j, k_idx);
+          }
+          if (ones_b) tma_load_2d_pair_a(sb, &tm_ones, fb, 0, 0);
         }
         __syncwarp();
         if (++stage == kStages) { stage = 0; phase ^= 1; }
@@ -637,6 +699,7 @@
     if (leader) {
       constexpr uint32_t idesc0 = umma_idesc_bf16(2 * kBlockM, BLOCK_N, false, true);
       constexpr uint32_t idesc1 = umma_idesc_bf16(2 * kBlockM, BLOCK_N, true, true);
+      constexpr uint32_t idesc1_ones = umma_idesc_bf16(2 * kBlockM, kOnesN, true, true);
       const uint64_t adesc_k = umma_smem_desc(smem0, DescConsts<false>::kLbo, 1024u);
       const uint64_t adesc_mn = umma_smem_desc(smem0, DescConsts<true>::kLbo, 1024u);
       const uint64_t bdesc0 = umma_smem_desc(smem0 + Cfg::kABytes, DescConsts<true>::kLbo, 1024u);
@@ -646,7 +709,9 @@
       for (int tile = pair_id; tile < num_tiles; tile += num_pairs, ++iter) {
         const bool second = tile >= tiles0;
         const int nkb = second ? p1.num_k_blocks : p0.num_k_blocks;
-        const uint32_t idesc = second ? idesc1 : idesc0;
+        const int mb = second ? p1.num_m_blocks : p0.num_m_blocks;
+        const bool ones = second && is_bias_grad_block<true>(p1, (tile - tiles0) / mb);
+        const uint32_t idesc = ones ? idesc1_ones : second ? idesc1 : idesc0;
         const uint64_t adesc0 = second ? adesc_mn : adesc_k;
         const uint32_t a_kstep = second ? DescConsts<true>::kKStep16 : DescConsts<false>::kKStep16;
         const int acc = iter & 1;
@@ -694,6 +759,10 @@
         mbar_wait_a(tfull0 + 8u * acc, acc_phase);
         tc_fence_after();
         drain_accumulator<BLOCK_N, EPI0>(p0, t_row, m_idx + quad * 32, n_idx, epi_stage, lane, half, ops, seed);
+      } else if (is_bias_grad_block<true>(p1, lt / mb)) {
+        mbar_wait_a(tfull0 + 8u * acc, acc_phase);
+        tc_fence_after();
+        if (half == 0) store_bias_grad(p1, t_row, m_idx + quad * 32, lane);
       } else {
         EpiOperands<EPI1> ops;
         drain_prefetch<BLOCK_N, EPI1>(p1, m_idx + quad * 32, n_idx, half, lane, ops);
@@ -750,9 +819,36 @@
   return B200B_OK;
 }
 
+static int ones_tmap(CUtensorMap* tm) {
+  constexpr int kMaxDevices = 64;
+  static std::mutex mu;
+  static CUtensorMap maps[kMaxDevices];
+  static bool have[kMaxDevices] = {};
+  int dev = 0;
+  cudaError_t e = cudaGetDevice(&dev);
+  if (e != cudaSuccess || dev < 0 || dev >= kMaxDevices) {
+    set_last_error("gemm: no usable current device for the bias-gradient operand (%s)", cudaGetErrorString(e));
+    return B200B_ERR_DEVICE;
+  }
+  std::lock_guard<std::mutex> lk(mu);
+  if (!have[dev]) {
+    void* ones = nullptr;
+    e = cudaGetSymbolAddress(&ones, g_ones_tile);
+    if (e != cudaSuccess) {
+      set_last_error("gemm: cudaGetSymbolAddress(g_ones_tile) failed: %s", cudaGetErrorString(e));
+      return (int)e;
+    }
+    const int rc = make_tmap_bf16(&maps[dev], ones, 64, 64, 64, kBlockK);
+    if (rc != B200B_OK) return rc;
+    have[dev] = true;
+  }
+  *tm = maps[dev];
+  return B200B_OK;
+}
+
 template <bool PAIR, int BLOCK_N, bool A_MN, bool B_MN, int EPI>
-static int launch_gemm(const CUtensorMap& ta, const CUtensorMap& tb, const GemmKernelParams& p, int grid,
-                       cudaStream_t stream) {
+static int launch_gemm(const CUtensorMap& ta, const CUtensorMap& tb, const CUtensorMap& tones,
+                       const GemmKernelParams& p, int grid, cudaStream_t stream) {
   static bool configured = false;
   if constexpr (PAIR) {
     auto kern = gemm_tcgen05_pair_kernel<BLOCK_N, A_MN, B_MN, EPI>;
@@ -765,7 +861,7 @@
       }
       configured = true;
     }
-    launch_pdl(kPdlGemm, kern, dim3(grid), dim3(kGemmThreads), GemmPairCfg<BLOCK_N>::kSmemBytes, stream, ta, tb, p);
+    launch_pdl(kPdlGemm, kern, dim3(grid), dim3(kGemmThreads), GemmPairCfg<BLOCK_N>::kSmemBytes, stream, ta, tb, tones, p);
     return check_launch("gemm_tcgen05_pair_kernel", stream);
   } else {
     auto kern = gemm_tcgen05_kernel<BLOCK_N, A_MN, B_MN, EPI>;
@@ -778,30 +874,30 @@
       }
       configured = true;
     }
-    launch_pdl(kPdlGemm, kern, dim3(grid), dim3(kGemmThreads), GemmCfg<BLOCK_N>::kSmemBytes, stream, ta, tb, p);
+    launch_pdl(kPdlGemm, kern, dim3(grid), dim3(kGemmThreads), GemmCfg<BLOCK_N>::kSmemBytes, stream, ta, tb, tones, p);
     return check_launch("gemm_tcgen05_kernel", stream);
   }
 }
 
 template <bool PAIR, int BLOCK_N, bool A_MN, bool B_MN>
-static int dispatch_epi(int epi, const CUtensorMap& ta, const CUtensorMap& tb, const GemmKernelParams& p, int grid,
-                        cudaStream_t stream) {
+static int dispatch_epi(int epi, const CUtensorMap& ta, const CUtensorMap& tb, const CUtensorMap& tones,
+                        const GemmKernelParams& p, int grid, cudaStream_t stream) {
   switch (epi) {
     case B200B_EPI_BF16_BIAS:
-      return launch_gemm<PAIR, BLOCK_N, A_MN, B_MN, B200B_EPI_BF16_BIAS>(ta, tb, p, grid, stream);
+      return launch_gemm<PAIR, BLOCK_N, A_MN, B_MN, B200B_EPI_BF16_BIAS>(ta, tb, tones, p, grid, stream);
     case B200B_EPI_BF16_DGELU:
-      return launch_gemm<PAIR, BLOCK_N, A_MN, B_MN, B200B_EPI_BF16_DGELU>(ta, tb, p, grid, stream);
+      return launch_gemm<PAIR, BLOCK_N, A_MN, B_MN, B200B_EPI_BF16_DGELU>(ta, tb, tones, p, grid, stream);
     case B200B_EPI_F32:
-      return launch_gemm<PAIR, BLOCK_N, A_MN, B_MN, B200B_EPI_F32>(ta, tb, p, grid, stream);
+      return launch_gemm<PAIR, BLOCK_N, A_MN, B_MN, B200B_EPI_F32>(ta, tb, tones, p, grid, stream);
     default:
       break;
   }
   if constexpr (!A_MN && !B_MN) {
     switch (epi) {
       case B200B_EPI_BF16_BIAS_GELU:
-        return launch_gemm<PAIR, BLOCK_N, false, false, B200B_EPI_BF16_BIAS_GELU>(ta, tb, p, grid, stream);
+        return launch_gemm<PAIR, BLOCK_N, false, false, B200B_EPI_BF16_BIAS_GELU>(ta, tb, tones, p, grid, stream);
       case B200B_EPI_F32_BIAS_RESID:
-        return launch_gemm<PAIR, BLOCK_N, false, false, B200B_EPI_F32_BIAS_RESID>(ta, tb, p, grid, stream);
+        return launch_gemm<PAIR, BLOCK_N, false, false, B200B_EPI_F32_BIAS_RESID>(ta, tb, tones, p, grid, stream);
       default:
         break;
     }
@@ -812,15 +908,16 @@
 
 template <bool PAIR, int BLOCK_N>
 static int dispatch_major(int a_mn, int b_mn, int epi, const CUtensorMap& ta, const CUtensorMap& tb,
-                          const GemmKernelParams& p, int grid, cudaStream_t stream) {
-  if (!a_mn && !b_mn) return dispatch_epi<PAIR, BLOCK_N, false, false>(epi, ta, tb, p, grid, stream);
-  if (!a_mn && b_mn) return dispatch_epi<PAIR, BLOCK_N, false, true>(epi, ta, tb, p, grid, stream);
-  if (a_mn && b_mn) return dispatch_epi<PAIR, BLOCK_N, true, true>(epi, ta, tb, p, grid, stream);
+                          const CUtensorMap& tones, const GemmKernelParams& p, int grid, cudaStream_t stream) {
+  if (!a_mn && !b_mn) return dispatch_epi<PAIR, BLOCK_N, false, false>(epi, ta, tb, tones, p, grid, stream);
+  if (!a_mn && b_mn) return dispatch_epi<PAIR, BLOCK_N, false, true>(epi, ta, tb, tones, p, grid, stream);
+  if (a_mn && b_mn) return dispatch_epi<PAIR, BLOCK_N, true, true>(epi, ta, tb, tones, p, grid, stream);
   set_last_error("gemm: a_major=1,b_major=0 is not built");
   return B200B_ERR_ARG;
 }
 
 static bool aligned16(const void* p) { return (reinterpret_cast<uintptr_t>(p) & 15) == 0; }
+static bool aligned4(const void* p) { return (reinterpret_cast<uintptr_t>(p) & 3) == 0; }
 
 struct TileChoice {
   int cta_group, block_n;
@@ -885,6 +982,16 @@
     set_last_error("gemm: dropout_p must be in [0,1)");
     return B200B_ERR_ARG;
   }
+  if (a->bias_grad != nullptr) {
+    if (!a->a_major || !(epi == B200B_EPI_F32 || (epi == B200B_EPI_BF16_BIAS && a->bias == nullptr))) {
+      set_last_error("gemm: bias_grad needs the weight-gradient form (a_major=1, epilogue F32 or BF16_BIAS without bias)");
+      return B200B_ERR_ARG;
+    }
+    if (!aligned4(a->bias_grad)) {
+      set_last_error("gemm: bias_grad must be 4-byte aligned");
+      return B200B_ERR_ALIGN;
+    }
+  }
   int num_sms = 0;
   int rc = device_sm_count(&num_sms);
   if (rc != B200B_OK) return rc;
@@ -912,12 +1019,15 @@
   if (!a->b_major) rc = make_tmap_bf16(&tb, a->b, (uint64_t)a->k, (uint64_t)a->n, (uint64_t)a->ldb, (uint32_t)b_rows);
   else             rc = make_tmap_bf16(&tb, a->b, (uint64_t)a->n, (uint64_t)a->k, (uint64_t)a->ldb, kBlockK);
   if (rc != B200B_OK) return rc;
+  CUtensorMap tones;
+  memset(&tones, 0, sizeof(tones));
+  if (a->bias_grad != nullptr && (rc = ones_tmap(&tones)) != B200B_OK) return rc;
 
   GemmKernelParams p;
   p.m = a->m; p.n = a->n; p.k = a->k;
   const int tile_m = pair ? 2 * kBlockM : kBlockM;
   p.num_m_blocks = (a->m + tile_m - 1) / tile_m;
-  p.num_n_blocks = (a->n + block_n - 1) / block_n;
+  p.num_n_blocks = (a->n + block_n - 1) / block_n + (a->bias_grad != nullptr ? 1 : 0);
   p.num_k_blocks = (a->k + kBlockK - 1) / kBlockK;
   p.out = a->out; p.ldo = a->ldo;
   p.aux = a->aux; p.ldaux = a->ldaux;
@@ -926,17 +1036,18 @@
   p.beta = a->beta;
   p.drop_stream = a->dropout_stream;
   p.drop = make_dropout_cfg(a->dropout_p, a->seed, &p.drop_stream);
+  p.bias_grad = a->bias_grad;
 
   const long long tiles = (long long)p.num_m_blocks * p.num_n_blocks;
   if (pair) {
     const long long pairs = num_sms / 2;
     const int grid = 2 * (int)(tiles < pairs ? tiles : pairs);
-    if (block_n == 256) return dispatch_major<true, 256>(a->a_major, a->b_major, epi, ta, tb, p, grid, stream);
-    return dispatch_major<true, 128>(a->a_major, a->b_major, epi, ta, tb, p, grid, stream);
+    if (block_n == 256) return dispatch_major<true, 256>(a->a_major, a->b_major, epi, ta, tb, tones, p, grid, stream);
+    return dispatch_major<true, 128>(a->a_major, a->b_major, epi, ta, tb, tones, p, grid, stream);
   }
   const int grid = (int)(tiles < num_sms ? tiles : num_sms);
-  if (block_n == 256) return dispatch_major<false, 256>(a->a_major, a->b_major, epi, ta, tb, p, grid, stream);
-  return dispatch_major<false, 128>(a->a_major, a->b_major, epi, ta, tb, p, grid, stream);
+  if (block_n == 256) return dispatch_major<false, 256>(a->a_major, a->b_major, epi, ta, tb, tones, p, grid, stream);
+  return dispatch_major<false, 128>(a->a_major, a->b_major, epi, ta, tb, tones, p, grid, stream);
 }
 
 namespace b200b {
@@ -944,7 +1055,7 @@
 static void fill_params(const b200b_gemm_args* a, GemmKernelParams* p) {
   p->m = a->m; p->n = a->n; p->k = a->k;
   p->num_m_blocks = (a->m + 2 * kBlockM - 1) / (2 * kBlockM);
-  p->num_n_blocks = (a->n + 127) / 128;
+  p->num_n_blocks = (a->n + 127) / 128 + (a->bias_grad != nullptr ? 1 : 0);
   p->num_k_blocks = (a->k + kBlockK - 1) / kBlockK;
   p->out = a->out; p->ldo = a->ldo;
   p->aux = nullptr; p->ldaux = 0;
@@ -953,11 +1064,13 @@
   p->beta = a->beta;
   p->drop_stream = 0;
   p->drop = make_dropout_cfg(0.f, 0, nullptr);
+  p->bias_grad = a->bias_grad;
 }
 
 template <int EPI1>
 static int launch_dual(const CUtensorMap& ta0, const CUtensorMap& tb0, const CUtensorMap& ta1, const CUtensorMap& tb1,
-                       const GemmKernelParams& p0, const GemmKernelParams& p1, int grid, cudaStream_t stream) {
+                       const CUtensorMap& tones, const GemmKernelParams& p0, const GemmKernelParams& p1, int grid,
+                       cudaStream_t stream) {
   static bool configured = false;
   auto kern = gemm_tcgen05_pair_dual_kernel<B200B_EPI_BF16_BIAS, EPI1>;
   if (!configured) {
@@ -968,7 +1081,8 @@
     }
     configured = true;
   }
-  launch_pdl(kPdlGemm, kern, dim3(grid), dim3(kGemmThreads), GemmPairCfg<128>::kSmemBytes, stream, ta0, tb0, ta1, tb1, p0, p1);
+  launch_pdl(kPdlGemm, kern, dim3(grid), dim3(kGemmThreads), GemmPairCfg<128>::kSmemBytes, stream, ta0, tb0, ta1, tb1, tones, p0,
+             p1);
   return check_launch("gemm_tcgen05_pair_dual_kernel", stream);
 }
 
@@ -990,6 +1104,10 @@
   cudaStream_t stream = reinterpret_cast<cudaStream_t>(stream_);
   if (dgrad == nullptr || wgrad == nullptr) {
     set_last_error("gemm_dual: null argument");
+    return B200B_ERR_ARG;
+  }
+  if (dgrad->bias_grad != nullptr) {
+    set_last_error("gemm_dual: bias_grad belongs to the weight gradient (dgrad->bias_grad must be NULL)");
     return B200B_ERR_ARG;
   }
   int num_sms = 0;
@@ -1005,7 +1123,8 @@
       choose_tile(dgrad->m, dgrad->n, num_sms).block_n == 128 && choose_tile(wgrad->m, wgrad->n, num_sms).block_n == 128 &&
       aligned16(dgrad->a) && aligned16(dgrad->b) && aligned16(dgrad->out) && aligned16(wgrad->a) && aligned16(wgrad->b) &&
       aligned16(wgrad->out) && (dgrad->lda % 8) == 0 && (dgrad->ldb % 8) == 0 && (dgrad->ldo % 8) == 0 &&
-      (wgrad->lda % 8) == 0 && (wgrad->ldb % 8) == 0 && (wgrad->ldo % (wgrad->epilogue == B200B_EPI_F32 ? 4 : 8)) == 0;
+      (wgrad->lda % 8) == 0 && (wgrad->ldb % 8) == 0 && (wgrad->ldo % (wgrad->epilogue == B200B_EPI_F32 ? 4 : 8)) == 0 &&
+      aligned4(wgrad->bias_grad);
   if (!eligible) {
     rc = b200b_gemm(wgrad, stream_);
     if (rc != B200B_OK) return rc;
@@ -1016,12 +1135,15 @@
   if ((rc = make_tmap_bf16(&tb0, dgrad->b, (uint64_t)dgrad->n, (uint64_t)dgrad->k, (uint64_t)dgrad->ldb, kBlockK)) != B200B_OK) return rc;
   if ((rc = make_tmap_bf16(&ta1, wgrad->a, (uint64_t)wgrad->m, (uint64_t)wgrad->k, (uint64_t)wgrad->lda, kBlockK)) != B200B_OK) return rc;
   if ((rc = make_tmap_bf16(&tb1, wgrad->b, (uint64_t)wgrad->n, (uint64_t)wgrad->k, (uint64_t)wgrad->ldb, kBlockK)) != B200B_OK) return rc;
+  CUtensorMap tones;
+  memset(&tones, 0, sizeof(tones));
+  if (wgrad->bias_grad != nullptr && (rc = ones_tmap(&tones)) != B200B_OK) return rc;
   GemmKernelParams p0, p1;
   fill_params(dgrad, &p0);
   fill_params(wgrad, &p1);
   const long long tiles = (long long)p0.num_m_blocks * p0.num_n_blocks + (long long)p1.num_m_blocks * p1.num_n_blocks;
   const long long pairs = num_sms / 2;
   const int grid = 2 * (int)(tiles < pairs ? tiles : pairs);
-  if (wgrad->epilogue == B200B_EPI_F32) return launch_dual<B200B_EPI_F32>(ta0, tb0, ta1, tb1, p0, p1, grid, stream);
-  return launch_dual<B200B_EPI_BF16_BIAS>(ta0, tb0, ta1, tb1, p0, p1, grid, stream);
-}
+  if (wgrad->epilogue == B200B_EPI_F32) return launch_dual<B200B_EPI_F32>(ta0, tb0, ta1, tb1, tones, p0, p1, grid, stream);
+  return launch_dual<B200B_EPI_BF16_BIAS>(ta0, tb0, ta1, tb1, tones, p0, p1, grid, stream);
+}
diff --git a/vlm-bridge-for-image-captioning_b200/ops.py b/vlm-bridge-for-image-captioning_b200/ops.py
--- a/vlm-bridge-for-image-captioning_b200/ops.py
+++ b/vlm-bridge-for-image-captioning_b200/ops.py
@@ -23,12 +23,19 @@
             raise RuntimeError("b200 bridge kernels need CUDA tensors (there is no CPU fallback)")
 
 
+def _check_bias_grad(bias_grad: torch.Tensor | None, m: int) -> None:
+    if bias_grad is not None and (bias_grad.dtype != torch.float32 or tuple(bias_grad.shape) != (m,)
+                                  or bias_grad.stride(0) != 1):
+        raise RuntimeError(f"bias_grad must be a contiguous f32 tensor of shape ({m},)")
+
+
 def gemm(a: torch.Tensor, b: torch.Tensor, *, a_major: int = 0, b_major: int = 0,
          epilogue: int = EPI_BF16_BIAS, out: torch.Tensor | None = None,
          bias: torch.Tensor | None = None, aux: torch.Tensor | None = None,
          resid: torch.Tensor | None = None, beta: float = 0.0, dropout_p: float = 0.0,
-         seed: int = 0, dropout_stream: int = 0, block_n: int = 0, cta_group: int = 0) -> torch.Tensor:
-    _need_cuda(a, b, out, bias, aux, resid)
+         seed: int = 0, dropout_stream: int = 0, block_n: int = 0, cta_group: int = 0,
+         bias_grad: torch.Tensor | None = None) -> torch.Tensor:
+    _need_cuda(a, b, out, bias, aux, resid, bias_grad)
     if a.dtype != torch.bfloat16 or b.dtype != torch.bfloat16:
         raise RuntimeError("gemm operands must be bf16")
     if a.dim() != 2 or b.dim() != 2 or a.stride(1) != 1 or b.stride(1) != 1:
@@ -44,13 +51,15 @@
         raise RuntimeError("gemm: bad `out` tensor")
     if epilogue == EPI_BF16_BIAS_GELU and aux is None:
         aux = torch.empty((m, n), device=a.device, dtype=torch.bfloat16)
+    _check_bias_grad(bias_grad, m)
     args = _lib.GemmArgs(
         a=a.data_ptr(), b=b.data_ptr(), a_major=a_major, b_major=b_major, m=m, n=n, k=k,
         lda=a.stride(0), ldb=b.stride(0), epilogue=epilogue, block_n=block_n,
         out=out.data_ptr(), ldo=out.stride(0),
         aux=_ptr(aux), ldaux=0 if aux is None else aux.stride(0),
         bias=_ptr(bias), resid=_ptr(resid), ldr=0 if resid is None else resid.stride(0),
-        beta=beta, dropout_p=dropout_p, seed=seed, dropout_stream=dropout_stream, cta_group=cta_group)
+        beta=beta, dropout_p=dropout_p, seed=seed, dropout_stream=dropout_stream, cta_group=cta_group,
+        bias_grad=_ptr(bias_grad))
     _lib.check(_lib.lib().b200b_gemm(C.byref(args), _stream_ptr()), "gemm")
     if epilogue == EPI_BF16_BIAS_GELU:
         return out, aux
@@ -254,10 +263,12 @@
     return out, lse
 
 
-def gemm_grad_pair(dy: torch.Tensor, w: torch.Tensor, x: torch.Tensor, *, wgrad_dtype: torch.dtype = torch.float32):
-    _need_cuda(dy, w, x)
+def gemm_grad_pair(dy: torch.Tensor, w: torch.Tensor, x: torch.Tensor, *, wgrad_dtype: torch.dtype = torch.float32,
+                   bias_grad: torch.Tensor | None = None):
+    _need_cuda(dy, w, x, bias_grad)
     rows, n_out = dy.shape
     n_in = w.shape[1]
+    _check_bias_grad(bias_grad, n_out)
     dx = torch.empty((rows, n_in), device=dy.device, dtype=torch.bfloat16)
     dw = torch.empty((n_out, n_in), device=dy.device, dtype=wgrad_dtype)
     dg = _lib.GemmArgs(a=dy.data_ptr(), b=w.data_ptr(), a_major=0, b_major=1, m=rows, n=n_in, k=n_out, lda=dy.stride(0),
@@ -266,6 +277,6 @@
     wg = _lib.GemmArgs(a=dy.data_ptr(), b=x.data_ptr(), a_major=1, b_major=1, m=n_out, n=n_in, k=rows, lda=dy.stride(0),
                        ldb=x.stride(0), epilogue=EPI_F32 if wgrad_dtype == torch.float32 else EPI_BF16_BIAS, block_n=0,
                        out=dw.data_ptr(), ldo=dw.stride(0), aux=None, ldaux=0, bias=None, resid=None, ldr=0, beta=0.0,
-                       dropout_p=0.0, seed=0, dropout_stream=0, cta_group=0)
+                       dropout_p=0.0, seed=0, dropout_stream=0, cta_group=0, bias_grad=_ptr(bias_grad))
     _lib.check(_lib.lib().b200b_gemm_dual(C.byref(dg), C.byref(wg), _stream_ptr()), "gemm_dual")
     return dx, dw
```

Measured after the change: 5167, median of 6. 1.03x the previous value.
